# scipopt/SCIP-SDP

Measured on AMD Instinct MI355X. Metric: node-SDP solves/sec, dense block n x n with m vars (IPM iters/sec in iters_per_sec), higher is better.
Workload: dtype f64

## Files before the change

include/hipsdp_units.h:

```cpp
#ifndef HIPSDP_UNITS_H
#define HIPSDP_UNITS_H

#include "hipsdp.h"

#ifdef __cplusplus
extern "C" {
#endif

HIPSDP_API int  hipsdp_dgemm_selfcheck(int device, int M, int N, int K, int layB, int batch, int splitk, int flags, double beta,
   int* used_v2, long long* ndiff);
HIPSDP_API int  hipsdp_pass_at_unit(int device, int R, long long E, const double* A, const double* coef, double sa, const double* add, int split,
   double* out, int* chunks);
HIPSDP_API int  hipsdp_dgemm_selfcheck2(int device, int M, int N, int K, int layB, int batch, int splitk, int flags, double alpha, double beta,
   int reps, int* used, long long* ndiff, double* ms_tile, double* ms_fast);
HIPSDP_API int  hipsdp_gram_plan_info(int device, int M, long long K, int nslab, int* no, int* nd, int* nitems, double* span);
HIPSDP_API int  hipsdp_gram_selfcheck(int device, int M, long long K, int reps, int* used, double* maxdiff, long long* nrepro, double* ms_tile,
   double* ms_gram);
HIPSDP_API int  hipsdp_dgemm_selfcheck3(int device, int M, int N, int K, int layB, int batch, int splitk, int flags, double alpha, double beta,
   int reps, int* used, long long* ndiff, double* maxdiff, long long* nrepro, double* ms_tile, double* ms_fast);
HIPSDP_API int  hipsdp_schur_identity_unit(int device, int m1, int n, const double* A, double ws_gbytes, int full_storage, double* Mx,
   double* flops);
HIPSDP_API int  hipsdp_schur_dense(int device, int m1, int n, const double* A, const double* X, const double* Zinv, double* Mx,
   double ws_gbytes);
HIPSDP_API int  hipsdp_schur_w(int device, int m1, int n, const double* A, const double* X, const double* Z, double* Mx);
HIPSDP_API int  hipsdp_schur_shard_time(int device, int m1, int n, int nranks, int rank, int by_columns, int reps, double ws_gbytes, double* ms);
HIPSDP_API int  hipsdp_schur_var_share_time(int device, int m1, int n, int nranks, int rank, int cw, int reps, double* ms, double* a2a_bytes);
HIPSDP_API int  hipsdp_schur_sparse_unit(int device, int n, int m, long long nnz, const int* var, const int* row, const int* col,
   const double* val, const double* X, const double* Zinv, double* Mx);
HIPSDP_API int  hipsdp_mfma_peak(int device, double ms, double* tflops, double* ghz);
HIPSDP_API int  hipsdp_potrf(int device, int n, double* A, int* fail);
HIPSDP_API int  hipsdp_potrf_ex(int device, int n, double* A, int psd, int v1, double* dinv, int* regmask, int* fail);
HIPSDP_API int  hipsdp_potrs(int device, int n, const double* A, int nrhs, double* rhs);
HIPSDP_API int  hipsdp_potrs_seq(int device, int n, const double* A, int psd, int ncalls, const int* nrhs, const int* mode, double* rhs,
   int* regmask, int* fail);
HIPSDP_API int  hipsdp_potrf_small_unit(int device, int n, int pair, const double* base, const double* dir, double alpha, int set_flag,
   int want_gram, double* L, double* dinv, double* Mout, double* Linv, double* Gram, int* flag);
HIPSDP_API int  hipsdp_trtri(int device, int n, const double* A, double* Linv);
HIPSDP_API int  hipsdp_lambda_min(int device, int n, const double* W, int steps, double* theta, double* resid);
HIPSDP_API int  hipsdp_lambda_min_scaled(int device, int n, const double* L, const double* D, int steps, double* theta, double* resid);
HIPSDP_API int  hipsdp_solve1_fits(int m, int q, int nblk, const int* ns);
HIPSDP_API int  hipsdp_solve1_class(int m, int nblk, const int* ns);
HIPSDP_API unsigned long long hipsdp_gram_gen_next(unsigned long long* counter);
HIPSDP_API int  hipsdp_gram_key_match_unit(int m_a, int nblk_a, const int* n_a, const int* form_a, const unsigned long long* gen_a,
   const long long* ws_a, int m_b, int nblk_b, const int* n_b, const int* form_b, const unsigned long long* gen_b, const long long* ws_b);
HIPSDP_API int  hipsdp_syev_many_unit(int device, int count, const int* ns, const double* A, double* lam, double* V, int* launches);
HIPSDP_API int  hipsdp_tridiag_unit(int device, int n, const double* A, double* d, double* e, double* Vrefl, double* tau);
HIPSDP_API int  hipsdp_tvec_unit(int device, int n, const double* d, const double* e, double* lam, double* Z);

#ifdef __cplusplus
}
#endif

#endif
```

scip-sdp_amd/binding.py:

```python
import ctypes as C
import os
import numpy as np

_HERE = os.path.dirname(os.path.abspath(__file__))
LIBPATH = os.environ.get("HIPSDP_LIB", os.path.join(_HERE, "lib", "libhipsdp.so"))

STATUS_NAMES = {0: "optimal", 1: "dual_infeasible", 2: "dual_unbounded", 3: "both_infeasible", 4: "iterlimit",
                5: "numeric", 6: "timelimit", 7: "objlimit", -1: "unsolved"}


class Params(C.Structure):
    _fields_ = [("gaptol", C.c_double), ("feastol", C.c_double), ("infeastol", C.c_double), ("objlimit", C.c_double),
                ("timelimit", C.c_double), ("gamma", C.c_double), ("ws_gbytes", C.c_double), ("maxiter", C.c_int),
                ("verbose", C.c_int), ("lanczos_steps", C.c_int), ("settings", C.c_int), ("pabstol", C.c_double), ("preoptgap", C.c_double)]


class Info(C.Structure):
    _fields_ = [("status", C.c_int), ("iterations", C.c_int), ("pobj", C.c_double), ("dobj", C.c_double),
                ("pinf", C.c_double), ("dinf", C.c_double), ("dabs", C.c_double), ("gap", C.c_double), ("mu", C.c_double),
                ("tau", C.c_double), ("kappa", C.c_double), ("solve_seconds", C.c_double), ("schur_seconds", C.c_double),
                ("schur_flops", C.c_double), ("schur_calls", C.c_int), ("chol_fail", C.c_int), ("warm_started", C.c_int),
                ("settings_used", C.c_int), ("schur_flops_executed", C.c_double)]


# ... 419 lines not shown
    L = _f64(A).copy()
    n = L.shape[0]
    dinv = np.zeros(((n + 63) // 64) * 4096)
    mask = np.zeros(n, dtype=np.int32)
    fail = C.c_int(0)
    _chk(ulib().hipsdp_potrf_ex(device, n, _dp(L), int(psd), int(v1), _dp(dinv), _ip(mask), C.byref(fail)), "hipsdp_potrf_ex")
    return L, dinv, mask, fail.value


def potrs(A, rhs, device=0):
    A = _f64(A)
    r = _f64(rhs).copy()
    r2 = r.reshape(-1, A.shape[0])
    _chk(ulib().hipsdp_potrs(device, A.shape[0], _dp(A), r2.shape[0], _dp(r2)), "hipsdp_potrs")
    return r2.reshape(r.shape)


def potrs_seq(A, calls, psd=False, device=0):
    A = _f64(A)
    n = A.shape[0]
    nc = len(calls)
    slab = np.zeros((max(nc, 1), 4, n))
    nrhs = np.zeros(max(nc, 1), dtype=np.int32)
    mode = np.zeros(max(nc, 1), dtype=np.int32)
    for c, (md, r) in enumerate(calls):
        r = _f64(r).reshape(-1, n)
        nrhs[c], mode[c] = r.shape[0], md
        slab[c, :min(r.shape[0], 4)] = r[:4]
    mask = np.zeros(n, dtype=np.int32)
    fail = C.c_int(0)
    _chk(ulib().hipsdp_potrs_seq(device, n, _dp(A), int(psd), nc, _ip(nrhs), _ip(mode), _dp(slab), _ip(mask), C.byref(fail)),
         "hipsdp_potrs_seq")
    return [slab[c, :nrhs[c]].copy() for c in range(nc)], mask, fail.value


def potrf_small_unit(base, dir=None, alpha=0.0, pair=False, set_flag=False, want_gram=False, device=0):
    base = _f64(base)
    n = base.shape[-1]
    npb = 2 if pair else 1
    assert base.size == npb * n * n
    d = None if dir is None else _f64(dir)
    assert d is None or d.size == base.size
    shp = (2, n, n) if pair else (n, n)
    out = {"L": np.zeros(shp), "dinv": np.zeros((2, 64, 64) if pair else (64, 64)), "Mout": np.zeros(shp), "Linv": np.zeros(shp),
           "Gram": np.zeros(shp) if want_gram else None}
    flag = np.zeros(2, dtype=np.int32)
    _chk(ulib().hipsdp_potrf_small_unit(device, n, int(pair), _dp(base), None if d is None else _dp(d), C.c_double(alpha), int(set_flag),
                                        int(want_gram), _dp(out["L"]), _dp(out["dinv"]), _dp(out["Mout"]), _dp(out["Linv"]),
                                        None if not want_gram else _dp(out["Gram"]), _ip(flag)), "hipsdp_potrf_small_unit")
    out["flag"] = flag.copy() if pair else int(flag[0])
    return out


def trtri(A, device=0):
    A = _f64(A)
    Li = np.zeros_like(A)
    _chk(ulib().hipsdp_trtri(device, A.shape[0], _dp(A), _dp(Li)), "hipsdp_trtri")
    return Li


def lambda_min(W, steps=0, device=0):
    W = _f64(W)
    th = C.c_double(0.0)
    rs = C.c_double(0.0)
    _chk(ulib().hipsdp_lambda_min(device, W.shape[0], _dp(W), steps, C.byref(th), C.byref(rs)), "hipsdp_lambda_min")
    return th.value, rs.value


def syev(A, device=0):
    A = _f64(A)
    n = A.shape[0]
    lam = np.zeros(n)
    V = np.zeros((n, n))
    _chk(lib().hipsdp_syev(device, n, _dp(A), _dp(lam), _dp(V)), "hipsdp_syev")
    return lam, V


def syevx(A, il, iu, vectors=True, device=0):
    A = _f64(A)
    n = A.shape[0]
    k = max(0, iu - il + 1)
    lam = np.zeros(k)
    V = np.zeros((k, n)) if vectors else None
    _chk(lib().hipsdp_syevx(device, n, _dp(A), int(il), int(iu), _dp(lam), _dp(V) if vectors else None), "hipsdp_syevx")
    return lam, V


def syevx_below(A, bound, maxk, vectors=True, device=0):
    A = _f64(A)
    n = A.shape[0]
    lam = np.zeros(max(1, maxk))
    V = np.zeros((max(1, maxk), n)) if vectors else None
    cnt, nbelow = C.c_int(-1), C.c_int(-1)
    _chk(lib().hipsdp_syevx_below(device, n, _dp(A), C.c_double(bound), int(maxk), C.byref(cnt), C.byref(nbelow), _dp(lam),
                                  _dp(V) if vectors else None), "hipsdp_syevx_below")
    return lam[:cnt.value].copy(), (V[:cnt.value].copy() if vectors else None), nbelow.value


def syevr(A, vectors=True, device=0):
    A = _f64(A)
    n = A.shape[0]
    lam = np.zeros(n)
    V = np.zeros((n, n)) if vectors else None
    _chk(lib().hipsdp_syevr(device, n, _dp(A), _dp(lam), _dp(V) if vectors else None), "hipsdp_syevr")
    return lam, V

# ... 85 lines not shown
```

scip-sdp_amd/csrc/chol.hip:

```cpp
#include "hs_kernels.h"
#include "hs_wave.h"
#include <cstdlib>

#define NB 64

#ifdef PD_TIMING
__device__ long long pd_tbuf[16];
__device__ int pd_tj0;
#define PD_T(idx) do { if ( threadIdx.x == 0 && j0 == pd_tj0 && blockIdx.x == (gridDim.x > 1 ? 1u : 0u) ) pd_tbuf[idx] = wall_clock64(); } while (0)
extern "C" __attribute__((visibility("default"))) int hipsdp_debug_pd_timing(int j0, long long* out)
{
   if ( out != NULL && hipMemcpyFromSymbol(out, HIP_SYMBOL(pd_tbuf), sizeof(long long) * 16) != hipSuccess )
      return 1;
   return hipMemcpyToSymbol(HIP_SYMBOL(pd_tj0), &j0, sizeof(int)) == hipSuccess ? 0 : 1;
}
#else
#define PD_T(idx) do { } while (0)
#endif

__device__ __forceinline__ void sqrt_and_rsqrt(double d, double y0, double* sd, double* isd)
{
   const double t = d * y0;
   const double e = fma(-t, y0, 1.0);
   const double p = fma(0.375, e, 0.5);
// ... 449 lines not shown

__device__ __forceinline__ void ps_load_tile(const double* __restrict__ src, long long lda, int rows, double (*dst)[PD_LD])
{
   double v0[8], v1[8];
#pragma unroll
   for (int q = 0; q < 8; ++q)
   {
      const int e = threadIdx.x + 256 * q;
      const int r = e >> 5, c = (e & 31) * 2;
      v0[q] = 0.0; v1[q] = 0.0;
      if ( r < rows )
      {
         v0[q] = src[(long long) r * lda + c];
         v1[q] = src[(long long) r * lda + c + 1];
      }
   }
#pragma unroll
   for (int q = 0; q < 8; ++q)
   {
      const int e = threadIdx.x + 256 * q;
      const int r = e >> 5, c = (e & 31) * 2;
      dst[r][c] = v0[q];
      dst[r][c + 1] = v1[q];
   }
}

template<bool LOWTRI>
__device__ __forceinline__ void ps_mma(const double (*Ta)[PD_LD], const double (*Tb)[PD_LD], int wave, int lane, v4dc* acc)
{
   const int lr = lane & 15, lk = lane >> 4;
   double a[16];
#pragma unroll
   for (int sidx = 0; sidx < 16; ++sidx)
      a[sidx] = Ta[16 * wave + lr][4 * sidx + lk];
#pragma unroll
   for (int t = 0; t < 4; ++t)
      acc[t] = (v4dc){0.0, 0.0, 0.0, 0.0};
#pragma unroll
   for (int sidx = 0; sidx < 16; ++sidx)
   {
#pragma unroll
      for (int t = 0; t < 4; ++t)
      {
         if ( !LOWTRI || sidx < 4 * (t + 1) )
         {
            const double b = Tb[16 * t + lr][4 * sidx + lk];
            acc[t] = __builtin_amdgcn_mfma_f64_16x16x4f64(a[sidx], b, acc[t], 0, 0, 0);
         }
      }
   }
}

template<int NBK>
__global__ void __launch_bounds__(256) k_potrf_step(double* __restrict__ A, long long lda, int n, int kb, int nblk,
   double* __restrict__ dinv, int* __restrict__ flag, const double* __restrict__ diag0, double regtol, pd_ext ext)
{
   extern __shared__ __attribute__((aligned(16))) double pd_smem[];
   double* lstage = dinv + (long long) nblk * NB * NB;
   double (*bufA)[PD_LD] = reinterpret_cast<double (*)[PD_LD]>(pd_smem);
   double (*bufB)[PD_LD] = reinterpret_cast<double (*)[PD_LD]>(pd_smem + NB * PD_LD);
   const double* forced = pd_smem + 2 * NB * PD_LD + 2 * NB;
   const int tid = threadIdx.x, lane = tid & 63;
   const int wave = __builtin_amdgcn_readfirstlane(tid >> 6);
   const int lr = lane & 15, lk = lane >> 4;
   const int nS = nblk - kb;
   const int j0 = kb * NB;
   v4dc acc[4];

   if ( (int) blockIdx.x >= nS )
   {
      const int tt = (int) blockIdx.x - nS;
      int ti = (int) ((sqrt(8.0 * (double) tt + 1.0) - 1.0) * 0.5);
      while ( (ti + 1) * (ti + 2) / 2 <= tt ) ++ti;
      while ( ti * (ti + 1) / 2 > tt ) --ti;
      const int tj = tt - ti * (ti + 1) / 2;
      const int bi = kb + 1 + ti, bj = kb + 1 + tj;
      const int ri = min(NB, n - bi * NB), rj = min(NB, n - bj * NB);
      const double* Pi = A + (long long) bi * NB * lda + (j0 - NB);
      const double* Pj = A + (long long) bj * NB * lda + (j0 - NB);
      ps_load_tile(Pi, lda, ri, bufA);
      if ( bi != bj )
         ps_load_tile(Pj, lda, rj, bufB);
      __syncthreads();
      ps_mma<false>(bufA, bi != bj ? bufB : bufA, wave, lane, acc);
      double* C = A + (long long) bi * NB * lda + (long long) bj * NB;
#pragma unroll
      for (int t = 0; t < 4; ++t)
#pragma unroll
         for (int rr = 0; rr < 4; ++rr)
         {
            const int row = 16 * wave + lk + 4 * rr, col = 16 * t + lr;
            if ( row < ri && col < rj )
            {
               double* c = C + (long long) row * lda + col;
               double v = -acc[t][rr];
               v += *c;
               *c = v;
            }
         }
      return;
   }

   PD_T(0);
   const int rb = kb + (int) blockIdx.x;
   const int r0 = rb * NB;
   const int nb = min(NB, n - j0);
   const int rows = min(NB, n - r0);
   double* Akk = A + (long long) j0 * lda + j0;
// ... 56 lines not shown
      PD_T(2);
   }
   pd_ext e2 = ext;
   e2.from_lds = from_lds ? 1 : 0;
   e2.nostore = blockIdx.x > 0 ? 1 : 0;
   e2.Lout = (nS > 1) ? lstage + (long long) kb * NB * NB : NULL;
   pd_body<NBK>(Akk, lda, nb, j0, dinv + (long long) kb * NB * NB, flag, diag0, regtol, e2);
   if ( blockIdx.x == 0 )
   {
      if ( kb > 0 )
      {
         const double* src = lstage + (long long) (kb - 1) * NB * NB;
         double* dst = A + (long long) (j0 - NB) * lda + (j0 - NB);
         for (int e = tid; e < NB * NB; e += 256)
         {
            const int r = e >> 6, c = e & 63;
            if ( c <= r )
               dst[(long long) r * lda + c] = src[e];
         }
      }
      return;
   }
   PD_T(9);
   __syncthreads();
#pragma unroll
   for (int t = 0; t < 4; ++t)
#pragma unroll
      for (int rr = 0; rr < 4; ++rr)
      {
         const int row = 16 * wave + lk + 4 * rr, col = 16 * t + lr;
         double v = 0.0;
         if ( row < rows )
         {
            v = -accB[t][rr];
            v += ark[t][rr];
         }
         bufB[row][col] = v;
      }
   __syncthreads();
   ps_mma<true>(bufB, bufA, wave, lane, acc);
#pragma unroll
   for (int t = 0; t < 4; ++t)
#pragma unroll
      for (int rr = 0; rr < 4; ++rr)
      {
         const int row = 16 * wave + lk + 4 * rr, col = 16 * t + lr;
         if ( row < rows )
            Ark[(long long) row * lda + col] = forced[col] != 0.0 ? 0.0 : acc[t][rr];
      }
   PD_T(10);
}

template<int NBK>
static int launch_potrf_step(hipStream_t s, double* A, long long lda, int n, int kb, int nblk, double* dinv, int* flag,
   const double* diag0, const pd_ext& ext)
{
   static hs_attr_mask attr_done;
   HS_CALL( hs_func_max_lds(reinterpret_cast<const void*>(&k_potrf_step<NBK>), PD_SMEM_BYTES, &attr_done) );
   const int nS = nblk - kb;
   const int t = nblk - kb - 1;
   const int nT = kb > 0 ? t * (t + 1) / 2 : 0;
   hipLaunchKernelGGL((k_potrf_step<NBK>), dim3(nS + nT), dim3(256), PD_SMEM_BYTES, s, A, lda, n, kb, nblk, dinv, flag, diag0, 1e-13, ext);
   HS_LAUNCH_CHECK();
   return HS_OK;
}

template<int NBK>
static int launch_potrf_diag(hipStream_t s, double* Ajj, long long lda, int nb, int j0, double* dj, int* flag, const double* diag0,
   const pd_ext* extp = NULL)
{
   pd_ext ext = {NULL, NULL, 0.0, NULL, NULL, NULL, 0, 2, NULL};
   if ( extp != NULL )
      ext = *extp;
   static hs_attr_mask attr_done;
   HS_CALL( hs_func_max_lds(reinterpret_cast<const void*>(&k_potrf_diag<NBK>), PD_SMEM_BYTES, &attr_done) );
   hipLaunchKernelGGL((k_potrf_diag<NBK>), dim3(1), dim3(256), PD_SMEM_BYTES, s, Ajj, lda, nb, j0, dj, flag, diag0, 1e-13, ext);
   HS_LAUNCH_CHECK();
   return HS_OK;
}

int hs_potrf_small_ext(hipStream_t s, int n, double* L, double* dinv, int* flag, const double* base, const double* dir, double alpha,
   double* Mout, double* Linv, double* Gram, int set_flag)
{
   if ( n <= 0 )
      return HS_OK;
   if ( n > NB || base == NULL || (Gram != NULL && n > 32) )
      return HS_ERR_ARG;
   pd_ext ext = {base, dir, alpha, Mout, Linv, Gram, set_flag, 2, NULL};
   if ( n <= 16 )
      return launch_potrf_diag<16>(s, L, n, n, 0, dinv, flag, NULL, &ext);
   if ( n <= 32 )
      return launch_potrf_diag<32>(s, L, n, n, 0, dinv, flag, NULL, &ext);
   if ( n <= 48 )
      return launch_potrf_diag<48>(s, L, n, n, 0, dinv, flag, NULL, &ext);
   return launch_potrf_diag<64>(s, L, n, n, 0, dinv, flag, NULL, &ext);
}

template<int NBK>
static int launch_potrf_diag_pair(hipStream_t s, int n, const pd_job& J0, const pd_job& J1)
{
   static hs_attr_mask attr_done;
   HS_CALL( hs_func_max_lds(reinterpret_cast<const void*>(&k_potrf_diag_pair<NBK>), PD_SMEM_BYTES, &attr_done) );
   hipLaunchKernelGGL((k_potrf_diag_pair<NBK>), dim3(2), dim3(256), PD_SMEM_BYTES, s, J0, J1, (long long) n, n);
   HS_LAUNCH_CHECK();
   return HS_OK;
}

int hs_potrf_small_ext_pair(hipStream_t s, int n, double* const* L, double* const* dinv, int* const* flag, const double* const* base,
   const double* const* dir, double alpha, double* const* Mout, double* const* Linv, double* const* Gram, int set_flag)
{
   if ( n <= 0 )
      return HS_OK;
   if ( n > NB || base[0] == NULL || base[1] == NULL || ((Gram[0] != NULL || Gram[1] != NULL) && n > 32) )
      return HS_ERR_ARG;
   pd_job J[2];
   for (int k = 0; k < 2; ++k)
   {
      const pd_ext ext = {base[k], dir[k], alpha, Mout[k], Linv[k], Gram[k], set_flag, 2, NULL};
      J[k].A = L[k]; J[k].dinv = dinv[k]; J[k].flag = flag[k]; J[k].ext = ext;
   }
   if ( n <= 16 )
      return launch_potrf_diag_pair<16>(s, n, J[0], J[1]);
   if ( n <= 32 )
      return launch_potrf_diag_pair<32>(s, n, J[0], J[1]);
   if ( n <= 48 )
      return launch_potrf_diag_pair<48>(s, n, J[0], J[1]);
   return launch_potrf_diag_pair<64>(s, n, J[0], J[1]);
}

__global__ void k_zero_forced_cols(int rows, int nb, double* __restrict__ P, long long lda, const int* __restrict__ mask)
{
   for (long long e = (long long) blockIdx.x * blockDim.x + threadIdx.x; e < (long long) rows * nb; e += (long long) gridDim.x * blockDim.x)
   {
      const int r = (int) (e / nb), c = (int) (e - (long long) r * nb);
      if ( mask[c] )
         P[(long long) r * lda + c] = 0.0;
   }
}

static int g_potrf_force_v1 = 0;
int hs_potrf_force_v1(int on) { const int old = g_potrf_force_v1; g_potrf_force_v1 = on; return old; }

long long hs_potrf_dinv_len(int n)
{
   const long long nblk = n > 0 ? (n + NB - 1) / NB : 1;
   return (nblk > 1 ? 2 : 1) * nblk * NB * NB;
}

int hs_potrf(hipStream_t s, int n, double* A, double* dinv, int* flag, const double* diag0)
{
   return hs_potrf_psd(s, n, A, dinv, flag, diag0, NULL, 0);
}

int hs_potrf_psd(hipStream_t s, int n, double* A, double* dinv, int* flag, const double* diag0, int* regmask, int set_flag)
{
   if ( n <= 0 )
      return HS_OK;
   if ( diag0 != NULL && regmask == NULL && n > NB )
      return HS_ERR_ARG;
   static int rule = getenv("HIPSDP_PIVOT_RULE") != NULL ? atoi(getenv("HIPSDP_PIVOT_RULE")) : 3;
   pd_ext ext = {NULL, NULL, 0.0, NULL, NULL, NULL, (set_flag && n <= NB) ? 1 : 0, rule, regmask};
   const pd_ext* extp = ((diag0 != NULL && regmask != NULL) || ext.set_flag) ? &ext : NULL;
   const long long lda = n;
   const int nblk = (n + NB - 1) / NB;
   if ( nblk > 1 && !g_potrf_force_v1 )
   {
      pd_ext est = {NULL, NULL, 0.0, NULL, NULL, NULL, 0, rule, (diag0 != NULL) ? regmask : NULL, 0, 0, NULL};
      for (int b = 0; b < nblk; ++b)
      {
         const int nb = (n - b * NB) < NB ? (n - b * NB) : NB;
         if ( nb <= 16 )
            HS_CALL( launch_potrf_step<16>(s, A, lda, n, b, nblk, dinv, flag, diag0, est) );
         else if ( nb <= 32 )
            HS_CALL( launch_potrf_step<32>(s, A, lda, n, b, nblk, dinv, flag, diag0, est) );
         else
            HS_CALL( launch_potrf_step<64>(s, A, lda, n, b, nblk, dinv, flag, diag0, est) );
      }
      return HS_OK;
   }
   for (int b = 0; b < nblk; ++b)
   {
      const int j0 = b * NB;
      const int nb = (n - j0) < NB ? (n - j0) : NB;
      double* Ajj = A + (long long) j0 * lda + j0;
      double* dj = dinv + (long long) b * NB * NB;
      if ( nb <= 16 )
         HS_CALL( launch_potrf_diag<16>(s, Ajj, lda, nb, j0, dj, flag, diag0, extp) );
      else if ( nb <= 32 )
         HS_CALL( launch_potrf_diag<32>(s, Ajj, lda, nb, j0, dj, flag, diag0, extp) );
      else
         HS_CALL( launch_potrf_diag<64>(s, Ajj, lda, nb, j0, dj, flag, diag0, extp) );
      const int j1 = j0 + nb;
      const int rem = n - j1;
      if ( rem <= 0 )
         break;
      double* P = A + (long long) j1 * lda + j0;
      hs_gemm_args g1 = {rem, nb, nb, HS_KC, HS_KC, P, lda, 0, dj, NB, 0, P, lda, 0, 1.0, 0.0, 1, HS_GEMM_TILE64, 1, NULL};
      HS_CALL( hs_dgemm(s, &g1) );
      if ( diag0 != NULL && regmask != NULL )
      {
         long long blocks = ((long long) rem * nb + 255) / 256;
         if ( blocks > 1024 ) blocks = 1024;
         hipLaunchKernelGGL(k_zero_forced_cols, dim3((unsigned) blocks), dim3(256), 0, s, rem, nb, P, lda, regmask + j0);
         HS_LAUNCH_CHECK();
// ... 749 lines not shown
```

scip-sdp_amd/csrc/hs_kernels.h:

```cpp
#ifndef HS_KERNELS_H
#define HS_KERNELS_H

#include "hs_common.h"

int hs_fill(hipStream_t s, double* p, long long n, double v);
int hs_set_identity(hipStream_t s, double* A, int n, double v);
int hs_copy(hipStream_t s, double* dst, const double* src, long long n);
int hs_axpy(hipStream_t s, long long n, double a, const double* x, double* y);
int hs_scale_add(hipStream_t s, long long n, double a, const double* x, double b, const double* y, double* out);
int hs_mirror_lower(hipStream_t s, double* A, int n, long long lda);
int hs_symmetrize(hipStream_t s, double* A, int n);
int hs_transpose(hipStream_t s, int n, const double* src, double* dst);

int hs_gemv_n(hipStream_t s, int R, long long E, const double* A, long long lda, int nv, const double* const* V,
   double* out, long long ldo, double* ws, long long wsdoubles);
int hs_gemv_t(hipStream_t s, int R, long long E, const double* A, long long lda, const double* coef, double sa,
   const double* add, double* out);

int hs_gemv_t_chunks(int R, long long E);
int hs_gemv_t_ws(hipStream_t s, int R, long long E, const double* A, long long lda, const double* coef, double sa,
   const double* add, double* out, double* ws, long long wsdoubles);
int hs_gemv_t3(hipStream_t s, int R, long long E, const double* A, long long lda, const double* c0, const double* c1, const double* c2,
   double* o0, double* o1, double* o2);

void hs_red_batch_begin(hipStream_t s);
int hs_red_batch_end(void);
int hs_red_batch_end_publish(hipStream_t s, int n, const double* src, double* dst, unsigned long long seq, unsigned long long* flag);
void hs_red_batch_reset(void);
int hs_fill_scalar(hipStream_t s, double* p, double v);
int hs_red_batch_solve(hipStream_t s, int m, const double* dinv, const double* L, int nrhs, double* vec, long long ld);
struct hs_rb_finish { int m; double eta, rg, sigmu, tau, kappa, etk; const double* u1; const double* u2; double* dy; double* dyt; double* sc;
   int s0, bub, bh, wrp, bu1, dtau, dkappa, den; };
int hs_red_batch_finish(hipStream_t s, const void* fin, size_t bytes);
int hs_copy_scalar(hipStream_t s, double* dst, const double* src);
void hs_red_batch_hold(hipStream_t s);
int hs_red_batch_release(void);
int hs_red_batch_flush(void);
int hs_red_batch_end_all(void);
int hs_make_ext(hipStream_t s, int m, double s0, double s1, const double* v, double* ext);
int hs_lp_rows_small(hipStream_t s, int q, int m1, const double* Dext, const double* v, int mode, double eta, double sigmu, const double* x,
   const double* z, const double* rd, const double* elp, double* out1, double* out2);
#define HS_AS_MAXBLK 8
struct hs_as_args { int nblk; int n2[HS_AS_MAXBLK]; const double* A[HS_AS_MAXBLK]; const double* V[HS_AS_MAXBLK]; };
int hs_apply_A_small(hipStream_t s, int m1, const hs_as_args* B, int q, const double* Dext, const double* vlp, double* out, int epi,
   double scal, const double* vin, double* vout);
int hs_axpy3(hipStream_t s, double a, long long n1, const double* x1, double* y1, long long n2, const double* x2, double* y2,
   long long n3, const double* x3, double* y3);
int hs_dot(hipStream_t s, long long n, const double* a, const double* b, double* out, int accumulate, double* ws);
int hs_absmax(hipStream_t s, long long n, const double* a, double* out, int accumulate, double* ws);
int hs_ratio_min(hipStream_t s, long long n, const double* x, const double* d, double* out, int accumulate, double* ws);

#define HS_SMALL_N 48
int hs_dir_block_small(hipStream_t s, int n, double c, const double* X, const double* R, const double* E, const double* Zinv,
   double s1, double* out);
int hs_dirmat(hipStream_t s, int n, double s1, const double* Zinv, const double* X, const double* GZ, double* H);

int hs_lp_dir(hipStream_t s, int q, double sigmu, double eta, const double* x, const double* z, const double* rd_or_dz,
   const double* elp, double* out);
int hs_lp_scale_rows(hipStream_t s, int q, int cols, const double* x, const double* z, const double* D, double* S);
int hs_vec_mul(hipStream_t s, long long n, const double* a, const double* b, double* out);
int hs_lp_s0(hipStream_t s, int q, const double* x, const double* z, const double* beta, double* out, int accumulate, double* ws);

int hs_pack_rows(hipStream_t s, int m1, int n, long long Lp, const double* A, double* Apk);
int hs_packed_diag(hipStream_t s, int m1, int n, int ldd, long long Lp, const double* Apk, double* D);
int hs_sub_lower(hipStream_t s, int n, const double* S, double* C);
int hs_pack_weighted(hipStream_t s, int n, const double* V, double* pk);
int hs_unpack_sym(hipStream_t s, int n, const double* pk, double sa, const double* add, double* out);
int hs_zero_upper(hipStream_t s, double* A, int n);

struct hs_schur_ws
{
   double*   T;
   double*   U;
   double*   K;
   double*   V;
   long long capT, capV;
   long long chunk_cols;
   long long n2;
   long long kws_len;
   int       full;
   double*   U2;
   double*   V2;
   void*     evP[2];
   void*     evX[2];
   void*     ev_g2;
   int       (*after_g1)(void*);
   void*     after_g1_arg;
};
int  hs_schur_ws_alloc(hs_schur_ws* w, int m1, long long n2max, double budget_gb);
void hs_schur_ws_free(hs_schur_ws* w);
int  hs_schur_U(hipStream_t s, int m1, int n, const double* A, const double* X, const double* Zinv, double* Mx,
   hs_schur_ws* w, int j_begin, int j_end);
int  hs_schur_W(hipStream_t s, int m1, int n, const double* A, const double* R, const double* G, double* Mx, hs_schur_ws* w);
int  hs_schur_W_identity(hipStream_t s, int m1, int n, const double* A, double* Mx, hs_schur_ws* w);
int  hs_schur_W_identity_range(hipStream_t s, int m1, int n, const double* A, long long k0, long long k1, double* Mx, hs_schur_ws* w);
int  hs_schur_W_identity_packed(hipStream_t s, int m1, int n, const double* Apk, long long Lp, double* Mx, hs_schur_ws* w);
int  hs_schur_identity_packed_fits(const hs_schur_ws* w, int m1, int n);

int  hs_schur_Urows(hipStream_t s, int m1, int n, const double* A, const double* X, const double* Zinv, double* Mx,
   hs_schur_ws* w, int r_begin, int r_end);
void hs_shard_rows(int m1, int nranks, int rank, int* chunk_rows, int* first_begin, int* second_begin);
int  hs_schur_Wcols(hipStream_t s, int m1, int n, const double* A, const double* R, const double* G, double* Mx, hs_schur_ws* w,
   int c0, int cw);
void hs_shard_cols(int m1, int n, int nranks, int rank, int* c_begin, int* c_width);
int  hs_schur_Wvar(hipStream_t s, void* comm, int rank, int nranks, int m1, int n, const double* A, const double* R, const double* G,
   double* Mx, hs_schur_ws* w, int c0, int cw);
int  hs_schur_ws_alloc_var(hs_schur_ws* w, int m1, int nranks, int n, int cwmax);
int  hs_schur_ws_alloc_var_overlap(hs_schur_ws* w);
int  hs_schur_Wvar_all(hipStream_t s, hipStream_t sc, void* comm, int rank, int nranks, int m1, int n, const double* A, const double* R,
   const double* G, double* Mx, hs_schur_ws* w, int cwmax, int overlap);
void hs_var_rows(int m1, int nranks, int rank, int* r0, int* r1);
void hs_var_wrows(int n, int nranks, int rank, int* q0, int* q1);
int  hs_alltoall(void* comm, const double* send, double* recv, const long long* cnt, hipStream_t stream);
int  hs_allreduce_sum(void* comm, double* buf, long long count, hipStream_t stream);
int  hs_mirror_upper(hipStream_t s, double* A, int n, long long lda);
int  hs_allgather_inplace(void* comm, double* buf, long long count_per_rank, int rank, hipStream_t stream);
int  hs_allgather(void* comm, const double* send, double* recv, long long count_per_rank, hipStream_t stream);

struct hs_sparse;
int  hs_sp_prefers_sparse(int n, int m, long long nnz);
int  hs_sp_build(hs_sparse** out, int n, int m, long long nnz, const int* var, const int* row, const int* col, const double* val);
void hs_sp_free(hs_sparse* sp);
long long hs_sp_nnz(const hs_sparse* sp);
int  hs_sp_apply_A(hipStream_t s, const hs_sparse* sp, const double* V, double* out_var1);
int  hs_sp_apply_AT(hipStream_t s, const hs_sparse* sp, const double* coef, double* out);
int  hs_sp_schur(hipStream_t s, const hs_sparse* sp, const double* X, const double* Zinv, double* Mx);
int  hs_sp_expand(hipStream_t s, const hs_sparse* sp, double* A);

int hs_potrf(hipStream_t s, int n, double* A, double* dinv, int* flag, const double* diag0);
long long hs_potrf_dinv_len(int n);
int hs_potrf_psd(hipStream_t s, int n, double* A, double* dinv, int* flag, const double* diag0, int* regmask, int set_flag);
int hs_trtri(hipStream_t s, int n, const double* L, const double* dinv, double* Linv, double* tmp);
int hs_potrf_small_ext_pair(hipStream_t s, int n, double* const* L, double* const* dinv, int* const* flag, const double* const* base,
   const double* const* dir, double alpha, double* const* Mout, double* const* Linv, double* const* Gram, int set_flag);
int hs_potrf_small_ext(hipStream_t s, int n, double* L, double* dinv, int* flag, const double* base, const double* dir, double alpha,
   double* Mout, double* Linv, double* Gram, int set_flag);
int hs_schur_small(hipStream_t s, int m1, int nblk, const int* n, const double* const* A, const double* const* X,
   const double* const* Zinv, int q, const double* Dext, const double* x, const double* z, double* Mx, double* Lm, double* diagM);
int hs_trsv(hipStream_t s, int n, const double* L, const double* dinv, int nrhs, double* rhs, long long ldr, int mode);
long long hs_trsv_sync_ws(int n);
int hs_trsv_sync_init(hipStream_t s, int n, int* sync_ws, int* epoch);
int hs_trsv_sync(hipStream_t s, int n, const double* L, const double* dinv, int nrhs, double* rhs, long long ldr, int mode,
   int* sync_ws, int* epoch);

int hs_lanczos_lmin(hipStream_t s, int n, const double* W, int maxsteps, double* res, double* ws);
long long hs_lanczos_ws(int n, int maxsteps);
#define HS_STEP_MAXJOBS 32
struct hs_step_jobs { int nblk; int n[HS_STEP_MAXJOBS]; const double* L0[HS_STEP_MAXJOBS]; const double* D0[HS_STEP_MAXJOBS];
   const double* L1[HS_STEP_MAXJOBS]; const double* D1[HS_STEP_MAXJOBS]; double* res0[HS_STEP_MAXJOBS]; double* res1[HS_STEP_MAXJOBS]; };
int hs_steplen_small_multi(hipStream_t s, const hs_step_jobs* P, int maxsteps);
int hs_lmin_exact_multi(hipStream_t st, const hs_step_jobs* P);
int hs_lanczos_scaled_small(hipStream_t s, int n, int maxsteps, const double* L0, const double* D0, const double* L1, const double* D1,
   double* res0, double* res1);
int hs_lmin_scaled_tiny(hipStream_t s, int n, const double* L0, const double* D0, const double* L1, const double* D1, double* res0,
   double* res1);
int hs_lanczos_lmin2(hipStream_t s, int n, const double* W0, const double* W1, int maxsteps, double* res0, double* res1,
   double* ws0, double* ws1, int* rot, unsigned long long* dsync, int nwipe);
long long hs_lanczos_sync_words(void);
int hs_lanczos_sync_reset(hipStream_t s, unsigned long long* dsync, int* rot);

long long hs_syev_small_scratch(int n);
int hs_syev_small_dev(hipStream_t st, int n, const double* A, double* lam, double* V, double* scratch);
struct hs_eig_job { int n; int pad; const double* in; double* ws; };
long long hs_syev_many_vecpos(int n);
int hs_syev_many_class(int n);
int hs_syev_small_many(hipStream_t st, int count, const hs_eig_job* hjobs, const hs_eig_job* jobs, int* launches);

int hs_psd_project_one(int device, int n, int nnz, const int* row, const int* col, const double* val, double minev,
   double epsilon, int mode, int cap, int* nnz_out, int* rowout, int* colout, double* valout);

#define HS_EC_DENSE  0
#define HS_EC_PACKED 1
#define HS_EC_SPARSE 2
struct hs_sp_view { long long nnz, npos; const int *voff, *vrow, *vcol; const double* vval; const int *poff, *prow, *pcol, *pvar; const double* pval; };
void hs_sp_get_view(const hs_sparse* sp, hs_sp_view* v);
struct hs_ec_job
{
   int n, form, blk, pad;
   long long ld;
   const double* A;
   hs_sp_view sp;
   double* Z;
   double* ws;
   long long vpos;
// ... 321 lines not shown
```

scip-sdp_amd/csrc/ipm.hip:

```cpp
#include "hs_kernels.h"
#include "hs_gram_cache.h"
#include "../../include/hipsdp.h"
#include <rocprofiler-sdk-roctx/roctx.h>
#include <vector>
#include <atomic>
#include <utility>
#include <functional>
#include <chrono>
#include <algorithm>
#include <cmath>
#include <cassert>
#include <cstdio>
#include <cstdlib>
#include <cstring>

enum
{
   SC_AX0 = 0,
   SC_DOBJ,
   SC_XZ,
   SC_RP2,
   SC_RD2,
   SC_RDLPMAX,
   SC_HP2,
// ... 747 lines not shown
      for (double** pm : mats)
         HS_CALL( dalloc(pm, n2) );
      const long long nd = hs_potrf_dinv_len(B.n);
      HS_CALL( dalloc(&R.dinvz, nd) );
      HS_CALL( dalloc(&R.dinvx, nd) );
      R.Lp = (((long long) B.n * (B.n + 1) / 2) + 1) & ~1LL;
      a_written(s, R);
      R.Apk = NULL;
      R.pkv = NULL;
      if ( B.n > 64 && !R.sparse )
      {
         if ( hipMalloc((void**) &R.Apkown, (size_t) ((arowsA > 0 ? arowsA : 1) * R.Lp) * sizeof(double)) != hipSuccess )
         {
            (void) hipGetLastError();
            R.Apkown = NULL;
         }
         else
         {
            R.Apk = R.Apkown - (long long) s->a_r0 * R.Lp;
            HS_CALL( dalloc(&R.pkv, 2 * R.Lp) );
            HS_HIP( hipMemsetAsync(R.pkv, 0, (size_t) (2 * R.Lp) * sizeof(double), s->stream) );
         }
      }
   }
   HS_CALL( dalloc(&s->b, mA) );
   HS_CALL( dalloc(&s->Dext, (long long) qA * m1A) );
   HS_CALL( dalloc(&s->y, mA) ); HS_CALL( dalloc(&s->ys, mA) );
   double** qv[] = {&s->x, &s->z, &s->rd, &s->tmpq, &s->hl, &s->beta, &s->elp, &s->dxa, &s->dza, &s->dx, &s->dz, &s->xs, &s->zs};
   for (double** p : qv) HS_CALL( dalloc(p, qA) );
   double** ev[] = {&s->yt, &s->dyt, &s->wt, &s->AX, &s->AH, &s->tmpe};
   for (double** p : ev) HS_CALL( dalloc(p, m1A) );
   double** mv[] = {&s->rp, &s->u2, &s->dy, &s->dya};
   for (double** p : mv) HS_CALL( dalloc(p, mA) );
   HS_CALL( dalloc(&s->rhs2, 3LL * mA) );
   s->u1 = s->rhs2 + 2LL * m;
   HS_CALL( dalloc(&s->cvec, 2LL * m1A) );
   HS_CALL( dalloc(&s->Mx, (m1A + 32) * m1A) );
   HS_CALL( dalloc(&s->Lm, (long long) mA * mA) );
   HS_CALL( dalloc(&s->dinvm, hs_potrf_dinv_len(mA)) );
   HS_CALL( dalloc(&s->Slp, (long long) qA * m1A) );
   HS_CALL( dalloc(&s->regmask, mA) );
   s->nsc = SC_FIXED_END + 8 * (nblocks > 0 ? nblocks : 1) + 8;
   HS_CALL( dalloc(&s->sc, s->nsc + 4) );
   s->flags = reinterpret_cast<int*>(s->sc + s->nsc);
   if ( s->hsc_cap < s->nsc + 8 )
   {
      if ( s->hsc != NULL ) (void) hipHostFree(s->hsc);
      s->hsc = NULL;
      s->hsc_cap = 2LL * (s->nsc + 8);
      HS_HIP( hipHostMalloc((void**) &s->hsc, (size_t) s->hsc_cap * sizeof(double), hipHostMallocMapped | hipHostMallocCoherent) );
      HS_HIP( hipHostGetDevicePointer((void**) &s->hsc_dev, s->hsc, 0) );
      memset(s->hsc, 0, (size_t) s->hsc_cap * sizeof(double));
   }
   HS_CALL( dalloc(&s->red_ws, 1024) );
   s->gemv_ws_len = 8192 + 4LL * 1024 * 4;
   HS_CALL( dalloc(&s->gemv_ws, s->gemv_ws_len) );
   {
      long long need = 0;
      for (auto& B : s->blk)
      {
         const long long n2 = (long long) B.n * B.n, lp = (long long) B.n * (B.n + 1) / 2;
         need = std::max(need, std::max((long long) hs_gemv_t_chunks(mA + 1, n2) * n2, (long long) hs_gemv_t_chunks(mA + 1, lp) * lp));
      }
      s->gemvt_ws_len = need;
      if ( need > 0 )
         HS_CALL( dalloc(&s->gemvt_ws, need) );
   }
   HS_CALL( dalloc(&s->lan_ws, hs_lanczos_ws(nmax, 256)) );
   HS_CALL( dalloc(&s->lan_ws2, hs_lanczos_ws(nmax, 256)) );
   if ( nmax > 64 )
   {
      if ( s->lan_sync == NULL )
         HS_HIP( hipMalloc((void**) &s->lan_sync, (size_t) hs_lanczos_sync_words() * sizeof(unsigned long long)) );
      HS_CALL( hs_lanczos_sync_reset(s->stream, s->lan_sync, s->lan_rot) );
   }
   HS_CALL( dalloc(&s->trsv_ws, hs_trsv_sync_ws(mA)) );
   if ( m > 2 * 64 )
      HS_CALL( hs_trsv_sync_init(s->stream, m, s->trsv_ws, &s->trsv_epoch) );
   s->trsv_epoch = 0;
   s->sws.T = s->sws.U = s->sws.K = s->sws.V = s->sws.U2 = s->sws.V2 = NULL;
   s->sws.evP[0] = s->sws.evP[1] = s->sws.evX[0] = s->sws.evX[1] = NULL; s->sws.ev_g2 = NULL; s->sws.after_g1 = NULL; s->sws.after_g1_arg = NULL;
   HS_HIP( hipMemsetAsync(s->Dext, 0, (size_t) ((long long) q * m1 > 0 ? (long long) q * m1 : 1) * sizeof(double), s->stream) );
   HS_HIP( hipMemsetAsync(s->b, 0, (size_t) (m > 0 ? m : 1) * sizeof(double), s->stream) );
   HS_HIP( hipStreamSynchronize(s->stream) );
   s->shaped = true;
   s->have_start = false;
   return HIPSDP_OK;
}

extern "C" int hipsdp_set_obj(hipsdp_solver* s, const double* b)
{
   if ( s == NULL || !s->shaped ) return HIPSDP_ERR_ARG;
   HS_HIP( hipSetDevice(s->device) );
   if ( s->m > 0 )
      HS_CALL( stage_upload(s, s->b, b, (size_t) s->m * sizeof(double)) );
   s->zero_b = false;
   s->solved = false;
   return HIPSDP_OK;
}

__global__ void k_scatter_coo(long long nnz, int n, const int* __restrict__ var, const int* __restrict__ row,
   const int* __restrict__ col, const double* __restrict__ val, double* __restrict__ A, int r0, int r1, double* __restrict__ A0,
   int vmax, int* __restrict__ err)
{
   const long long n2 = (long long) n * n;
   for (long long e = (long long) blockIdx.x * blockDim.x + threadIdx.x; e < nnz; e += (long long) gridDim.x * blockDim.x)
   {
// ... 373 lines not shown
      else
      {
         int *dact, *dkept;
         HS_CALL( flush_cmds(s) );
         HS_CALL( dalloc(&dact, nactive) ); HS_CALL( dalloc(&dkept, nkept) );
         HS_HIP( hipMemcpyAsync(dact, activevars, (size_t) nactive * sizeof(int), hipMemcpyHostToDevice, s->stream) );
         HS_HIP( hipMemcpyAsync(dkept, kept, (size_t) nkept * sizeof(int), hipMemcpyHostToDevice, s->stream) );
         hipLaunchKernelGGL(k_master_gather, dim3((unsigned) g), dim3(256), 0, s->stream, nactive, nkept, N, dact, dkept,
            s->master_A[master_block], B.A);
         HS_LAUNCH_CHECK();
         HS_HIP( hipStreamSynchronize(s->stream) );
         dfree(dact); dfree(dkept);
      }
   }
   s->solved = false;
   return HIPSDP_OK;
}

extern "C" int hipsdp_set_block_dense(hipsdp_solver* s, int block, const double* A)
{
   if ( s == NULL || !s->shaped || block < 0 || block >= (int) s->blk.size() )
      return HIPSDP_ERR_ARG;
   HS_HIP( hipSetDevice(s->device) );
   HS_CALL( stage_sync(s) );
   Block& B = s->blk[block];
   if ( B.sparse )
   {
      set_err("hipsdp_set_block_dense: the block is kept as nonzeros (hipsdp_set_shape2 with a count): use hipsdp_add_entries");
      return HIPSDP_ERR_ARG;
   }
   const size_t n2b = (size_t) B.n * B.n * sizeof(double);
   a_written(s, B);
   if ( s->a_r1 > s->a_r0 )
      HS_HIP( hipMemcpy(B.Aown, A + (size_t) s->a_r0 * B.n * B.n, (size_t) (s->a_r1 - s->a_r0) * n2b, hipMemcpyHostToDevice) );
   if ( B.A0sep != NULL )
      HS_HIP( hipMemcpy(B.A0sep, A, n2b, hipMemcpyHostToDevice) );
   s->solved = false;
   return HIPSDP_OK;
}

extern "C" int hipsdp_set_lp(hipsdp_solver* s, const double* Dext)
{
   if ( s == NULL || !s->shaped ) return HIPSDP_ERR_ARG;
   HS_HIP( hipSetDevice(s->device) );
   if ( s->q > 0 )
      HS_CALL( stage_upload(s, s->Dext, Dext, (size_t) s->q * (s->m + 1) * sizeof(double)) );
   s->zero_D = false;
   s->solved = false;
   return HIPSDP_OK;
}

int hs_gen_dense(hipStream_t s, int n, int i0, int i1, long long seed, double* A);
static int ensure_packed(hipsdp_solver* s);
static int pass_A(hipsdp_solver* s, Block& B, const double* V, double* out);
static int pass_AT(hipsdp_solver* s, Block& B, const double* coef, double sa, const double* add, double* out);

extern "C" int hipsdp_gen_planted(hipsdp_solver* s, int n, int m, long long seed, const double* Xstar, const double* Zstar,
   const double* ystar, double* b_out)
{
   if ( s == NULL || !s->shaped || s->blk.size() != 1 || s->blk[0].n != n || s->m != m || s->q != 0 || s->blk[0].sparse )
      return HIPSDP_ERR_ARG;
   HS_HIP( hipSetDevice(s->device) );
   HS_CALL( stage_sync(s) );
   Block& B = s->blk[0];
   const long long n2 = (long long) n * n;
   const int m1 = m + 1;
   hipStream_t st = s->stream;
   a_written(s, B);
   HS_CALL( hs_gen_dense(st, n, s->a_r0 > 1 ? s->a_r0 : 1, s->a_r1, seed, B.A) );
   HS_HIP( hipMemcpyAsync(B.Z, Zstar, (size_t) n2 * sizeof(double), hipMemcpyHostToDevice, st) );
   HS_HIP( hipMemcpyAsync(B.X, Xstar, (size_t) n2 * sizeof(double), hipMemcpyHostToDevice, st) );
   HS_HIP( hipMemsetAsync(s->yt, 0, sizeof(double), st) );
   HS_HIP( hipMemcpyAsync(s->yt + 1, ystar, (size_t) m * sizeof(double), hipMemcpyHostToDevice, st) );
   HS_HIP( hipMemsetAsync(B.A0, 0, (size_t) n2 * sizeof(double), st) );
   if ( s->shardA )
   {
      a_written(s, B);
      HS_CALL( ensure_packed(s) );
      HS_CALL( pass_AT(s, B, s->yt, -1.0, B.Z, B.T1) );
      HS_CALL( hs_symmetrize(st, B.T1, n) );
      HS_CALL( hs_copy(st, B.A0, B.T1, n2) );
      HS_CALL( pass_A(s, B, B.X, s->AX) );
   }
   else
   {
   HS_CALL( hs_gemv_t(st, m1, n2, B.A, n2, s->yt, -1.0, B.Z, B.T1) );
   HS_CALL( hs_symmetrize(st, B.T1, n) );
   HS_CALL( hs_copy(st, B.A, B.T1, n2) );
   const double* v = B.X;
   HS_CALL( hs_gemv_n(st, m1, n2, B.A, n2, 1, &v, s->AX, m1, s->gemv_ws, s->gemv_ws_len) );
   }
   HS_CALL( hs_copy(st, s->b, s->AX + 1, m) );
   HS_HIP( hipMemcpyAsync(b_out, s->b, (size_t) m * sizeof(double), hipMemcpyDeviceToHost, st) );
   HS_HIP( hipStreamSynchronize(st) );
   a_written(s, B);
   s->solved = false;
   return HIPSDP_OK;
}

void hs_gen_set_density(double density);

extern "C" int hipsdp_gen_planted_density(hipsdp_solver* s, int n, int m, long long seed, double density, const double* Xstar,
   const double* Zstar, const double* ystar, double* b_out)
{
   hs_gen_set_density(density);
   const int rc = hipsdp_gen_planted(s, n, m, seed, Xstar, Zstar, ystar, b_out);
   hs_gen_set_density(1.0);
// ... 47 lines not shown
   HS_HIP( hipSetDevice(s->device) );
   if ( s->m > 0 )
      HS_CALL( stage_upload(s, s->y, y, (size_t) s->m * sizeof(double)) );
   for (size_t k = 0; k < s->blk.size(); ++k)
   {
      const size_t bytes = (size_t) s->blk[k].n * s->blk[k].n * sizeof(double);
      HS_CALL( stage_upload(s, s->blk[k].X, X[k], bytes) );
      HS_CALL( stage_upload(s, s->blk[k].Z, Z[k], bytes) );
   }
   if ( s->q > 0 )
   {
      HS_CALL( stage_upload(s, s->x, x, (size_t) s->q * sizeof(double)) );
      HS_CALL( stage_upload(s, s->z, z, (size_t) s->q * sizeof(double)) );
   }
   s->have_start = true;
   s->s1_sol_host = false;
   return HIPSDP_OK;
}


__global__ void k_flag_nonpositive(int q, const double* __restrict__ x, const double* __restrict__ z, int* __restrict__ flag)
{
   const int i = blockIdx.x * blockDim.x + threadIdx.x;
   if ( i < q && (!(x[i] > 0.0) || !(z[i] > 0.0) || !(x[i] < 1e300) || !(z[i] < 1e300)) )
      atomicExch(flag, 1);
}

__global__ void k_rp(int m, double tau, const double* __restrict__ b, const double* __restrict__ AX, double* __restrict__ rp)
{
   const int i = blockIdx.x * blockDim.x + threadIdx.x;
   if ( i < m )
      rp[i] = b[i] * tau - AX[1 + i];
}

__global__ void k_rhs2(int m, const double* __restrict__ Mx, const double* __restrict__ b, double* __restrict__ rhs2)
{
   const int i = blockIdx.x * blockDim.x + threadIdx.x;
   if ( i < m )
   {
      rhs2[i] = Mx[1 + i];
      rhs2[m + i] = b[i];
   }
}

__global__ void k_after_solve2(int m, const double* __restrict__ rhs2, double* __restrict__ u2, double* __restrict__ wt)
{
   const int i = blockIdx.x * blockDim.x + threadIdx.x;
   if ( i == 0 )
      wt[0] = 1.0;
   if ( i < m )
   {
      u2[i] = rhs2[m + i] - rhs2[i];
      wt[1 + i] = -rhs2[i];
   }
}

__global__ void __launch_bounds__(128) k_solve2_small(int m, const double* __restrict__ Mx, const double* __restrict__ b,
   const double* __restrict__ dinv, const double* __restrict__ L, double* __restrict__ rhs2, double* __restrict__ u2, double* __restrict__ wt,
   int subst)
{
   __shared__ double r[2][64], t[2][64], c[2][64];
   __shared__ double sL[64 * 65];
   const int k = threadIdx.x >> 6, i = threadIdx.x & 63;
   r[k][i] = (i < m) ? (k == 0 ? Mx[1 + i] : b[i]) : 0.0;
   if ( subst )
   {
      for (int e = threadIdx.x; e < m * m; e += 128)
      {
         const int ii = e / m, jj = e - ii * m;
         if ( jj <= ii )
            sL[ii * 65 + jj] = L[(long long) ii * m + jj];
      }
      __syncthreads();
      const double x = hs_wl_msolve(sL, m, i, r[k][i]);
      __syncthreads();
      r[k][i] = x;
      __syncthreads();
      if ( i < m )
         rhs2[k * m + i] = x;
      if ( k == 0 )
      {
         if ( i == 0 )
            wt[0] = 1.0;
         if ( i < m )
         {
            u2[i] = r[1][i] - r[0][i];
            wt[1 + i] = -r[0][i];
         }
      }
      return;
   }
   __syncthreads();
   double acc = 0.0;
   if ( i < m )
      for (int j = 0; j <= i; ++j)
         acc += dinv[i * 64 + j] * r[k][j];
   t[k][i] = acc;
   __syncthreads();
   double res = 0.0;
   if ( i < m )
   {
      for (int j = 0; j <= i; ++j)
         res += L[(long long) i * m + j] * t[k][j];
      res = r[k][i] - res;
   }
   c[k][i] = res;
// ... 36 lines not shown
      if ( i < m )
      {
         u2[i] = r[1][i] - r[0][i];
         wt[1 + i] = -r[0][i];
      }
   }
}

__global__ void k_h(int m, double eta, const double* __restrict__ AH, const double* __restrict__ rp, double* __restrict__ h)
{
   const int i = blockIdx.x * blockDim.x + threadIdx.x;
   if ( i < m )
      h[i] = AH[1 + i] - eta * rp[i];
}

__global__ void k_finish_dir(int m, double eta, double rg, double sigmu, double tau, double kappa, double etk,
   const double* __restrict__ u1, const double* __restrict__ u2, double* __restrict__ dy, double* __restrict__ dyt,
   double* __restrict__ sc)
{
   const double den = sc[SC_S0] + kappa / tau + sc[SC_BUB];
   const double num = -eta * rg + (sigmu - tau * kappa - etk) / tau - sc[SC_BH] - eta * sc[SC_WRP] + sc[SC_BU1];
   const double dtau = num / den;
   const int i = blockIdx.x * blockDim.x + threadIdx.x;
   if ( i == 0 )
   {
      sc[SC_DTAU] = dtau;
      sc[SC_DKAPPA] = (sigmu - tau * kappa - etk - kappa * dtau) / tau;
      sc[SC_DEN] = den;
      dyt[0] = -dtau;
   }
   if ( i < m )
   {
      const double v = u1[i] - u2[i] * dtau;
      dy[i] = v;
      dyt[1 + i] = v;
   }
}

__global__ void k_dz_combine(long long n2, double* __restrict__ dZ, const double* __restrict__ P2, const double* __restrict__ sc, double eta,
   const double* __restrict__ Rd)
{
   const double dtau = sc[SC_DTAU];
   for (long long i = (long long) blockIdx.x * blockDim.x + threadIdx.x; i < n2; i += (long long) gridDim.x * blockDim.x)
      dZ[i] = (dZ[i] - dtau * P2[i]) + eta * Rd[i];
}

__global__ void k_cert(long long n2, double tau, const double* __restrict__ Rd, const double* __restrict__ A0, double* __restrict__ out)
{
   for (long long i = (long long) blockIdx.x * blockDim.x + threadIdx.x; i < n2; i += (long long) gridDim.x * blockDim.x)
      out[i] = Rd[i] + tau * A0[i];
}

static inline dim3 g1d(long long n) { long long g = (n + 255) / 256; if ( g < 1 ) g = 1; if ( g > 4096 ) g = 4096; return dim3((unsigned) g); }

static int gemm_on(hipStream_t st, int layA, int layB, int M, int N, int K, double alpha, const double* A, long long lda,
   const double* B, long long ldb, double beta, double* C, long long ldc, int flags = 0)
{
   (void) hs_red_batch_flush();
   hs_gemm_args g = {M, N, K, layA, layB, A, lda, 0, B, ldb, 0, C, ldc, 0, alpha, beta, 1, flags, 1, NULL};
   return hs_dgemm(st, &g);
}

static int gemm(hipsdp_solver* s, int layA, int layB, int M, int N, int K, double alpha, const double* A, long long lda,
   const double* B, long long ldb, double beta, double* C, long long ldc, int flags = 0)
{
   return gemm_on(s->stream, layA, layB, M, N, K, alpha, A, lda, B, ldb, beta, C, ldc, flags);
}

static int fork2(hipsdp_solver* s)
{
   if ( !s->use2 )
      return HS_OK;
   s->busy2 = true;
   HS_HIP( hipEventRecord(s->evFork, s->stream) );
   HS_HIP( hipStreamWaitEvent(s->stream2, s->evFork, 0) );
   return HS_OK;
}

static int join2(hipsdp_solver* s)
{
   if ( !s->use2 )
      return HS_OK;
   s->busy2 = false;
   HS_HIP( hipEventRecord(s->evJoin, s->stream2) );
   HS_HIP( hipStreamWaitEvent(s->stream, s->evJoin, 0) );
   return HS_OK;
}

static int ensure_schur_ws(hipsdp_solver* s)
{
   if ( s->sws.T != NULL )
      return HS_OK;
   {
      bool anydense = false;
      for (auto& B : s->blk) anydense = anydense || !B.sparse;
      if ( !anydense && !s->blk.empty() )
         return HS_OK;
   }
   const int m1 = s->m + 1;
   long long n2max = 1;
   for (auto& B : s->blk) { const long long n2 = (long long) B.n * B.n; if ( !B.sparse && n2 > n2max ) n2max = n2; }
   double budget = s->par.ws_gbytes > 0.0 ? s->par.ws_gbytes : 40.0;
   const char* env = getenv("HIPSDP_WS_GB");
   if ( env != NULL && atof(env) > 0.0 )
      budget = atof(env);
   else if ( s->par.ws_gbytes <= 0.0 && s->comm == NULL )
// ... 205 lines not shown
   *r1 = *r0 + c < m1 ? *r0 + c : m1;
}

static int ensure_sparse(hipsdp_solver* s)
{
   for (auto& B : s->blk)
      if ( B.sparse && (B.sp_dirty || B.sp == NULL) )
      {
         if ( B.sp != NULL ) hs_sp_free(B.sp);
         B.sp = NULL;
         HS_HIP( hipStreamSynchronize(s->stream) );
         const SpHost& h = *B.sph;
         HS_CALL( hs_sp_build(&B.sp, B.n, s->m, (long long) h.var.size(), h.var.data(), h.row.data(), h.col.data(), h.val.data()) );
         B.sp_dirty = false;
      }
   return HS_OK;
}

__global__ void k_sp_base(long long n2, const double* __restrict__ c, const double* __restrict__ A0, double sa, const double* __restrict__ add,
   double* __restrict__ out)
{
   const double c0 = c[0];
   for (long long e = (long long) blockIdx.x * blockDim.x + threadIdx.x; e < n2; e += (long long) gridDim.x * blockDim.x)
      out[e] = c0 * A0[e] + (add != NULL ? sa * add[e] : 0.0);
}

__global__ void __launch_bounds__(1024) k_sp_dot0(long long n, const double* __restrict__ a, const double* __restrict__ b, double* __restrict__ out)
{
   __shared__ double part[16];
   double acc = 0.0;
   for (long long e = threadIdx.x; e < n; e += 1024)
      acc += a[e] * b[e];
#pragma unroll
   for (int off = 32; off > 0; off >>= 1)
      acc += __shfl_xor(acc, off, 64);
   if ( (threadIdx.x & 63) == 0 )
      part[threadIdx.x >> 6] = acc;
   __syncthreads();
   if ( threadIdx.x == 0 )
   {
      double t = 0.0;
      for (int w = 0; w < 16; ++w)
         t += part[w];
      out[0] = t;
   }
}

__global__ void k_add_col0(int m1, const double* __restrict__ v, double* __restrict__ Mx)
{
   for (int i = blockIdx.x * blockDim.x + threadIdx.x; i < m1; i += gridDim.x * blockDim.x)
      Mx[(long long) i * m1] += v[i];
}

static int pass_A(hipsdp_solver* s, Block& B, const double* V, double* out)
{
   const int m1 = s->m + 1;
   if ( B.sparse )
   {
      HS_CALL( hs_gemv_n(s->stream, 1, (long long) B.n * B.n, B.A0, (long long) B.n * B.n, 1, &V, out, 1, s->gemv_ws, s->gemv_ws_len) );
      return hs_sp_apply_A(s->stream, B.sp, V, out + 1);
   }
   if ( passes_sharded(s, B) )
   {
      int c, r0, r1;
      pass_rows(s, &c, &r0, &r1);
      if ( s->passg == NULL )
         HS_CALL( dalloc(&s->passg, (long long) c * s->nranks) );
      double* mine = s->passg + (long long) s->rank * c;
      if ( B.Apk != NULL )
      {
         HS_CALL( hs_pack_weighted(s->stream, B.n, V, B.pkv) );
         const double* v = B.pkv;
         if ( r1 > r0 )
            HS_CALL( hs_gemv_n(s->stream, r1 - r0, B.Lp, B.Apk + (long long) r0 * B.Lp, B.Lp, 1, &v, mine, r1 - r0, s->gemv_ws, s->gemv_ws_len) );
      }
      else if ( r1 > r0 )
      {
         const long long n2 = (long long) B.n * B.n;
         HS_CALL( hs_gemv_n(s->stream, r1 - r0, n2, B.A + (long long) r0 * n2, n2, 1, &V, mine, r1 - r0, s->gemv_ws, s->gemv_ws_len) );
      }
      hs_comm_phase(1);
      const int rcg = hs_allgather_inplace(s->comm, s->passg, c, s->rank, s->stream);
      hs_comm_phase(2);
      HS_CALL( rcg );
      return hs_copy(s->stream, out, s->passg, m1);
   }
   if ( B.Apk != NULL )
   {
      HS_CALL( hs_pack_weighted(s->stream, B.n, V, B.pkv) );
      const double* v = B.pkv;
      return hs_gemv_n(s->stream, m1, B.Lp, B.Apk, B.Lp, 1, &v, out, m1, s->gemv_ws, s->gemv_ws_len);
   }
   return hs_gemv_n(s->stream, m1, (long long) B.n * B.n, B.A, (long long) B.n * B.n, 1, &V, out, m1, s->gemv_ws, s->gemv_ws_len);
}

static int pass_AT(hipsdp_solver* s, Block& B, const double* coef, double sa, const double* add, double* out)
{
   const int m1 = s->m + 1;
   const long long n2 = (long long) B.n * B.n;
   if ( B.sparse )
   {
      hipLaunchKernelGGL(k_sp_base, g1d(n2), dim3(256), 0, s->stream, n2, coef, B.A0, sa, add, out);
      HS_LAUNCH_CHECK();
      return hs_sp_apply_AT(s->stream, B.sp, coef, out);
   }
   if ( passes_sharded(s, B) )
   {
      int c, r0, r1;
      pass_rows(s, &c, &r0, &r1);
      if ( B.Apk != NULL )
      {
         HS_CALL( hs_gemv_t(s->stream, r1 - r0, B.Lp, B.Apk + (long long) r0 * B.Lp, B.Lp, coef + r0, 0.0, NULL, B.pkv + B.Lp) );
         hs_comm_phase(1);
         const int rcr = hs_allreduce_sum(s->comm, B.pkv + B.Lp, B.Lp, s->stream);
         hs_comm_phase(2);
         HS_CALL( rcr );
         return hs_unpack_sym(s->stream, B.n, B.pkv + B.Lp, sa, add, out);
      }
      HS_CALL( hs_gemv_t(s->stream, r1 - r0, n2, B.A + (long long) r0 * n2, n2, coef + r0, s->rank == 0 ? sa : 0.0,
            s->rank == 0 ? add : NULL, out) );
      hs_comm_phase(1);
      const int rcr = hs_allreduce_sum(s->comm, out, n2, s->stream);
      hs_comm_phase(2);
      return rcr;
   }
   if ( B.Apk != NULL )
   {
      HS_CALL( hs_gemv_t_ws(s->stream, m1, B.Lp, B.Apk, B.Lp, coef, 0.0, NULL, B.pkv + B.Lp, s->gemvt_ws, s->gemvt_ws_len) );
      return hs_unpack_sym(s->stream, B.n, B.pkv + B.Lp, sa, add, out);
   }
   return hs_gemv_t_ws(s->stream, m1, n2, B.A, n2, coef, sa, add, out, s->gemvt_ws, s->gemvt_ws_len);
}

#define AS_MAXBLK HS_AS_MAXBLK

static bool small_problem(const hipsdp_solver* s)
{
   if ( s->blk.size() > AS_MAXBLK || s->q > 4096 || s->m + 1 > 4096 || s->shardA )
      return false;
   long long tot = 0;
   for (auto& B : s->blk)
   {
      if ( B.Apk != NULL || B.sparse || B.A == NULL )
         return false;
      tot += (long long) B.n * B.n;
   }
   return tot <= 8192;
}

static bool batch_regions(const hipsdp_solver* s)
{
   static int on = -1;
   if ( on < 0 )
   {
      const char* env = getenv("HIPSDP_BATCH");
      on = (env != NULL && env[0] == '0') ? 0 : 1;
   }
   return on != 0 && s->comm == NULL && small_problem(s);
}

struct BatchRegion
{
   bool on;
   BatchRegion(hipsdp_solver* s, bool want) : on(want) { if ( on ) hs_red_batch_hold(s->stream); }
   int close() { if ( !on ) return HS_OK; on = false; return hs_red_batch_release(); }
   ~BatchRegion() { if ( on ) (void) hs_red_batch_release(); }
};

static int apply_A_small(hipsdp_solver* s, double* const* Vk, const double* vlp, double* out, int epi, double scal,
   const double* vin, double* vout)
{
   if ( !small_problem(s) )
      return 0;
   for (auto& Bk : s->blk)
      if ( Bk.A == NULL )
         return 0;
   hs_as_args B;
   B.nblk = (int) s->blk.size();
   for (int k = 0; k < AS_MAXBLK; ++k)
   {
      B.n2[k] = 0; B.A[k] = NULL; B.V[k] = NULL;
   }
   for (size_t k = 0; k < s->blk.size(); ++k)
   {
      B.n2[k] = s->blk[k].n * s->blk[k].n;
      B.A[k] = s->blk[k].A;
      B.V[k] = Vk[k];
   }
   const int rc = hs_apply_A_small(s->stream, s->m + 1, &B, s->q, s->Dext, vlp, out, epi, scal, vin, vout);
   if ( rc != HS_OK )
      return -rc;
   return 1;
}

static int apply_A(hipsdp_solver* s, double* const* Vk, const double* vlp, double* out)
{
   const int m1 = s->m + 1;
   bool first = true;
   for (size_t k = 0; k < s->blk.size(); ++k)
   {
      Block& B = s->blk[k];
      const double* v = Vk[k];
      double* dst = first ? out : s->tmpe;
      HS_CALL( pass_A(s, B, v, dst) );
      if ( !first )
         HS_CALL( hs_axpy(s->stream, m1, 1.0, s->tmpe, out) );
      first = false;
   }
   if ( first )
      HS_CALL( hs_fill(s->stream, out, m1, 0.0) );
   if ( s->q > 0 )
      HS_CALL( hs_gemv_t(s->stream, s->q, m1, s->Dext, m1, vlp, 1.0, out, out) );
   return HS_OK;
}

struct QueueSwap
{
   hipsdp_solver* s;
   explicit QueueSwap(hipsdp_solver* s_) : s(s_) { std::swap(s->stream, s->stream2); }
   ~QueueSwap() { std::swap(s->stream, s->stream2); }
};

static const int SOLVE_MODE = 3 | 4;

static int direction(hipsdp_solver* s, double sigma, double eta, double mu, double rg, bool useE, double etk, int part = 0,
   bool u1_solved = false, int split = 0)
{
   const int m = s->m, m1 = s->m + 1, q = s->q;
   const double sigmu = sigma * mu;
   std::vector<double*> Hs;
   int fusedA = 0;
   BatchRegion region(s, part == 0 && batch_regions(s));
   if ( part != 2 )
   {
   for (auto& B : s->blk)
   {
      const int n = B.n;
      const long long n2 = (long long) n * n;
      if ( n <= HS_SMALL_N )
         HS_CALL( hs_dir_block_small(s->stream, n, eta, B.X, B.Rd, useE ? B.E : NULL, B.Zinv, sigmu, B.H) );
      else
      {
         if ( useE )
            HS_CALL( hs_copy(s->stream, B.G, B.E, n2) );
         HS_CALL( gemm(s, HS_KC, HS_MC, n, n, n, eta, B.X, n, B.Rd, n, useE ? 1.0 : 0.0, B.G, n) );
         HS_CALL( gemm(s, HS_KC, HS_MC, n, n, n, 1.0, B.G, n, B.Zinv, n, 0.0, B.GZ, n) );
         HS_CALL( hs_dirmat(s->stream, n, sigmu, B.Zinv, B.X, B.GZ, B.H) );
      }
      Hs.push_back(B.H);
   }
   if ( q > 0 )
      HS_CALL( hs_lp_dir(s->stream, q, sigmu, eta, s->x, s->z, s->rd, useE ? s->elp : NULL, s->hl) );
   fusedA = part == 1 ? 0 : apply_A_small(s, Hs.data(), s->hl, s->AH, 1, eta, s->rp, s->u1);
   if ( fusedA < 0 )
      return -fusedA;
   if ( fusedA == 0 )
      HS_CALL( apply_A(s, Hs.data(), s->hl, s->AH) );
   if ( fusedA == 0 && m > 0 )
   {
      HS_CALL( hs_red_batch_flush() );
      hipLaunchKernelGGL(k_h, g1d(m), dim3(256), 0, s->stream, m, eta, s->AH, s->rp, s->u1);
      HS_LAUNCH_CHECK();
   }
   if ( part == 1 )
      return HS_OK;
   }
   const bool fuse_solve = (fusedA == 1) && m > 0 && m <= 64;
   if ( m > 0 && !fuse_solve && !u1_solved )
   {
      HS_CALL( hs_red_batch_flush() );
      HS_CALL( hs_trsv_sync(s->stream, m, s->Lm, s->dinvm, 1, s->u1, m, SOLVE_MODE, s->trsv_ws, &s->trsv_epoch) );
   }
   hs_red_batch_begin(s->stream);
   if ( fuse_solve )
      (void) hs_red_batch_solve(s->stream, m, s->dinvm, s->Lm, 1, s->u1, m);
   HS_CALL( hs_fill_scalar(s->stream, s->sc + SC_BH, 0.0) );
   for (auto& B : s->blk)
      HS_CALL( hs_dot(s->stream, (long long) B.n * B.n, B.B, B.H, s->sc + SC_BH, 1, s->red_ws) );
   if ( q > 0 )
      HS_CALL( hs_dot(s->stream, q, s->beta, s->hl, s->sc + SC_BH, 1, s->red_ws) );
   HS_CALL( hs_dot(s->stream, m, s->rhs2, s->rp, s->sc + SC_WRP, 0, s->red_ws) );
   HS_CALL( hs_dot(s->stream, m, s->b, s->u1, s->sc + SC_BU1, 0, s->red_ws) );
   bool finished = false;
   if ( fuse_solve )
   {
      hs_rb_finish F = {m, eta, rg, sigmu, s->tau, s->kappa, etk, s->u1, s->u2, s->dy, s->dyt, s->sc,
         SC_S0, SC_BUB, SC_BH, SC_WRP, SC_BU1, SC_DTAU, SC_DKAPPA, SC_DEN};
      finished = hs_red_batch_finish(s->stream, &F, sizeof(F)) == 1;
   }
   HS_CALL( hs_red_batch_end() );
   if ( !finished )
   {
      HS_CALL( hs_red_batch_flush() );
      hipLaunchKernelGGL(k_finish_dir, g1d(m > 0 ? m : 1), dim3(256), 0, s->stream, m, eta, rg, sigmu, s->tau, s->kappa, etk,
         s->u1, s->u2, s->dy, s->dyt, s->sc);
      HS_LAUNCH_CHECK();
   }
   for (auto& B : s->blk)
   {
      const int n = B.n;
      const long long n2 = (long long) n * n;
      if ( split == 0 )
         HS_CALL( pass_AT(s, B, s->dyt, eta, B.Rd, B.dZ) );
      else
      {
         if ( split == 1 )
         {
            if ( &B == &s->blk[0] )
            {
               HS_CALL( hs_make_ext(s->stream, m, 0.0, 1.0, s->u1, s->cvec + m1) );
               HS_LAUNCH_CHECK();
            }
            HS_CALL( pass_AT(s, B, s->cvec + m1, 0.0, NULL, B.dZ) );
         }
         HS_CALL( hs_red_batch_flush() );
         hipLaunchKernelGGL(k_dz_combine, g1d(n2), dim3(256), 0, s->stream, n2, B.dZ, B.P2, s->sc, eta, B.Rd);
         HS_LAUNCH_CHECK();
      }
      if ( n <= HS_SMALL_N )
         HS_CALL( hs_dir_block_small(s->stream, n, 1.0, B.X, B.dZ, useE ? B.E : NULL, B.Zinv, sigmu, B.dX) );
      else
      {
         if ( useE )
            HS_CALL( hs_copy(s->stream, B.G, B.E, n2) );
         HS_CALL( gemm(s, HS_KC, HS_MC, n, n, n, 1.0, B.X, n, B.dZ, n, useE ? 1.0 : 0.0, B.G, n) );
         HS_CALL( gemm(s, HS_KC, HS_MC, n, n, n, 1.0, B.G, n, B.Zinv, n, 0.0, B.GZ, n) );
         HS_CALL( hs_dirmat(s->stream, n, sigmu, B.Zinv, B.X, B.GZ, B.dX) );
      }
   }
   if ( q > 0 )
   {
      if ( small_problem(s) )
      {
         HS_CALL( hs_lp_rows_small(s->stream, q, m1, s->Dext, s->dyt, 1, eta, sigmu, s->x, s->z,
            s->rd, useE ? s->elp : NULL, s->dz, s->dx) );
      }
      else
      {
         const double* v = s->dyt;
         HS_CALL( hs_gemv_n(s->stream, q, m1, s->Dext, m1, 1, &v, s->tmpq, q, s->gemv_ws, s->gemv_ws_len) );
         HS_CALL( hs_scale_add(s->stream, q, 1.0, s->tmpq, eta, s->rd, s->dz) );
         HS_CALL( hs_lp_dir(s->stream, q, sigmu, 1.0, s->x, s->z, s->dz, useE ? s->elp : NULL, s->dx) );
      }
   }
   return region.close();
}

static int steplen_enqueue(hipsdp_solver* s)
{
   int k = 0;
   hipStream_t st = s->stream, st2 = s->use2 ? s->stream2 : s->stream;
   HS_CALL( fork2(s) );
   for (auto& B : s->blk)
   {
      const int n = B.n;
      if ( n <= 64 )
         continue;
      HS_CALL( gemm_on(st, HS_KC, HS_MC, n, n, n, 1.0, B.LxInv, n, B.dX, n, 0.0, B.T1, n) );
      HS_CALL( gemm_on(st, HS_KC, HS_KC, n, n, n, 1.0, B.T1, n, B.LxInv, n, 0.0, B.W, n) );
      HS_CALL( gemm_on(st2, HS_KC, HS_MC, n, n, n, 1.0, B.LzInv, n, B.dZ, n, 0.0, B.T2, n) );
      HS_CALL( gemm_on(st2, HS_KC, HS_KC, n, n, n, 1.0, B.T2, n, B.LzInv, n, 0.0, B.W2, n) );
   }
   HS_CALL( join2(s) );
   int nmax_blk = 0;
   for (auto& B : s->blk)
      if ( B.n > nmax_blk ) nmax_blk = B.n;
   for (int cls = 0; cls < 2; ++cls)
   {
      hs_step_jobs J;
      J.nblk = 0;
// ... 683 lines not shown
         for (auto& B : s->blk)
         {
            const long long n2 = (long long) B.n * B.n;
            HS_CALL( hs_symmetrize(st, B.X, B.n) );
            HS_CALL( hs_symmetrize(st, B.Z, B.n) );
            HS_CALL( factor(st, B.n, B.Lz, B.dinvz, B.Z, 0) );
            HS_CALL( factor(st, B.n, B.Lx, B.dinvx, B.X, 1) );
            HS_CALL( hs_dot(st, n2, B.X, B.Z, s->sc + SC_XZ, 1, s->red_ws) );
         }
         if ( q > 0 )
         {
            hipLaunchKernelGGL(k_flag_nonpositive, g1d(q), dim3(256), 0, st, q, s->x, s->z, s->flags + 3);
            HS_LAUNCH_CHECK();
            HS_CALL( hs_dot(st, q, s->x, s->z, s->sc + SC_XZ, 1, s->red_ws) );
         }
         int f4[4];
         HS_HIP( hipMemcpyAsync(s->hsc + 4, s->flags, 4 * sizeof(int), hipMemcpyDeviceToHost, st) );
         HS_HIP( hipMemcpyAsync(s->hsc + 8, s->sc + SC_XZ, sizeof(double), hipMemcpyDeviceToHost, st) );
         HS_HIP( hipStreamSynchronize(st) );
         memcpy(f4, s->hsc + 4, sizeof(f4));
         const double mu0 = s->hsc[8] / (double) (N > 0 ? N : 1);
         if ( f4[0] == 0 && f4[1] == 0 && f4[3] == 0 && std::isfinite(mu0) && mu0 > 0.0 )
         {
            s->tau = 1.0;
            s->kappa = mu0;
            factors_valid = true;
         }
         else
            s->have_start = false;
      }
      if ( !s->have_start )
      {
         const double xi = fmax(1.0, sqrt(fmax(fmax(normb, normC), 1.0)));
         HS_CALL( hs_fill(st, s->y, m, 0.0) );
         for (auto& B : s->blk)
         {
            HS_CALL( hs_set_identity(st, B.X, B.n, xi) );
            HS_CALL( hs_set_identity(st, B.Z, B.n, xi) );
         }
         HS_CALL( hs_fill(st, s->x, q, xi) );
         HS_CALL( hs_fill(st, s->z, q, xi) );
         s->tau = 1.0;
         s->kappa = xi * xi;
         identity_start = !no_identity_start;
      }
      info->warm_started = s->have_start ? 1 : 0;
      s->have_start = false;
      return HS_OK;
   }

   int enqueue_residuals()
   {
      const bool recur = rd_have && !want_cert;
      HS_CALL( hs_make_ext(st, m, -s->tau, 1.0, s->y, s->yt) );
      HS_LAUNCH_CHECK();
      hs_red_batch_begin(st);
      HS_CALL( hs_fill_scalar(st, s->sc + SC_RD2, 0.0) );
      HS_CALL( hs_fill_scalar(st, s->sc + SC_XZ, 0.0) );
      HS_CALL( hs_fill_scalar(st, s->sc + SC_HD2, 0.0) );
      std::vector<double*> Xs;
      for (int k = 0; k < K; ++k)
      {
         Block& B = s->blk[k];
         const long long n2 = (long long) B.n * B.n;
         if ( !recur )
            HS_CALL( pass_AT(s, B, s->yt, -1.0, B.Z, B.Rd) );
         else if ( rd_pending )
            HS_CALL( hs_scale_add(st, n2, rd_scale, B.Rd, 0.0, NULL, B.Rd) );
         HS_CALL( hs_dot(st, n2, B.Rd, B.Rd, s->sc + SC_BLK(k, 0), 0, s->red_ws) );
         HS_CALL( hs_dot(st, n2, B.X, B.Z, s->sc + SC_XZ, 1, s->red_ws) );
         if ( want_cert )
         {
            HS_CALL( hs_red_batch_flush() );
            hipLaunchKernelGGL(k_cert, g1d(n2), dim3(256), 0, st, n2, s->tau, B.Rd, B.A0, B.T1);
            HS_LAUNCH_CHECK();
            HS_CALL( hs_dot(st, n2, B.T1, B.T1, s->sc + SC_HD2, 1, s->red_ws) );
         }
         Xs.push_back(B.X);
      }
      if ( q > 0 )
      {
         if ( small_problem(s) )
         {
            HS_CALL( hs_lp_rows_small(st, q, m1, s->Dext, s->yt, 0, 0.0, 0.0, s->x, s->z,
               (const double*) NULL, (const double*) NULL, s->rd, (double*) NULL) );
         }
         else if ( !recur )
         {
            const double* v = s->yt;
            HS_CALL( hs_gemv_n(st, q, m1, s->Dext, m1, 1, &v, s->tmpq, q, s->gemv_ws, s->gemv_ws_len) );
            HS_CALL( hs_scale_add(st, q, 1.0, s->tmpq, -1.0, s->z, s->rd) );
         }
         else if ( rd_pending )
            HS_CALL( hs_scale_add(st, q, rd_scale, s->rd, 0.0, NULL, s->rd) );
         HS_CALL( hs_dot(st, q, s->rd, s->rd, s->sc + SC_RD2, 1, s->red_ws) );
         HS_CALL( hs_absmax(st, q, s->rd, s->sc + SC_RDLPMAX, 0, s->red_ws) );
         HS_CALL( hs_dot(st, q, s->x, s->z, s->sc + SC_XZ, 1, s->red_ws) );
         if ( want_cert )
         {
            HS_CALL( hs_red_batch_flush() );
            HS_HIP( hipMemcpy2DAsync(s->tmpq, sizeof(double), s->Dext, (size_t) m1 * sizeof(double), sizeof(double), (size_t) q, hipMemcpyDeviceToDevice, st) );
            HS_CALL( hs_scale_add(st, q, s->tau, s->tmpq, 1.0, s->rd, s->tmpq) );
            HS_CALL( hs_dot(st, q, s->tmpq, s->tmpq, s->sc + SC_HD2, 1, s->red_ws) );
         }
      }
      else
         HS_CALL( hs_fill_scalar(st, s->sc + SC_RDLPMAX, 0.0) );
      const int fusedA = apply_A_small(s, Xs.data(), s->x, s->AX, 2, s->tau, s->b, s->rp);
      if ( fusedA < 0 )
         return -fusedA;
      if ( fusedA == 0 )
         HS_CALL( apply_A(s, Xs.data(), s->x, s->AX) );
      HS_CALL( hs_copy_scalar(st, s->sc + SC_AX0, s->AX) );
      if ( fusedA == 0 )
      {
         HS_CALL( hs_red_batch_flush() );
         hipLaunchKernelGGL(k_rp, g1d(m > 0 ? m : 1), dim3(256), 0, st, m, s->tau, s->b, s->AX, s->rp);
         HS_LAUNCH_CHECK();
      }
      HS_CALL( hs_dot(st, m, s->rp, s->rp, s->sc + SC_RP2, 0, s->red_ws) );
      HS_CALL( hs_dot(st, m, s->AX + 1, s->AX + 1, s->sc + SC_HP2, 0, s->red_ws) );
      HS_CALL( hs_dot(st, m, s->b, s->y, s->sc + SC_DOBJ, 0, s->red_ws) );
      rd_pending = false;
// ... 392 lines not shown
         HS_LAUNCH_CHECK();
         HS_CALL( hs_sp_schur(st, B.sp, B.X, B.Zinv, s->Mx) );
      }
      if ( q > 0 )
      {
         HS_CALL( hs_lp_scale_rows(st, q, m1, s->x, s->z, s->Dext, s->Slp) );
         HS_CALL( gemm(s, HS_MC, HS_MC, m1, m1, q, 1.0, s->Dext, m1, s->Slp, m1, 1.0, s->Mx, m1, HS_GEMM_LOWER) );
      }
      return hs_mirror_lower(st, s->Mx, m1, m1);
   }

   int solve_m()
   {
      phase_mark(s, PH_MSOLVE);
      predH_queued = predH_joined = split_dz = false;
      if ( s->use2 && s->comm == NULL && !small_problem(s) && m > 0 )
      {
         HS_CALL( fork2(s) );
         {
            QueueSwap sw(s);
            HS_CALL( direction(s, 0.0, 1.0, mu, rg, false, 0.0, 1) );
         }
         predH_queued = true;
      }
      if ( m > 0 )
      {
         if ( !schur_small )
         {
            HS_HIP( hipMemcpy2DAsync(s->Lm, (size_t) m * sizeof(double), s->Mx + m1 + 1, (size_t) m1 * sizeof(double),
                  (size_t) m * sizeof(double), (size_t) m, hipMemcpyDeviceToDevice, st) );
            HS_HIP( hipMemcpy2DAsync(s->dya, sizeof(double), s->Mx + m1 + 1, (size_t) (m1 + 1) * sizeof(double), sizeof(double), (size_t) m,
                  hipMemcpyDeviceToDevice, st) );
         }
         HS_CALL( hs_potrf_psd(st, m, s->Lm, s->dinvm, s->flags + 2, s->dya, s->regmask, setf) );
         if ( m <= 64 )
         {
            hipLaunchKernelGGL(k_solve2_small, dim3(1), dim3(128), 0, st, m, s->Mx, s->b, s->dinvm, s->Lm, s->rhs2, s->u2, s->wt, hs_small_solve_by_substitution());
            HS_LAUNCH_CHECK();
         }
         else
         {
            hipLaunchKernelGGL(k_rhs2, g1d(m), dim3(256), 0, st, m, s->Mx, s->b, s->rhs2);
            HS_LAUNCH_CHECK();
            if ( predH_queued )
            {
               HS_CALL( join2(s) );
               predH_joined = true;
               HS_CALL( hs_trsv_sync(st, m, s->Lm, s->dinvm, 3, s->rhs2, m, SOLVE_MODE, s->trsv_ws, &s->trsv_epoch) );
            }
            else
               HS_CALL( hs_trsv_sync(st, m, s->Lm, s->dinvm, 2, s->rhs2, m, SOLVE_MODE, s->trsv_ws, &s->trsv_epoch) );
         }
      }
      if ( m == 0 || m > 64 )
      {
         hipLaunchKernelGGL(k_after_solve2, g1d(m1), dim3(256), 0, st, m, s->rhs2, s->u2, s->wt);
         HS_LAUNCH_CHECK();
      }
      hs_red_batch_begin(st);
      HS_CALL( hs_fill_scalar(st, s->sc + SC_S0, 0.0) );
      split_dz = predH_joined && s->comm == NULL;
      for (auto& B : s->blk)
         if ( B.Apk == NULL )
            split_dz = false;
      if ( split_dz )
      {
         HS_CALL( hs_make_ext(st, m, 1.0, 1.0, s->u2, s->cvec) );
         HS_CALL( hs_make_ext(st, m, 0.0, 1.0, s->u1, s->cvec + m1) );
         HS_LAUNCH_CHECK();
      }
      for (auto& B : s->blk)
      {
         const int n = B.n;
         const long long n2 = (long long) n * n;
         bool swept = false;
         if ( split_dz )
         {
            if ( B.P2 == NULL )
            {
               HS_CALL( dalloc(&B.P2, n2) );
               HS_CALL( dalloc(&B.pk3, 3 * B.Lp) );
            }
            const int r3 = hs_gemv_t3(st, m1, B.Lp, B.Apk, B.Lp, s->wt, s->cvec, s->cvec + m1, B.pk3, B.pk3 + B.Lp, B.pk3 + 2 * B.Lp);
            if ( r3 < 0 )
               return -r3;
            if ( r3 == 1 )
            {
               HS_CALL( hs_unpack_sym(st, n, B.pk3, 0.0, NULL, B.B) );
               HS_CALL( hs_unpack_sym(st, n, B.pk3 + B.Lp, 0.0, NULL, B.P2) );
               HS_CALL( hs_unpack_sym(st, n, B.pk3 + 2 * B.Lp, 0.0, NULL, B.dZ) );
               swept = true;
            }
            else
            {
               HS_CALL( pass_AT(s, B, s->cvec, 0.0, NULL, B.P2) );
               HS_CALL( pass_AT(s, B, s->cvec + m1, 0.0, NULL, B.dZ) );
            }
         }
         if ( !swept )
            HS_CALL( pass_AT(s, B, s->wt, 0.0, NULL, B.B) );
         HS_CALL( gemm(s, HS_KC, HS_MC, n, n, n, 1.0, B.X, n, B.B, n, 0.0, B.T1, n) );
         HS_CALL( gemm(s, HS_KC, HS_MC, n, n, n, 1.0, B.T1, n, B.Zinv, n, 0.0, B.W, n) );
         HS_CALL( hs_dot(st, n2, B.B, B.W, s->sc + SC_S0, 1, s->red_ws) );
      }
      if ( q > 0 )
      {
         const double* v = s->wt;
         HS_CALL( hs_gemv_n(st, q, m1, s->Dext, m1, 1, &v, s->beta, q, s->gemv_ws, s->gemv_ws_len) );
         HS_CALL( hs_lp_s0(st, q, s->x, s->z, s->beta, s->sc + SC_S0, 1, s->red_ws) );
      }
      HS_CALL( hs_dot(st, m, s->b, s->rhs2 + m, s->sc + SC_BUB, 0, s->red_ws) );
      return hs_red_batch_end();
   }

   int predictor()
   {
      phase_mark(s, PH_PRED);
      if ( predH_queued && !predH_joined )
         HS_CALL( join2(s) );
      HS_CALL( direction(s, 0.0, 1.0, mu, rg, false, 0.0, predH_queued ? 2 : 0, predH_joined, split_dz ? 2 : 0) );
      HS_CALL( steplen_enqueue(s) );
      HS_CALL( read_scalars(s, hs, hflags) );
      float ms = 0.f;
      if ( hipEventElapsedTime(&ms, s->ev0, s->ev1) == hipSuccess )
         schur_ms += ms;
      info->schur_calls++;
      for (auto& B : s->blk)
         if ( !gram_cached )
            info->schur_flops += (gram_only_used && !B.sparse ? 0.0 : 4.0 * m1 * (double) B.n * B.n * B.n) + (double) m1 * m1 * (double) B.n * B.n;
      if ( hflags[0] != 0 || hflags[1] != 0 || hflags[2] != 0 )
      {
         if ( par.verbose )
            printf("hipsdp: Cholesky failure flags Z=%d X=%d M=%d\n", hflags[0], hflags[1], hflags[2]);
         return halt(HIPSDP_STATUS_NUMERIC);
      }
      const double aa = fmin(1.0, steplen_host(s, hs));
      dta = hs.v[SC_DTAU];
      dka = hs.v[SC_DKAPPA];
      if ( !std::isfinite(aa) || !std::isfinite(dta) )
      {
         if ( par.verbose )
            printf("hipsdp: predictor not finite (alpha %g dtau %g)\n", aa, dta);
         return halt(HIPSDP_STATUS_NUMERIC);
      }
      sigma = (1.0 - aa) * (1.0 - aa) * (1.0 - aa);
      sigma = fmin(1.0, fmax(sigma_floor, sigma));
      eta = 1.0 - sigma;
      return HS_OK;
   }

   int corrector()
   {
      phase_mark(s, PH_CORR);
      for (auto& B : s->blk)
         HS_CALL( gemm(s, HS_KC, HS_MC, B.n, B.n, B.n, 1.0, B.dX, B.n, B.dZ, B.n, 0.0, B.E, B.n) );
      {
         BatchRegion region(s, batch_regions(s));
         if ( q > 0 )
            HS_CALL( hs_vec_mul(st, q, s->dx, s->dz, s->elp) );
         HS_CALL( direction(s, sigma, eta, mu, rg, true, dta * dka, 0, false, split_dz ? 1 : 0) );
         HS_CALL( region.close() );
      }
      HS_CALL( steplen_enqueue(s) );
      HS_CALL( read_scalars(s, hs, NULL) );
      amax = steplen_host(s, hs);
      alpha = fmin(1.0, gamma_eff * amax);
      dt = hs.v[SC_DTAU];
      dk = hs.v[SC_DKAPPA];
      if ( !std::isfinite(alpha) || !std::isfinite(dt) || !std::isfinite(dk) )
      {
         if ( par.verbose )
            printf("hipsdp: corrector not finite (alpha %g dtau %g dkappa %g)\n", alpha, dt, dk);
         return halt(HIPSDP_STATUS_NUMERIC);
      }
      return HS_OK;
   }

   int update()
   {
      phase_mark(s, PH_UPDATE);
      for (auto& B : s->blk)
      {
         const long long n2 = (long long) B.n * B.n;
         if ( B.n <= 64 )
            continue;
         HS_CALL( hs_copy(st, B.Xs, B.X, n2) );
         HS_CALL( hs_copy(st, B.Zs, B.Z, n2) );
      }
      tau0 = s->tau;
      kappa0 = s->kappa;
      applied = 0.0;
      return (small_all && K > 0) ? step_small() : step_general();
   }

   int step_small()
   {
      for (int attempt = 0; attempt < 8; ++attempt)
      {
         if ( !setf )
            HS_HIP( hipMemsetAsync(s->flags, 0, 8 * sizeof(int), st) );
         for (auto& B : s->blk)
         {
            double* L2[2] = {B.Lx, B.Lz};
            double* di2[2] = {B.dinvx, B.dinvz};
            int* fl2[2] = {s->flags + 1, s->flags + 0};
            const double* ba2[2] = {B.X, B.Z};
            const double* dr2[2] = {B.dX, B.dZ};
            double* mo2[2] = {B.Xs, B.Zs};
            double* li2[2] = {B.LxInv, B.LzInv};
            double* gr2[2] = {NULL, B.n <= 32 ? B.Zinv : NULL};
            HS_CALL( hs_potrf_small_ext_pair(st, B.n, L2, di2, fl2, ba2, dr2, alpha, mo2, li2, gr2, setf) );
         }
         swap_trial();
         if ( batch_regions(s) )
            hs_red_batch_hold(st);
         HS_CALL( apply_step() );
         HS_CALL( enqueue_residuals() );
         HS_CALL( read_scalars(s, hs, hflags) );
         if ( hflags[0] == 0 && hflags[1] == 0 )
         {
            for (auto& B : s->blk)
               B.derived_valid = true;
            factors_valid = true;
            residuals_ready = true;
            alpha_last = alpha;
            return HS_OK;
         }
         swap_trial();
         alpha *= 0.5;
         info->chol_fail++;
      }
      return give_up(true);
   }

   int step_general()
   {
      if ( it == 2 && overstep != NULL )
         alpha = amax * atof(overstep);
      for (int attempt = 0; attempt < 8; ++attempt)
      {
         HS_HIP( hipMemsetAsync(s->flags, 0, 8 * sizeof(int), st) );
         HS_CALL( fork2(s) );
         for (auto& B : s->blk)
         {
            const int n = B.n;
            const long long n2 = (long long) n * n;
            if ( n <= 64 )
            {
               HS_CALL( hs_potrf_small_ext(st, n, B.Lx, B.dinvx, s->flags + 1, B.X, B.dX, alpha, B.Xs, B.LxInv, NULL, setf) );
               HS_CALL( hs_potrf_small_ext(st2, n, B.Lz, B.dinvz, s->flags + 0, B.Z, B.dZ, alpha, B.Zs, B.LzInv, n <= 32 ? B.Zinv : NULL, setf) );
               continue;
            }
            HS_CALL( hs_scale_add(st, n2, alpha, B.dX, 1.0, B.Xs, B.X) );
            HS_CALL( factor(st, n, B.Lx, B.dinvx, B.X, 1) );
            HS_CALL( hs_scale_add(st2, n2, alpha, B.dZ, 1.0, B.Zs, B.Z) );
            HS_CALL( factor(st2, n, B.Lz, B.dinvz, B.Z, 0) );
         }
         HS_CALL( join2(s) );
         if ( K == 0 )
            break;
         if ( optimistic )
         {
            swap_trial();
            HS_CALL( apply_step() );
            factors_valid = true;
            if ( s->use2 && !zchain_queued )
               HS_CALL( queue_z_chains() );
            if ( attempt == 0 )
            {
               rd_have = !small_problem(s);
               rd_pending = rd_have;
               rd_scale = 1.0 - alpha * eta;
            }
            HS_CALL( enqueue_residuals() );
            HS_CALL( read_back(hflags) );
            if ( hflags[0] == 0 && hflags[1] == 0 )
               break;
            swap_trial();
            factors_valid = zchain_queued = xchain_queued = false;
            rd_have = rd_pending = false;
         }
         else
         {
            if ( s->comm == NULL )
               HS_CALL( publish_and_wait(s, s->nsc, 2) );
            else
            {
               HS_CALL( hs_bcast_ints(s->comm, s->flags, 3, st) );
               HS_HIP( hipMemcpyAsync(s->hsc + s->nsc, s->flags, 4 * sizeof(int), hipMemcpyDeviceToHost, st) );
               HS_HIP( hipStreamSynchronize(st) );
            }
            memcpy(hflags, s->hsc + s->nsc, 3 * sizeof(int));
            if ( hflags[0] == 0 && hflags[1] == 0 )
               break;
         }
         alpha *= 0.5;
         info->chol_fail++;
      }
      if ( K > 0 && (hflags[0] != 0 || hflags[1] != 0) )
         return give_up(optimistic && applied != 0.0);
      if ( !optimistic )
         swap_trial();
      for (auto& B : s->blk)
         if ( B.n <= 64 )
            B.derived_valid = true;
      factors_valid = (K > 0);
      alpha_last = alpha;
      if ( optimistic && K > 0 )
      {
         residuals_ready = true;
         return HS_OK;
// ... 893 lines not shown
```

scip-sdp_amd/csrc/kernels.hip:

```cpp
#include "hs_kernels.h"
#include <string.h>
#include <stdio.h>
#include <stdlib.h>

static int hs_rec_dir_block_small(hipStream_t s, int n, double c, const double* X, const double* R, const double* E, const double* Zinv,
   double s1, double* out);
static int hs_rec_lp_dir(hipStream_t s, int q, double sigmu, double eta, const double* x, const double* z, const double* r, const double* elp,
   double* out);
static int hs_rec_vec_mul(hipStream_t s, long long n, const double* a, const double* b, double* out);
static int hs_rec_axpy3(hipStream_t s, double a, long long n1, const double* x1, double* y1, long long n2, const double* x2, double* y2,
   long long n3, const double* x3, double* y3);
static int hs_rec_gemv_t(hipStream_t s, int R, long long E, const double* A, long long lda, const double* coef, double sa, const double* add,
   double* out);

struct __attribute__((aligned(16))) dbl2 { double x, y; };
__device__ __forceinline__ dbl2 load_stream2(const double* p)
{
   typedef double gv2 __attribute__((ext_vector_type(2)));
   const gv2 t = __builtin_nontemporal_load(reinterpret_cast<const gv2*>(p));
   dbl2 r; r.x = t.x; r.y = t.y;
   return r;
}

static inline int hs_launch_ok(void)
// ... 66 lines not shown
      const int r = (int) (rc / n), c = (int) (rc - (long long) r * n);
      if ( c <= r )
         Apk[i * Lp + (long long) r * (r + 1) / 2 + c] = A[e];
   }
}

__global__ void k_packed_diag(int m1, int n, int ldd, long long Lp, const double* __restrict__ Apk, double* __restrict__ D)
{
   const long long total = (long long) m1 * ldd;
   for (long long e = (long long) blockIdx.x * blockDim.x + threadIdx.x; e < total; e += (long long) gridDim.x * blockDim.x)
   {
      const long long i = e / ldd;
      const int r = (int) (e - i * ldd);
      D[e] = r < n ? Apk[i * Lp + (long long) r * (r + 3) / 2] : 0.0;
   }
}

__global__ void k_sub_lower(int n, const double* __restrict__ S, double* __restrict__ C)
{
   const long long total = (long long) n * n;
   for (long long e = (long long) blockIdx.x * blockDim.x + threadIdx.x; e < total; e += (long long) gridDim.x * blockDim.x)
   {
      const int r = (int) (e / n), c = (int) (e - (long long) r * n);
      if ( c <= r )
         C[e] -= S[e];
   }
}

__global__ void k_pack_weighted(int n, const double* __restrict__ V, double* __restrict__ pk)
{
   const long long total = (long long) n * n;
   for (long long e = (long long) blockIdx.x * blockDim.x + threadIdx.x; e < total; e += (long long) gridDim.x * blockDim.x)
   {
      const int r = (int) (e / n), c = (int) (e - (long long) (e / n) * n);
      if ( c <= r )
         pk[(long long) r * (r + 1) / 2 + c] = (r == c ? 1.0 : 2.0) * V[e];
   }
}

__global__ void k_unpack_sym(int n, const double* __restrict__ pk, double sa, const double* __restrict__ add, double* __restrict__ out)
{
   const long long total = (long long) n * n;
   for (long long e = (long long) blockIdx.x * blockDim.x + threadIdx.x; e < total; e += (long long) gridDim.x * blockDim.x)
   {
      const int r0 = (int) (e / n), c0 = (int) (e - (long long) (e / n) * n);
      const int r = r0 > c0 ? r0 : c0, c = r0 > c0 ? c0 : r0;
      double v = pk[(long long) r * (r + 1) / 2 + c];
      if ( add != NULL )
         v += sa * add[e];
      out[e] = v;
   }
}

__global__ void k_zero_upper(double* A, int n)
{
   const long long total = (long long) n * n;
   for (long long i = (long long) blockIdx.x * blockDim.x + threadIdx.x; i < total; i += (long long) gridDim.x * blockDim.x)
   {
      const int r = (int) (i / n);
      const int c = (int) (i - (long long) r * n);
      if ( r < c )
         A[i] = 0.0;
   }
}

__global__ void k_symmetrize(double* A, int n)
{
   const long long total = (long long) n * n;
   for (long long i = (long long) blockIdx.x * blockDim.x + threadIdx.x; i < total; i += (long long) gridDim.x * blockDim.x)
   {
      const int r = (int) (i / n);
      const int c = (int) (i - (long long) r * n);
      if ( r > c )
      {
         const double v = 0.5 * (A[(long long) r * n + c] + A[(long long) c * n + r]);
         A[(long long) r * n + c] = v;
         A[(long long) c * n + r] = v;
      }
   }
}

__global__ void k_dirmat(int n, double s1, const double* __restrict__ Zinv, const double* __restrict__ X,
   const double* __restrict__ GZ, double* __restrict__ H)
{
   const long long total = (long long) n * n;
   for (long long i = (long long) blockIdx.x * blockDim.x + threadIdx.x; i < total; i += (long long) gridDim.x * blockDim.x)
   {
      const int r = (int) (i / n);
      const int c = (int) (i - (long long) r * n);
      const double g = 0.5 * (GZ[i] + GZ[(long long) c * n + r]);
      H[i] = s1 * Zinv[i] - X[i] - g;
   }
}

__global__ void k_lp_dir(int q, double sigmu, double eta, const double* __restrict__ x, const double* __restrict__ z,
   const double* __restrict__ r, const double* __restrict__ elp, double* __restrict__ out)
{
   const int i = blockIdx.x * blockDim.x + threadIdx.x;
   if ( i < q )
   {
      double t = eta * x[i] * r[i];
      if ( elp != NULL )
         t += elp[i];
      out[i] = sigmu / z[i] - x[i] - t / z[i];
   }
}
// ... 49 lines not shown

int hs_copy(hipStream_t s, double* dst, const double* src, long long n)
{
   (void) hs_red_batch_flush();
   if ( n <= 0 ) return HS_OK;
   if ( n <= (1LL << 16) )
   {
      hipLaunchKernelGGL(k_copy, dim3(grid_for(n, 256, 256)), dim3(256), 0, s, n, src, dst);
      HS_LAUNCH_CHECK();
      return HS_OK;
   }
   HS_HIP( hipMemcpyAsync(dst, src, (size_t) n * sizeof(double), hipMemcpyDeviceToDevice, s) );
   return HS_OK;
}

__global__ void k_axpy3(double a, long long n1, const double* __restrict__ x1, double* __restrict__ y1, long long n2,
   const double* __restrict__ x2, double* __restrict__ y2, long long n3, const double* __restrict__ x3, double* __restrict__ y3)
{
   const long long total = n1 + n2 + n3;
   for (long long i = (long long) blockIdx.x * blockDim.x + threadIdx.x; i < total; i += (long long) gridDim.x * blockDim.x)
   {
      if ( i < n1 )
         y1[i] += a * x1[i];
      else if ( i < n1 + n2 )
         y2[i - n1] += a * x2[i - n1];
      else
         y3[i - n1 - n2] += a * x3[i - n1 - n2];
   }
}

int hs_axpy3(hipStream_t s, double a, long long n1, const double* x1, double* y1, long long n2, const double* x2, double* y2,
   long long n3, const double* x3, double* y3)
{
   if ( n1 < 0 ) n1 = 0;
   if ( n2 < 0 ) n2 = 0;
   if ( n3 < 0 ) n3 = 0;
   if ( n1 + n2 + n3 == 0 ) return HS_OK;
   if ( hs_rec_axpy3(s, a, n1, x1, y1, n2, x2, y2, n3, x3, y3) )
      return HS_OK;
   hipLaunchKernelGGL(k_axpy3, dim3(grid_for(n1 + n2 + n3, 256, 2048)), dim3(256), 0, s, a, n1, x1, y1, n2, x2, y2, n3, x3, y3);
   HS_LAUNCH_CHECK();
   return HS_OK;
}

int hs_scale_add(hipStream_t s, long long n, double a, const double* x, double b, const double* y, double* out)
{
   (void) hs_red_batch_flush();
   if ( n <= 0 ) return HS_OK;
   hipLaunchKernelGGL(k_scale_add, dim3(grid_for(n, 256, 2048)), dim3(256), 0, s, n, a, x, b, y, out);
   HS_LAUNCH_CHECK();
   return HS_OK;
}

int hs_axpy(hipStream_t s, long long n, double a, const double* x, double* y)
{
   (void) hs_red_batch_flush();
   return hs_scale_add(s, n, a, x, 1.0, y, y);
}

int hs_mirror_lower(hipStream_t s, double* A, int n, long long lda)
{
   (void) hs_red_batch_flush();
   if ( n <= 1 ) return HS_OK;
   hipLaunchKernelGGL(k_mirror_lower, dim3(grid_for((long long) n * n, 256, 2048)), dim3(256), 0, s, A, n, lda);
   HS_LAUNCH_CHECK();
   return HS_OK;
}

int hs_mirror_upper(hipStream_t s, double* A, int n, long long lda)
{
   (void) hs_red_batch_flush();
   if ( n <= 1 ) return HS_OK;
   hipLaunchKernelGGL(k_mirror_upper, dim3(grid_for((long long) n * n, 256, 2048)), dim3(256), 0, s, A, n, lda);
   HS_LAUNCH_CHECK();
   return HS_OK;
}

int hs_pack_rows(hipStream_t s, int m1, int n, long long Lp, const double* A, double* Apk)
{
   (void) hs_red_batch_flush();
   HS_HIP( hipMemsetAsync(Apk, 0, (size_t) m1 * (size_t) Lp * sizeof(double), s) );
   hipLaunchKernelGGL(k_pack_rows, dim3(grid_for((long long) m1 * n * n, 256, 65536)), dim3(256), 0, s, m1, n, Lp, A, Apk);
   HS_LAUNCH_CHECK();
   return HS_OK;
}

int hs_packed_diag(hipStream_t s, int m1, int n, int ldd, long long Lp, const double* Apk, double* D)
{
   (void) hs_red_batch_flush();
   if ( ldd < n )
      return HS_ERR_ARG;
   hipLaunchKernelGGL(k_packed_diag, dim3(grid_for((long long) m1 * ldd, 256, 2048)), dim3(256), 0, s, m1, n, ldd, Lp, Apk, D);
   HS_LAUNCH_CHECK();
   return HS_OK;
}

int hs_sub_lower(hipStream_t s, int n, const double* S, double* C)
{
   (void) hs_red_batch_flush();
   hipLaunchKernelGGL(k_sub_lower, dim3(grid_for((long long) n * n, 256, 2048)), dim3(256), 0, s, n, S, C);
   HS_LAUNCH_CHECK();
   return HS_OK;
}

int hs_pack_weighted(hipStream_t s, int n, const double* V, double* pk)
{
   (void) hs_red_batch_flush();
   hipLaunchKernelGGL(k_pack_weighted, dim3(grid_for((long long) n * n, 256, 2048)), dim3(256), 0, s, n, V, pk);
   HS_LAUNCH_CHECK();
   return HS_OK;
}

int hs_unpack_sym(hipStream_t s, int n, const double* pk, double sa, const double* add, double* out)
{
   (void) hs_red_batch_flush();
   hipLaunchKernelGGL(k_unpack_sym, dim3(grid_for((long long) n * n, 256, 2048)), dim3(256), 0, s, n, pk, sa, add, out);
   HS_LAUNCH_CHECK();
   return HS_OK;
}

int hs_zero_upper(hipStream_t s, double* A, int n)
{
   (void) hs_red_batch_flush();
   if ( n <= 1 ) return HS_OK;
   hipLaunchKernelGGL(k_zero_upper, dim3(grid_for((long long) n * n, 256, 2048)), dim3(256), 0, s, A, n);
   HS_LAUNCH_CHECK();
   return HS_OK;
}

__global__ void __launch_bounds__(256) k_transpose(int n, const double* __restrict__ src, double* __restrict__ dst)
{
   __shared__ double tile[32][33];
   const int bx = blockIdx.x * 32, by = blockIdx.y * 32;
   const int tx = threadIdx.x & 31, ty = threadIdx.x >> 5;
   for (int r = ty; r < 32; r += 8)
      if ( by + r < n && bx + tx < n )
         tile[r][tx] = src[(long long) (by + r) * n + bx + tx];
   __syncthreads();
   for (int r = ty; r < 32; r += 8)
      if ( bx + r < n && by + tx < n )
         dst[(long long) (bx + r) * n + by + tx] = tile[tx][r];
}

int hs_transpose(hipStream_t s, int n, const double* src, double* dst)
{
   (void) hs_red_batch_flush();
   if ( n <= 0 ) return HS_OK;
   const int t = (n + 31) / 32;
   hipLaunchKernelGGL(k_transpose, dim3(t, t), dim3(256), 0, s, n, src, dst);
   HS_LAUNCH_CHECK();
   return HS_OK;
}

int hs_symmetrize(hipStream_t s, double* A, int n)
{
   (void) hs_red_batch_flush();
   if ( n <= 1 ) return HS_OK;
   hipLaunchKernelGGL(k_symmetrize, dim3(grid_for((long long) n * n, 256, 2048)), dim3(256), 0, s, A, n);
   HS_LAUNCH_CHECK();
   return HS_OK;
}

#include "hs_lds_product.h"

__device__ void d_dir_block_small(int n, double c, const double* __restrict__ X, const double* __restrict__ R,
   const double* __restrict__ E, const double* __restrict__ Zinv, double s1, double* __restrict__ out, double* db_smem)
{
   const int ld = n + 1;
   double* sx = db_smem;
// ... 74 lines not shown
            sr[r * ld + cc] = rv[u];
            sz[r * ld + cc] = zv[u];
         }
      }
   }
   __syncthreads();
   db_product(n, ld, sx, sr, [&](int i, int j, int r, int cc, double acc)
   {
      double g = acc * c;
      if ( E != NULL )
         g = __dadd_rn(g, ev[i][j]);
      sg[r * ld + cc] = g;
   });
   __syncthreads();
   db_product(n, ld, sg, sz, [&](int, int, int r, int cc, double acc) { sr[r * ld + cc] = acc; });
   __syncthreads();
   for (int e = tid; e < n2; e += 256)
   {
      const int r = e / n, cc = e - r * n;
      out[e] = s1 * sz[r * ld + cc] - sx[r * ld + cc] - 0.5 * (sr[r * ld + cc] + sr[cc * ld + r]);
   }
}

__global__ void __launch_bounds__(256) k_dir_block_small(int n, double c, const double* __restrict__ X, const double* __restrict__ R,
   const double* __restrict__ E, const double* __restrict__ Zinv, double s1, double* __restrict__ out)
{
   extern __shared__ double db_smem_k[];
   d_dir_block_small(n, c, X, R, E, Zinv, s1, out, db_smem_k);
}

int hs_dir_block_small(hipStream_t s, int n, double c, const double* X, const double* R, const double* E, const double* Zinv,
   double s1, double* out)
{
   if ( n <= 0 ) return HS_OK;
   if ( n > HS_SMALL_N ) return HS_ERR_ARG;
   if ( hs_rec_dir_block_small(s, n, c, X, R, E, Zinv, s1, out) )
      return HS_OK;
   static hs_attr_mask attr_done;
   HS_CALL( hs_func_max_lds(reinterpret_cast<const void*>(&k_dir_block_small), 4 * HS_SMALL_N * (HS_SMALL_N + 1) * (int) sizeof(double), &attr_done) );
   hipLaunchKernelGGL(k_dir_block_small, dim3(1), dim3(256), (size_t) 4 * n * (n + 1) * sizeof(double), s, n, c, X, R, E, Zinv, s1, out);
   HS_LAUNCH_CHECK();
   return HS_OK;
}

int hs_dirmat(hipStream_t s, int n, double s1, const double* Zinv, const double* X, const double* GZ, double* H)
{
   (void) hs_red_batch_flush();
   if ( n <= 0 ) return HS_OK;
   hipLaunchKernelGGL(k_dirmat, dim3(grid_for((long long) n * n, 256, 2048)), dim3(256), 0, s, n, s1, Zinv, X, GZ, H);
   HS_LAUNCH_CHECK();
   return HS_OK;
}

int hs_lp_dir(hipStream_t s, int q, double sigmu, double eta, const double* x, const double* z, const double* r,
   const double* elp, double* out)
{
   if ( q <= 0 ) return HS_OK;
   if ( hs_rec_lp_dir(s, q, sigmu, eta, x, z, r, elp, out) )
      return HS_OK;
   hipLaunchKernelGGL(k_lp_dir, dim3((q + 255) / 256), dim3(256), 0, s, q, sigmu, eta, x, z, r, elp, out);
   HS_LAUNCH_CHECK();
   return HS_OK;
}

int hs_lp_scale_rows(hipStream_t s, int q, int cols, const double* x, const double* z, const double* D, double* S)
{
   (void) hs_red_batch_flush();
   if ( q <= 0 ) return HS_OK;
   hipLaunchKernelGGL(k_lp_scale_rows, dim3(grid_for((long long) q * cols, 256, 2048)), dim3(256), 0, s, q, cols, x, z, D, S);
   HS_LAUNCH_CHECK();
   return HS_OK;
}

int hs_vec_mul(hipStream_t s, long long n, const double* a, const double* b, double* out)
{
   if ( n <= 0 ) return HS_OK;
   if ( hs_rec_vec_mul(s, n, a, b, out) )
      return HS_OK;
   hipLaunchKernelGGL(k_vec_mul, dim3(grid_for(n, 256, 2048)), dim3(256), 0, s, n, a, b, out);
   HS_LAUNCH_CHECK();
   return HS_OK;
}


struct OpSum { __device__ static double id() { return 0.0; } __device__ static double f(double a, double b) { return a + b; } };
struct OpMax { __device__ static double id() { return 0.0; } __device__ static double f(double a, double b) { return a > b ? a : b; } };
struct OpMin { __device__ static double id() { return 1e300; } __device__ static double f(double a, double b) { return a < b ? a : b; } };

template<class OP>
__device__ __forceinline__ double wave_reduce(double v)
{
#pragma unroll
   for (int off = 32; off > 0; off >>= 1)
      v = OP::f(v, __shfl_down(v, off, 64));
   return v;
}

template<class OP>
__device__ __forceinline__ double block_reduce_256(double v, double* sh)
{
   v = wave_reduce<OP>(v);
   const int lane = threadIdx.x & 63;
   const int wave = threadIdx.x >> 6;
   if ( lane == 0 )
      sh[wave] = v;
   __syncthreads();
// ... 27 lines not shown
      return a[i] * b[i];
   if ( KIND == RED_ABSMAX )
      return fabs(a[i]);
   if ( KIND == RED_RATIOMIN )
   {
      const double d = b[i];
      return d < 0.0 ? -a[i] / d : 1e300;
   }
   return (a[i] / b[i]) * c[i] * c[i];
}

template<int KIND>
__global__ void __launch_bounds__(256) k_reduce_stage1(long long n, const double* __restrict__ a, const double* __restrict__ b,
   const double* __restrict__ c, double* __restrict__ part, double* __restrict__ out, int accumulate, int direct)
{
   typedef typename RedTraits<KIND>::OP OP;
   __shared__ double sh[4];
   double v = OP::id();
   for (long long i = (long long) blockIdx.x * blockDim.x + threadIdx.x; i < n; i += (long long) gridDim.x * blockDim.x)
      v = OP::f(v, red_elem<KIND>(i, a, b, c));
   v = block_reduce_256<OP>(v, sh);
   if ( threadIdx.x == 0 )
   {
      if ( direct )
         *out = accumulate ? OP::f(*out, v) : v;
      else
         part[blockIdx.x] = v;
   }
}

template<int KIND>
__global__ void __launch_bounds__(256) k_reduce_stage2(int nparts, const double* __restrict__ part, double* __restrict__ out,
   int accumulate)
{
   typedef typename RedTraits<KIND>::OP OP;
   __shared__ double sh[4];
   double v = OP::id();
   for (int i = threadIdx.x; i < nparts; i += blockDim.x)
      v = OP::f(v, part[i]);
   v = block_reduce_256<OP>(v, sh);
   if ( threadIdx.x == 0 )
      *out = accumulate ? OP::f(*out, v) : v;
}

#define RB_MAX   24
#define RB_MAXN  16384
#define RB_ROWS  64
#define RB_MATS  32
#define RB_MAXWORK 16384
#define RB_FILL  100
#define RB_COPY1 101
#define RB_SOLVE 102
#define RB_FINISH 103
#define RB_DIRBLK  110
#define RB_LPDIR   111
#define RB_VECMUL  112
#define RB_AXPY3   113
#define RB_MAKEEXT 114
#define RB_GEMVT   115
#define RB_LPROWS  116
#define RB_APPLYA  117

struct rb_desc { int kind; int accumulate; int i[6]; double d[4]; const void* p[10]; };
struct rb_finish { int m; double eta, rg, sigmu, tau, kappa, etk; const double* u1; const double* u2; double* dy; double* dyt; double* sc;
   int s0, bub, bh, wrp, bu1, dtau, dkappa, den; };
struct rb_args { int cnt; rb_desc d[RB_MAX]; rb_finish fin; int pub_n; const double* pub_src; double* pub_dst;
   unsigned long long pub_seq; unsigned long long* pub_flag;
   unsigned long long* dbg; };
static_assert(sizeof(rb_args) <= 4096, "the records travel as kernel arguments");
static thread_local struct { bool open; hipStream_t s; int hold; size_t smem; rb_args args; } g_rb = {false, NULL, 0, 0, {0, {}}};

template<int KIND>
__device__ __forceinline__ double rb_run(const rb_desc& D, double* sh)
{
   typedef typename RedTraits<KIND>::OP OP;
   double v = OP::id();
   const double* a = (const double*) D.p[0];
   const double* b = (const double*) D.p[1];
   const double* c = (const double*) D.p[2];
   double* out = (double*) D.p[3];
   for (long long i = threadIdx.x; i < D.i[0]; i += 256)
      v = OP::f(v, red_elem<KIND>(i, a, b, c));
   v = block_reduce_256<OP>(v, sh);
   if ( threadIdx.x == 0 )
      *out = D.accumulate ? OP::f(*out, v) : v;
   return v;
}

__device__ __forceinline__ double d_tree64(double (&p)[64])
{
#pragma unroll
   for (int off = 32; off > 0; off >>= 1)
#pragma unroll
      for (int l = 0; l < off; ++l)
         p[l] += p[l + off];
   return p[0];
}

template<int KIND>
__device__ __forceinline__ void rb_run_wave(const rb_desc& D)
{
   typedef typename RedTraits<KIND>::OP OP;
   const double* a = (const double*) D.p[0];
   const double* b = (const double*) D.p[1];
   const double* c = (const double*) D.p[2];
   double* out = (double*) D.p[3];
// ... 22 lines not shown
{
   extern __shared__ double rb_dyn[];
   __shared__ double sh[4];
   for (int t = 0; t < A.cnt; ++t)
   {
      {
         int g = 0;
         while ( g < 4 && t + g < A.cnt && A.d[t + g].kind <= RED_LPS0 && A.d[t + g].i[0] <= 1024 )
         {
            bool fresh = true;
            for (int h = 0; h < g; ++h)
               fresh = fresh && A.d[t + h].p[3] != A.d[t + g].p[3];
            if ( !fresh )
               break;
            ++g;
         }
         if ( g > 1 )
         {
            const unsigned long long tg_begin = (A.dbg != NULL) ? wall_clock64() : 0ULL;
            const int w = threadIdx.x >> 6;
            if ( w < g )
            {
               const rb_desc& G = A.d[t + w];
               switch ( G.kind )
               {
               case RED_DOT:      rb_run_wave<RED_DOT>(G); break;
               case RED_ABSMAX:   rb_run_wave<RED_ABSMAX>(G); break;
               case RED_RATIOMIN: rb_run_wave<RED_RATIOMIN>(G); break;
               default:           rb_run_wave<RED_LPS0>(G); break;
               }
            }
            __threadfence_block();
            __syncthreads();
            if ( A.dbg != NULL && threadIdx.x == 0 )
            {
               atomicAdd(A.dbg + 2 * 8, wall_clock64() - tg_begin);
               atomicAdd(A.dbg + 2 * 8 + 1, 1ULL);
            }
            t += g - 1;
            continue;
         }
      }
      const rb_desc& D = A.d[t];
      const unsigned long long t_begin = (A.dbg != NULL) ? wall_clock64() : 0ULL;
      const unsigned long long c_begin = (A.dbg != NULL) ? clock64() : 0ULL;
      switch ( D.kind )
      {
      case RED_DOT:      rb_run<RED_DOT>(D, sh); break;
      case RED_ABSMAX:   rb_run<RED_ABSMAX>(D, sh); break;
      case RED_RATIOMIN: rb_run<RED_RATIOMIN>(D, sh); break;
      case RED_LPS0:     rb_run<RED_LPS0>(D, sh); break;
      case RB_FILL:      if ( threadIdx.x == 0 ) *(double*) D.p[3] = D.d[0]; break;
      case RB_COPY1:     if ( threadIdx.x == 0 ) *(double*) D.p[3] = *(const double*) D.p[0]; break;
      case RB_DIRBLK:
         d_dir_block_small(D.i[0], D.d[0], (const double*) D.p[0], (const double*) D.p[1], (const double*) D.p[2], (const double*) D.p[3],
            D.d[1], (double*) D.p[4], rb_dyn);
         break;
      case RB_LPDIR:
      {
         const double* x = (const double*) D.p[0]; const double* z = (const double*) D.p[1]; const double* r = (const double*) D.p[2];
         const double* elp = (const double*) D.p[3]; double* out = (double*) D.p[4];
         const double sigmu = D.d[0], eta = D.d[1];
         for (int i = threadIdx.x; i < D.i[0]; i += 256)
         {
            double t = eta * x[i] * r[i];
            if ( elp != NULL )
               t += elp[i];
            out[i] = sigmu / z[i] - x[i] - t / z[i];
         }
         break;
      }
      case RB_VECMUL:
      {
         const double* a = (const double*) D.p[0]; const double* b = (const double*) D.p[1]; double* out = (double*) D.p[2];
         for (int i = threadIdx.x; i < D.i[0]; i += 256)
            out[i] = a[i] * b[i];
         break;
      }
      case RB_AXPY3:
      {
         const double a = D.d[0];
         for (int v = 0; v < 3; ++v)
         {
            const double* x = (const double*) D.p[2 * v]; double* y = (double*) D.p[2 * v + 1];
            for (int i = threadIdx.x; i < D.i[v]; i += 256)
               y[i] += a * x[i];
         }
         break;
      }
      case RB_MAKEEXT:
      {
         const double* v = (const double*) D.p[0]; double* ext = (double*) D.p[1];
         if ( threadIdx.x == 0 )
            ext[0] = D.d[0];
         for (int i = threadIdx.x; i < D.i[0]; i += 256)
            ext[1 + i] = D.d[1] * v[i];
         break;
      }
      case RB_GEMVT:
      {
         const double* Am = (const double*) D.p[0]; const double* coef = (const double*) D.p[1]; const double* add = (const double*) D.p[2];
         double* out = (double*) D.p[3];
         const int R = D.i[0], E = D.i[1];
         const long long lda = D.i[2];
         const double sa = D.d[0];
         for (int e = threadIdx.x; e < E; e += 256)
// ... 752 lines not shown
   {
      rb_desc* D = rb_record_ext(s, RB_APPLYA, (size_t) RB_MATS * 4 * 65 * sizeof(double));
      if ( D != NULL )
      {
         D->i[0] = m1; D->i[1] = B->nblk; D->i[2] = B->n2[0]; D->i[3] = B->nblk > 1 ? B->n2[1] : 0; D->i[4] = q; D->i[5] = epi;
         D->d[0] = scal;
         D->p[0] = B->A[0]; D->p[1] = B->V[0]; D->p[2] = B->nblk > 1 ? B->A[1] : NULL; D->p[3] = B->nblk > 1 ? B->V[1] : NULL;
         D->p[4] = Dext; D->p[5] = vlp; D->p[6] = out; D->p[7] = vin; D->p[8] = vout;
         return HS_OK;
      }
   }
   else
      (void) rb_decline();
   hipLaunchKernelGGL(k_apply_A_small, dim3(m1), dim3(256), 0, s, m1, *B, q, Dext, vlp, out, epi, scal, vin, vout);
   HS_LAUNCH_CHECK();
   return HS_OK;
}

template<int KIND>
static int reduce_launch(hipStream_t s, long long n, const double* a, const double* b, const double* c, double* out,
   int accumulate, double* ws)
{
   if ( n > 0 && rb_record(s, KIND, n, a, b, c, out, accumulate, 0.0) )
      return HS_OK;
   if ( n <= 0 )
   {
      if ( !accumulate )
      {
         const double idv = (KIND == RED_RATIOMIN) ? 1e300 : 0.0;
         HS_CALL( hs_fill_scalar(s, out, idv) );
      }
      return HS_OK;
   }
   const int g = grid_for(n, 2048, 256);
   (void) hs_red_batch_flush();
   if ( g == 1 )
   {
      hipLaunchKernelGGL((k_reduce_stage1<KIND>), dim3(1), dim3(256), 0, s, n, a, b, c, ws, out, accumulate, 1);
      HS_LAUNCH_CHECK();
      return HS_OK;
   }
   hipLaunchKernelGGL((k_reduce_stage1<KIND>), dim3(g), dim3(256), 0, s, n, a, b, c, ws, out, accumulate, 0);
   HS_LAUNCH_CHECK();
   hipLaunchKernelGGL((k_reduce_stage2<KIND>), dim3(1), dim3(256), 0, s, g, ws, out, accumulate);
   HS_LAUNCH_CHECK();
   return HS_OK;
}

int hs_dot(hipStream_t s, long long n, const double* a, const double* b, double* out, int accumulate, double* ws)
{
   return reduce_launch<RED_DOT>(s, n, a, b, NULL, out, accumulate, ws);
}

int hs_absmax(hipStream_t s, long long n, const double* a, double* out, int accumulate, double* ws)
{
   return reduce_launch<RED_ABSMAX>(s, n, a, NULL, NULL, out, accumulate, ws);
}

int hs_ratio_min(hipStream_t s, long long n, const double* x, const double* d, double* out, int accumulate, double* ws)
{
   return reduce_launch<RED_RATIOMIN>(s, n, x, d, NULL, out, accumulate, ws);
}

int hs_lp_s0(hipStream_t s, int q, const double* x, const double* z, const double* beta, double* out, int accumulate, double* ws)
{
   return reduce_launch<RED_LPS0>(s, q, x, z, beta, out, accumulate, ws);
}


struct gemvn_vecs { const double* v[4]; };

template<int NV, bool VEC>
__global__ void __launch_bounds__(256) k_gemv_n(int R, long long E, const double* __restrict__ A, long long lda,
   gemvn_vecs V, double* __restrict__ out, long long ldo, int nsplit, long long chunk)
{
   __shared__ double sh[4];
   const int row = blockIdx.x;
   const int sp = blockIdx.y;
   const long long e0 = sp * chunk;
   long long e1 = e0 + chunk;
   if ( e1 > E ) e1 = E;
   const double* a = A + (long long) row * lda;
   double acc[NV];
#pragma unroll
   for (int v = 0; v < NV; ++v)
      acc[v] = 0.0;

   if ( VEC )
   {
      long long e = e0 + 2 * threadIdx.x;
      for (; e + 1 < e1; e += 512)
      {
         const dbl2 x = *reinterpret_cast<const dbl2*>(a + e);
#pragma unroll
         for (int v = 0; v < NV; ++v)
         {
            const dbl2 w = *reinterpret_cast<const dbl2*>(V.v[v] + e);
            acc[v] += x.x * w.x;
            acc[v] += x.y * w.y;
         }
      }
      if ( ((e1 - e0) & 1) && threadIdx.x == 0 )
      {
#pragma unroll
         for (int v = 0; v < NV; ++v)
            acc[v] += a[e1 - 1] * V.v[v][e1 - 1];
// ... 394 lines not shown
```

scip-sdp_amd/csrc/units.hip:

```cpp
#include "hs_kernels.h"
#include "hs_gram_cache.h"
#include "../../include/hipsdp.h"
#include "../../include/hipsdp_units.h"
#include <vector>
#include <cstring>
#include <cstdlib>

namespace {

struct DevBuf
{
   double* p;
   DevBuf() : p(NULL) {}
   ~DevBuf() { if ( p ) (void) hipFree(p); }
   int alloc(long long n) { if ( n <= 0 ) n = 1; hipError_t e = hipMalloc((void**) &p, (size_t) n * sizeof(double)); if ( e != hipSuccess ) { hs_record_hip_error(e, "hipMalloc", __FILE__, __LINE__); return e == hipErrorOutOfMemory ? HS_ERR_NOMEM : HS_ERR_HIP; } return HS_OK; }
   int up(const double* h, long long n) { if ( n <= 0 ) return HS_OK; hipError_t e = hipMemcpy(p, h, (size_t) n * sizeof(double), hipMemcpyHostToDevice); if ( e != hipSuccess ) { hs_record_hip_error(e, "H2D", __FILE__, __LINE__); return HS_ERR_HIP; } return HS_OK; }
   int down(double* h, long long n) { if ( n <= 0 ) return HS_OK; hipError_t e = hipMemcpy(h, p, (size_t) n * sizeof(double), hipMemcpyDeviceToHost); if ( e != hipSuccess ) { hs_record_hip_error(e, "D2H", __FILE__, __LINE__); return HS_ERR_HIP; } return HS_OK; }
};

int pick_device(int device)
{
   int nd = 0;
   if ( hipGetDeviceCount(&nd) != hipSuccess || nd <= 0 )
      return HIPSDP_ERR_NODEVICE;
// ... 624 lines not shown
      for (int i = 0; i < n; ++i) regmask[i] = psd ? hint[1 + i] : 0;
   return gaveup == 0 ? HIPSDP_OK : HIPSDP_ERR_NUMERIC;
}

extern "C" int hipsdp_potrf_small_unit(int device, int n, int pair, const double* base, const double* dir, double alpha, int set_flag,
   int want_gram, double* L, double* dinv, double* Mout, double* Linv, double* Gram, int* flag)
{
   if ( n < 1 || n > 64 || (pair != 0 && pair != 1) || base == NULL || L == NULL || dinv == NULL || flag == NULL
         || (set_flag != 0 && set_flag != 1) || (want_gram != 0 && want_gram != 1) || (want_gram && (n > 32 || Gram == NULL)) )
      return HIPSDP_ERR_ARG;
   HS_CALL( pick_device(device) );
   const int np = pair ? 2 : 1;
   const long long n2 = (long long) n * n;
   DevBuf dB, dR, dL, dD, dM, dI, dG;
   int* dflag = NULL;
   HS_CALL( dB.alloc(np * n2) ); HS_CALL( dR.alloc(np * n2) ); HS_CALL( dL.alloc(np * n2) ); HS_CALL( dD.alloc(np * 4096) );
   HS_CALL( dM.alloc(np * n2) ); HS_CALL( dI.alloc(np * n2) ); HS_CALL( dG.alloc(np * n2) );
   HS_HIP( hipMalloc((void**) &dflag, 2 * sizeof(int)) );
   HS_HIP( hipMemset(dflag, 0, 2 * sizeof(int)) );
   HS_HIP( hipMemset(dL.p, 0xFF, (size_t) (np * n2) * sizeof(double)) ); HS_HIP( hipMemset(dD.p, 0xFF, (size_t) (np * 4096) * sizeof(double)) );
   HS_HIP( hipMemset(dM.p, 0xFF, (size_t) (np * n2) * sizeof(double)) ); HS_HIP( hipMemset(dI.p, 0xFF, (size_t) (np * n2) * sizeof(double)) );
   HS_HIP( hipMemset(dG.p, 0xFF, (size_t) (np * n2) * sizeof(double)) );
   HS_CALL( dB.up(base, np * n2) );
   if ( dir != NULL ) HS_CALL( dR.up(dir, np * n2) );
   int rc;
   if ( !pair )
      rc = hs_potrf_small_ext(0, n, dL.p, dD.p, dflag, dB.p, dir != NULL ? dR.p : NULL, alpha, Mout != NULL ? dM.p : NULL,
         Linv != NULL ? dI.p : NULL, want_gram ? dG.p : NULL, set_flag);
   else
   {
      double* pL[2] = {dL.p, dL.p + n2};
      double* pD[2] = {dD.p, dD.p + 4096};
      int* pF[2] = {dflag, dflag + 1};
      const double* pB[2] = {dB.p, dB.p + n2};
      const double* pR[2] = {dir != NULL ? dR.p : NULL, dir != NULL ? dR.p + n2 : NULL};
      double* pM[2] = {Mout != NULL ? dM.p : NULL, Mout != NULL ? dM.p + n2 : NULL};
      double* pI[2] = {Linv != NULL ? dI.p : NULL, Linv != NULL ? dI.p + n2 : NULL};
      double* pG[2] = {want_gram ? dG.p : NULL, want_gram ? dG.p + n2 : NULL};
      rc = hs_potrf_small_ext_pair(0, n, pL, pD, pF, pB, pR, alpha, pM, pI, pG, set_flag);
   }
   if ( rc == HS_OK && hipDeviceSynchronize() != hipSuccess ) rc = HS_ERR_HIP;
   int hflag[2] = {0, 0};
   if ( rc == HS_OK && hipMemcpy(hflag, dflag, 2 * sizeof(int), hipMemcpyDeviceToHost) != hipSuccess ) rc = HS_ERR_HIP;
   (void) hipFree(dflag);
   HS_CALL( rc );
   HS_CALL( dL.down(L, np * n2) ); HS_CALL( dD.down(dinv, np * 4096) );
   if ( Mout != NULL ) HS_CALL( dM.down(Mout, np * n2) );
   if ( Linv != NULL ) HS_CALL( dI.down(Linv, np * n2) );
   if ( want_gram ) HS_CALL( dG.down(Gram, np * n2) );
   for (int k = 0; k < np; ++k) flag[k] = hflag[k];
   return HIPSDP_OK;
}

extern "C" int hipsdp_trtri(int device, int n, const double* A, double* Linv)
{
   HS_CALL( pick_device(device) );
   const long long n2 = (long long) n * n;
   DevBuf dA, dD, dL, dT;
   int* dflag = NULL;
   HS_CALL( dA.alloc(n2) ); HS_CALL( dD.alloc(hs_potrf_dinv_len(n)) ); HS_CALL( dL.alloc(n2) ); HS_CALL( dT.alloc(n2) );
   HS_HIP( hipMalloc((void**) &dflag, sizeof(int)) );
   HS_HIP( hipMemset(dflag, 0, sizeof(int)) );
   HS_CALL( dA.up(A, n2) );
   int rc = hs_potrf(0, n, dA.p, dD.p, dflag, NULL);
   if ( rc == HS_OK ) rc = hs_trtri(0, n, dA.p, dD.p, dL.p, dT.p);
   if ( rc == HS_OK && hipDeviceSynchronize() != hipSuccess ) rc = HS_ERR_HIP;
   int hflag = 0;
   if ( rc == HS_OK && hipMemcpy(&hflag, dflag, sizeof(int), hipMemcpyDeviceToHost) != hipSuccess ) rc = HS_ERR_HIP;
   (void) hipFree(dflag);
   HS_CALL( rc );
   HS_CALL( dL.down(Linv, n2) );
   return hflag == 0 ? HIPSDP_OK : HIPSDP_ERR_NUMERIC;
}

extern "C" int hipsdp_lambda_min(int device, int n, const double* W, int steps, double* theta, double* resid)
{
   HS_CALL( pick_device(device) );
   if ( n <= 0 ) return HIPSDP_ERR_ARG;
   if ( steps <= 0 ) steps = n < 250 ? n : 250;
   if ( steps > 250 ) steps = 250;
   const long long n2 = (long long) n * n;
   DevBuf dW, dR, dS;
   HS_CALL( dW.alloc(n2) ); HS_CALL( dR.alloc(8) ); HS_CALL( dS.alloc(hs_lanczos_ws(n, steps)) );
   HS_CALL( dW.up(W, n2) );
   HS_CALL( hs_lanczos_lmin(0, n, dW.p, steps, dR.p, dS.p) );
   HS_HIP( hipDeviceSynchronize() );
   double h[3];
   HS_CALL( dR.down(h, 3) );
   *theta = h[0];
   if ( resid != NULL ) *resid = h[1];
   return HIPSDP_OK;
}

extern "C" int hipsdp_lambda_min_scaled(int device, int n, const double* L, const double* D, int steps, double* theta, double* resid)
{
   HS_CALL( pick_device(device) );
   if ( n <= 0 || n > 64 || theta == NULL ) return HIPSDP_ERR_ARG;
   const long long n2 = (long long) n * n;
   DevBuf dL, dD, dR;
   HS_CALL( dL.alloc(n2) ); HS_CALL( dD.alloc(n2) ); HS_CALL( dR.alloc(16) );
   HS_CALL( dL.up(L, n2) ); HS_CALL( dD.up(D, n2) );
   DevBuf dR2;
   HS_CALL( dR2.alloc(16) );
   hs_step_jobs J;
   J.nblk = 2;
   for (int j = 0; j < 2; ++j)
// ... 261 lines not shown
```

Before: 13.35.

## Fuse IPM direction tail kernels and batch paired Cholesky and trial-step launches

Adds fused device paths for the per-iteration IPM tail. Paired Cholesky factorizations run in one launch per panel step via blockIdx.y. Deferred dot reductions get separate workspace slots so they can be batched and finished in one kernel. Dirmat is fused with packing, three symmetric unpacks are fused, unpack is combined with the dZ update, and post-solve vector updates are merged into one kernel. The aim is fewer small kernel launches and synchronisation points per iteration, at the cost of more code paths and a larger reduction workspace.

```diff
diff --git a/include/hipsdp_units.h b/include/hipsdp_units.h
--- a/include/hipsdp_units.h
+++ b/include/hipsdp_units.h
@@ -35,6 +35,20 @@
    int* regmask, int* fail);
 HIPSDP_API int  hipsdp_potrf_small_unit(int device, int n, int pair, const double* base, const double* dir, double alpha, int set_flag,
    int want_gram, double* L, double* dinv, double* Mout, double* Linv, double* Gram, int* flag);
+HIPSDP_API long long hipsdp_potrf_dinv_len(int n);
+HIPSDP_API int  hipsdp_potrf_pair_unit(int device, int n, int pair, double* A, double* dinv, int* fail);
+HIPSDP_API int  hipsdp_trial_pair_unit(int device, int n, int fused, int first, double alpha, double* io);
+HIPSDP_API int  hipsdp_tail_after_solve2_unit(int device, int m, int fused, const double* rhs2, const double* u1, double* u2, double* wt,
+   double* e2, double* e1);
+HIPSDP_API int  hipsdp_tail_unpack3_unit(int device, int n, int fused, const double* pk, double* out);
+HIPSDP_API int  hipsdp_tail_dz_unit(int device, int n, int fused, const double* pk, const double* P2, const double* Rd, double dtau, double eta,
+   double* dZ);
+HIPSDP_API int  hipsdp_tail_dirmat_unit(int device, int n, int fused, double s1, const double* Zinv, const double* X, const double* GZ, double* H,
+   double* pk);
+HIPSDP_API int  hipsdp_tail_sc_len(void);
+HIPSDP_API int  hipsdp_tail_dir_unit(int device, int m, int n, int fused, const double* B, const double* H, const double* rhs2, const double* rp,
+   const double* b, const double* u1, const double* u2, const double* par, double* sc, double* dy, double* dyt);
+HIPSDP_API int  hipsdp_tail_dots_unit(int device, int m, int n, int fused, const double* a, const double* v, double* out);
 HIPSDP_API int  hipsdp_trtri(int device, int n, const double* A, double* Linv);
 HIPSDP_API int  hipsdp_lambda_min(int device, int n, const double* W, int steps, double* theta, double* resid);
 HIPSDP_API int  hipsdp_lambda_min_scaled(int device, int n, const double* L, const double* D, int steps, double* theta, double* resid);
diff --git a/scip-sdp_amd/binding.py b/scip-sdp_amd/binding.py
--- a/scip-sdp_amd/binding.py
+++ b/scip-sdp_amd/binding.py
@@ -495,6 +495,94 @@
     return out
 
 
+def potrf_pair_unit(A2, pair=True, device=0):
+    L = _f64(A2).copy()
+    n = L.shape[-1]
+    assert L.shape == (2, n, n)
+    ulib().hipsdp_potrf_dinv_len.restype = C.c_longlong
+    nd = int(ulib().hipsdp_potrf_dinv_len(n))
+    dinv = np.zeros((2, nd))
+    fail = np.zeros(2, dtype=np.int32)
+    _chk(ulib().hipsdp_potrf_pair_unit(device, n, int(pair), _dp(L), _dp(dinv), _ip(fail)), "hipsdp_potrf_pair_unit")
+    return L, dinv, fail
+
+
+def trial_pair_unit(arrays, alpha, fused=True, first=True, device=0):
+    io = _f64(arrays).copy()
+    n = io.shape[-1]
+    assert io.shape == (8, n, n)
+    _chk(ulib().hipsdp_trial_pair_unit(device, n, int(fused), int(first), C.c_double(alpha), _dp(io)), "hipsdp_trial_pair_unit")
+    return io
+
+
+def _packed_len(n):
+    t = n * (n + 1) // 2
+    return t + (t & 1)
+
+
+def tail_after_solve2_unit(rhs2, u1, fused, device=0):
+    rhs2, u1 = _f64(rhs2), _f64(u1)
+    m = u1.size
+    assert rhs2.size == 2 * m
+    u2, wt, e2, e1 = np.zeros(m), np.zeros(m + 1), np.zeros(m + 1), np.zeros(m + 1)
+    _chk(ulib().hipsdp_tail_after_solve2_unit(device, m, int(fused), _dp(rhs2), _dp(u1), _dp(u2), _dp(wt), _dp(e2), _dp(e1)),
+         "hipsdp_tail_after_solve2_unit")
+    return u2, wt, e2, e1
+
+
+def tail_unpack3_unit(pk, n, fused, device=0):
+    pk = _f64(pk)
+    assert pk.shape == (3, _packed_len(n))
+    out = np.zeros((3, n, n))
+    _chk(ulib().hipsdp_tail_unpack3_unit(device, n, int(fused), _dp(pk), _dp(out)), "hipsdp_tail_unpack3_unit")
+    return out
+
+
+def tail_dz_unit(pk, P2, Rd, dtau, eta, fused, device=0):
+    pk, P2, Rd = _f64(pk), _f64(P2), _f64(Rd)
+    n = P2.shape[0]
+    assert pk.size == _packed_len(n) and P2.shape == Rd.shape == (n, n)
+    dZ = np.zeros((n, n))
+    _chk(ulib().hipsdp_tail_dz_unit(device, n, int(fused), _dp(pk), _dp(P2), _dp(Rd), C.c_double(dtau), C.c_double(eta), _dp(dZ)),
+         "hipsdp_tail_dz_unit")
+    return dZ
+
+
+def tail_dirmat_unit(s1, Zinv, X, GZ, fused, device=0):
+    Zinv, X, GZ = _f64(Zinv), _f64(X), _f64(GZ)
+    n = X.shape[0]
+    H, pk = np.zeros((n, n)), np.zeros(_packed_len(n))
+    _chk(ulib().hipsdp_tail_dirmat_unit(device, n, int(fused), C.c_double(s1), _dp(Zinv), _dp(X), _dp(GZ), _dp(H), _dp(pk)),
+         "hipsdp_tail_dirmat_unit")
+    return H, pk
+
+
+def tail_dir_unit(B, H, rhs2, rp, b, u1, u2, par, sc, fused, device=0):
+    B, H = _f64(B), _f64(H)
+    vs = [_f64(v) for v in (rhs2, rp, b, u1, u2)]
+    m, n = vs[0].size, B.shape[0]
+    par = _f64(par)
+    sc = _f64(sc).copy()
+    assert par.size == 6 and sc.size == ulib().hipsdp_tail_sc_len() and all(v.size == m for v in vs) and B.shape == H.shape == (n, n)
+    dy, dyt = np.zeros(m), np.zeros(m + 1)
+    _chk(ulib().hipsdp_tail_dir_unit(device, m, n, int(fused), _dp(B), _dp(H), _dp(vs[0]), _dp(vs[1]), _dp(vs[2]), _dp(vs[3]), _dp(vs[4]),
+                                     _dp(par), _dp(sc), _dp(dy), _dp(dyt)), "hipsdp_tail_dir_unit")
+    return sc, dy, dyt
+
+
+def tail_sc_len():
+    return int(ulib().hipsdp_tail_sc_len())
+
+
+def tail_dots_unit(a, v, fused, device=0):
+    a, v = _f64(a), _f64(v)
+    n = int(round(np.sqrt(a.shape[1])))
+    assert a.shape == (3, n * n) and v.shape[0] == 2
+    out = np.zeros(3)
+    _chk(ulib().hipsdp_tail_dots_unit(device, v.shape[1], n, int(fused), _dp(a), _dp(v), _dp(out)), "hipsdp_tail_dots_unit")
+    return out
+
+
 def trtri(A, device=0):
     A = _f64(A)
     Li = np.zeros_like(A)
diff --git a/scip-sdp_amd/csrc/chol.hip b/scip-sdp_amd/csrc/chol.hip
--- a/scip-sdp_amd/csrc/chol.hip
+++ b/scip-sdp_amd/csrc/chol.hip
@@ -525,8 +525,8 @@
 }
 
 template<int NBK>
-__global__ void __launch_bounds__(256) k_potrf_step(double* __restrict__ A, long long lda, int n, int kb, int nblk,
-   double* __restrict__ dinv, int* __restrict__ flag, const double* __restrict__ diag0, double regtol, pd_ext ext)
+__device__ __forceinline__ void ps_step_body(double* __restrict__ A, long long lda, int n, int kb, int nblk,
+   double* __restrict__ dinv, int* __restrict__ flag, const double* __restrict__ diag0, double regtol, const pd_ext& ext)
 {
    extern __shared__ __attribute__((aligned(16))) double pd_smem[];
    double* lstage = dinv + (long long) nblk * NB * NB;
@@ -689,6 +689,34 @@
 }
 
 template<int NBK>
+__global__ void __launch_bounds__(256) k_potrf_step(double* __restrict__ A, long long lda, int n, int kb, int nblk,
+   double* __restrict__ dinv, int* __restrict__ flag, const double* __restrict__ diag0, double regtol, pd_ext ext)
+{
+   ps_step_body<NBK>(A, lda, n, kb, nblk, dinv, flag, diag0, regtol, ext);
+}
+
+struct ps_job { double* A; double* dinv; int* flag; };
+template<int NBK>
+__global__ void __launch_bounds__(256) k_potrf_step_pair(ps_job J0, ps_job J1, long long lda, int n, int kb, int nblk, pd_ext ext)
+{
+   const ps_job J = blockIdx.y ? J1 : J0;
+   ps_step_body<NBK>(J.A, lda, n, kb, nblk, J.dinv, J.flag, NULL, 1e-13, ext);
+}
+
+template<int NBK>
+static int launch_potrf_step_pair(hipStream_t s, const ps_job* J, long long lda, int n, int kb, int nblk, const pd_ext& ext)
+{
+   static hs_attr_mask attr_done;
+   HS_CALL( hs_func_max_lds(reinterpret_cast<const void*>(&k_potrf_step_pair<NBK>), PD_SMEM_BYTES, &attr_done) );
+   const int nS = nblk - kb;
+   const int t = nblk - kb - 1;
+   const int nT = kb > 0 ? t * (t + 1) / 2 : 0;
+   hipLaunchKernelGGL((k_potrf_step_pair<NBK>), dim3(nS + nT, 2), dim3(256), PD_SMEM_BYTES, s, J[0], J[1], lda, n, kb, nblk, ext);
+   HS_LAUNCH_CHECK();
+   return HS_OK;
+}
+
+template<int NBK>
 static int launch_potrf_step(hipStream_t s, double* A, long long lda, int n, int kb, int nblk, double* dinv, int* flag,
    const double* diag0, const pd_ext& ext)
 {
@@ -787,6 +815,33 @@
 int hs_potrf(hipStream_t s, int n, double* A, double* dinv, int* flag, const double* diag0)
 {
    return hs_potrf_psd(s, n, A, dinv, flag, diag0, NULL, 0);
+}
+
+int hs_potrf_pair(hipStream_t s, int n, const hs_potrf_job* jobs)
+{
+   if ( n <= 0 )
+      return HS_OK;
+   if ( jobs == NULL || jobs[0].A == NULL || jobs[1].A == NULL || jobs[0].A == jobs[1].A || jobs[0].dinv == jobs[1].dinv )
+      return HS_ERR_ARG;
+   const int nblk = (n + NB - 1) / NB;
+   if ( nblk <= 1 || g_potrf_force_v1 )
+   {
+      HS_CALL( hs_potrf(s, n, jobs[0].A, jobs[0].dinv, jobs[0].flag, NULL) );
+      return hs_potrf(s, n, jobs[1].A, jobs[1].dinv, jobs[1].flag, NULL);
+   }
+   const ps_job J[2] = {{jobs[0].A, jobs[0].dinv, jobs[0].flag}, {jobs[1].A, jobs[1].dinv, jobs[1].flag}};
+   const pd_ext est = {NULL, NULL, 0.0, NULL, NULL, NULL, 0, 3, NULL, 0, 0, NULL};
+   for (int b = 0; b < nblk; ++b)
+   {
+      const int nb = (n - b * NB) < NB ? (n - b * NB) : NB;
+      if ( nb <= 16 )
+         HS_CALL( launch_potrf_step_pair<16>(s, J, n, n, b, nblk, est) );
+      else if ( nb <= 32 )
+         HS_CALL( launch_potrf_step_pair<32>(s, J, n, n, b, nblk, est) );
+      else
+         HS_CALL( launch_potrf_step_pair<64>(s, J, n, n, b, nblk, est) );
+   }
+   return HS_OK;
 }
 
 int hs_potrf_psd(hipStream_t s, int n, double* A, double* dinv, int* flag, const double* diag0, int* regmask, int set_flag)
diff --git a/scip-sdp_amd/csrc/hs_kernels.h b/scip-sdp_amd/csrc/hs_kernels.h
--- a/scip-sdp_amd/csrc/hs_kernels.h
+++ b/scip-sdp_amd/csrc/hs_kernels.h
@@ -8,6 +8,8 @@
 int hs_copy(hipStream_t s, double* dst, const double* src, long long n);
 int hs_axpy(hipStream_t s, long long n, double a, const double* x, double* y);
 int hs_scale_add(hipStream_t s, long long n, double a, const double* x, double b, const double* y, double* out);
+struct hs_trial_job { double* V; const double* dV; double* Vs; double* L; };
+int hs_trial_pair(hipStream_t s, long long n, double alpha, int first, const hs_trial_job* jobs);
 int hs_mirror_lower(hipStream_t s, double* A, int n, long long lda);
 int hs_symmetrize(hipStream_t s, double* A, int n);
 int hs_transpose(hipStream_t s, int n, const double* src, double* dst);
@@ -47,6 +49,10 @@
 int hs_axpy3(hipStream_t s, double a, long long n1, const double* x1, double* y1, long long n2, const double* x2, double* y2,
    long long n3, const double* x3, double* y3);
 int hs_dot(hipStream_t s, long long n, const double* a, const double* b, double* out, int accumulate, double* ws);
+#define HS_DOT_SLOT_DOUBLES 256
+#define HS_DOT_SLOTS 4
+#define HS_RED_WS_DOUBLES (HS_DOT_SLOTS * HS_DOT_SLOT_DOUBLES)
+int hs_dot_deferred(hipStream_t s, long long n, const double* a, const double* b, double* out, int accumulate, double* ws, int slot);
 int hs_absmax(hipStream_t s, long long n, const double* a, double* out, int accumulate, double* ws);
 int hs_ratio_min(hipStream_t s, long long n, const double* x, const double* d, double* out, int accumulate, double* ws);
 
@@ -54,6 +60,7 @@
 int hs_dir_block_small(hipStream_t s, int n, double c, const double* X, const double* R, const double* E, const double* Zinv,
    double s1, double* out);
 int hs_dirmat(hipStream_t s, int n, double s1, const double* Zinv, const double* X, const double* GZ, double* H);
+int hs_dirmat_pack(hipStream_t s, int n, double s1, const double* Zinv, const double* X, const double* GZ, double* H, double* pk);
 
 int hs_lp_dir(hipStream_t s, int q, double sigmu, double eta, const double* x, const double* z, const double* rd_or_dz,
    const double* elp, double* out);
@@ -66,6 +73,9 @@
 int hs_sub_lower(hipStream_t s, int n, const double* S, double* C);
 int hs_pack_weighted(hipStream_t s, int n, const double* V, double* pk);
 int hs_unpack_sym(hipStream_t s, int n, const double* pk, double sa, const double* add, double* out);
+int hs_unpack_sym3(hipStream_t s, int n, int cnt, const double* const* pk, double* const* out);
+int hs_unpack_dz_combine(hipStream_t s, int n, const double* pk, const double* P2, const double* sc, int idtau, double eta, const double* Rd,
+   double* dZ);
 int hs_zero_upper(hipStream_t s, double* A, int n);
 
 struct hs_schur_ws
@@ -127,9 +137,20 @@
 int  hs_sp_schur(hipStream_t s, const hs_sparse* sp, const double* X, const double* Zinv, double* Mx);
 int  hs_sp_expand(hipStream_t s, const hs_sparse* sp, double* A);
 
+struct hs_dir_tail_args { int m, q, K; const int* n; const double* const* B; const double* const* H; const double* beta; const double* hl;
+   const double* rhs2; const double* rp; const double* b; double* u1; const double* u2; double* dy; double* dyt; double* sc; double* red_ws;
+   const double* dinvm; const double* Lm; double eta, rg, sigmu, tau, kappa, etk; };
+int hs_ipm_dir_tail(hipStream_t st, const hs_dir_tail_args* a, int tail, int fuse_solve);
+int hs_ipm_after_solve2(hipStream_t st, int m, const double* rhs2, double* u2, double* wt, const double* u1, double* e2, double* e1, int fused);
+int hs_ipm_dz_combine(hipStream_t st, long long n2, double* dZ, const double* P2, const double* sc, double eta, const double* Rd);
+int hs_ipm_sc_dtau(void);
+int hs_ipm_sc_len(int nblocks);
+
 int hs_potrf(hipStream_t s, int n, double* A, double* dinv, int* flag, const double* diag0);
 long long hs_potrf_dinv_len(int n);
 int hs_potrf_psd(hipStream_t s, int n, double* A, double* dinv, int* flag, const double* diag0, int* regmask, int set_flag);
+struct hs_potrf_job { double* A; double* dinv; int* flag; };
+int hs_potrf_pair(hipStream_t s, int n, const hs_potrf_job* jobs);
 int hs_trtri(hipStream_t s, int n, const double* L, const double* dinv, double* Linv, double* tmp);
 int hs_potrf_small_ext_pair(hipStream_t s, int n, double* const* L, double* const* dinv, int* const* flag, const double* const* base,
    const double* const* dir, double alpha, double* const* Mout, double* const* Linv, double* const* Gram, int set_flag);
diff --git a/scip-sdp_amd/csrc/ipm.hip b/scip-sdp_amd/csrc/ipm.hip
--- a/scip-sdp_amd/csrc/ipm.hip
+++ b/scip-sdp_amd/csrc/ipm.hip
@@ -823,7 +823,7 @@
       HS_HIP( hipHostGetDevicePointer((void**) &s->hsc_dev, s->hsc, 0) );
       memset(s->hsc, 0, (size_t) s->hsc_cap * sizeof(double));
    }
-   HS_CALL( dalloc(&s->red_ws, 1024) );
+   HS_CALL( dalloc(&s->red_ws, HS_RED_WS_DOUBLES) );
    s->gemv_ws_len = 8192 + 4LL * 1024 * 4;
    HS_CALL( dalloc(&s->gemv_ws, s->gemv_ws_len) );
    {
@@ -1303,7 +1303,7 @@
 
 int hs_gen_dense(hipStream_t s, int n, int i0, int i1, long long seed, double* A);
 static int ensure_packed(hipsdp_solver* s);
-static int pass_A(hipsdp_solver* s, Block& B, const double* V, double* out);
+static int pass_A(hipsdp_solver* s, Block& B, const double* V, double* out, bool packed = false);
 static int pass_AT(hipsdp_solver* s, Block& B, const double* coef, double sa, const double* add, double* out);
 
 extern "C" int hipsdp_gen_planted(hipsdp_solver* s, int n, int m, long long seed, const double* Xstar, const double* Zstar,
@@ -1457,6 +1457,26 @@
    {
       u2[i] = rhs2[m + i] - rhs2[i];
       wt[1 + i] = -rhs2[i];
+   }
+}
+
+__global__ void k_after_solve2_ext(int m, const double* __restrict__ rhs2, double* __restrict__ u2, double* __restrict__ wt,
+   double s20, double s21, double* __restrict__ e2, double s10, double s11, const double* __restrict__ u1, double* __restrict__ e1)
+{
+   const int i = blockIdx.x * blockDim.x + threadIdx.x;
+   if ( i == 0 )
+   {
+      wt[0] = 1.0;
+      e2[0] = s20;
+      e1[0] = s10;
+   }
+   if ( i < m )
+   {
+      const double v = rhs2[m + i] - rhs2[i];
+      u2[i] = v;
+      wt[1 + i] = -rhs2[i];
+      e2[1 + i] = s21 * v;
+      e1[1 + i] = s11 * u1[i];
    }
 }
 
@@ -1599,6 +1619,72 @@
 }
 
 static inline dim3 g1d(long long n) { long long g = (n + 255) / 256; if ( g < 1 ) g = 1; if ( g > 4096 ) g = 4096; return dim3((unsigned) g); }
+
+int hs_ipm_dir_tail(hipStream_t st, const hs_dir_tail_args* a, int tail, int fuse_solve)
+{
+   const int m = a->m;
+   hs_red_batch_begin(st);
+   if ( fuse_solve )
+      (void) hs_red_batch_solve(st, m, a->dinvm, a->Lm, 1, a->u1, m);
+   HS_CALL( hs_fill_scalar(st, a->sc + SC_BH, 0.0) );
+   for (int k = 0; k < a->K; ++k)
+   {
+      const long long n2 = (long long) a->n[k] * a->n[k];
+      if ( tail )
+         HS_CALL( hs_dot_deferred(st, n2, a->B[k], a->H[k], a->sc + SC_BH, 1, a->red_ws, k) );
+      else
+         HS_CALL( hs_dot(st, n2, a->B[k], a->H[k], a->sc + SC_BH, 1, a->red_ws) );
+   }
+   if ( a->q > 0 )
+      HS_CALL( hs_dot(st, a->q, a->beta, a->hl, a->sc + SC_BH, 1, a->red_ws) );
+   HS_CALL( hs_dot(st, m, a->rhs2, a->rp, a->sc + SC_WRP, 0, a->red_ws) );
+   HS_CALL( hs_dot(st, m, a->b, a->u1, a->sc + SC_BU1, 0, a->red_ws) );
+   bool finished = false;
+   if ( fuse_solve || tail )
+   {
+      hs_rb_finish F = {m, a->eta, a->rg, a->sigmu, a->tau, a->kappa, a->etk, a->u1, a->u2, a->dy, a->dyt, a->sc,
+         SC_S0, SC_BUB, SC_BH, SC_WRP, SC_BU1, SC_DTAU, SC_DKAPPA, SC_DEN};
+      finished = hs_red_batch_finish(st, &F, sizeof(F)) == 1;
+   }
+   HS_CALL( hs_red_batch_end() );
+   if ( !finished )
+   {
+      HS_CALL( hs_red_batch_flush() );
+      hipLaunchKernelGGL(k_finish_dir, g1d(m > 0 ? m : 1), dim3(256), 0, st, m, a->eta, a->rg, a->sigmu, a->tau, a->kappa, a->etk,
+         a->u1, a->u2, a->dy, a->dyt, a->sc);
+      HS_LAUNCH_CHECK();
+   }
+   return HS_OK;
+}
+
+int hs_ipm_after_solve2(hipStream_t st, int m, const double* rhs2, double* u2, double* wt, const double* u1, double* e2, double* e1, int fused)
+{
+   if ( fused && e2 != NULL )
+   {
+      hipLaunchKernelGGL(k_after_solve2_ext, g1d(m + 1), dim3(256), 0, st, m, rhs2, u2, wt, 1.0, 1.0, e2, 0.0, 1.0, u1, e1);
+      HS_LAUNCH_CHECK();
+      return HS_OK;
+   }
+   hipLaunchKernelGGL(k_after_solve2, g1d(m + 1), dim3(256), 0, st, m, rhs2, u2, wt);
+   HS_LAUNCH_CHECK();
+   if ( e2 != NULL )
+   {
+      HS_CALL( hs_make_ext(st, m, 1.0, 1.0, u2, e2) );
+      HS_CALL( hs_make_ext(st, m, 0.0, 1.0, u1, e1) );
+   }
+   return HS_OK;
+}
+
+int hs_ipm_dz_combine(hipStream_t st, long long n2, double* dZ, const double* P2, const double* sc, double eta, const double* Rd)
+{
+   HS_CALL( hs_red_batch_flush() );
+   hipLaunchKernelGGL(k_dz_combine, g1d(n2), dim3(256), 0, st, n2, dZ, P2, sc, eta, Rd);
+   HS_LAUNCH_CHECK();
+   return HS_OK;
+}
+
+int hs_ipm_sc_dtau(void) { return SC_DTAU; }
+int hs_ipm_sc_len(int nblocks) { return SC_FIXED_END + 8 * (nblocks > 0 ? nblocks : 1) + 8; }
 
 static int gemm_on(hipStream_t st, int layA, int layB, int M, int N, int K, double alpha, const double* A, long long lda,
    const double* B, long long ldb, double beta, double* C, long long ldc, int flags = 0)
@@ -1910,7 +1996,7 @@
       Mx[(long long) i * m1] += v[i];
 }
 
-static int pass_A(hipsdp_solver* s, Block& B, const double* V, double* out)
+static int pass_A(hipsdp_solver* s, Block& B, const double* V, double* out, bool packed)
 {
    const int m1 = s->m + 1;
    if ( B.sparse )
@@ -1945,7 +2031,8 @@
    }
    if ( B.Apk != NULL )
    {
-      HS_CALL( hs_pack_weighted(s->stream, B.n, V, B.pkv) );
+      if ( !packed )
+         HS_CALL( hs_pack_weighted(s->stream, B.n, V, B.pkv) );
       const double* v = B.pkv;
       return hs_gemv_n(s->stream, m1, B.Lp, B.Apk, B.Lp, 1, &v, out, m1, s->gemv_ws, s->gemv_ws_len);
    }
@@ -2024,6 +2111,21 @@
    int close() { if ( !on ) return HS_OK; on = false; return hs_red_batch_release(); }
    ~BatchRegion() { if ( on ) (void) hs_red_batch_release(); }
 };
+
+static bool general_tail(const hipsdp_solver* s)
+{
+   if ( s->comm != NULL || s->m <= 64 || s->blk.empty() || batch_regions(s) )
+      return false;
+   for (auto& B : s->blk)
+      if ( B.n <= 64 )
+         return false;
+   return true;
+}
+
+static bool pack_with_dirmat(const hipsdp_solver* s, const Block& B)
+{
+   return general_tail(s) && B.Apk != NULL && !B.sparse;
+}
 
 static int apply_A_small(hipsdp_solver* s, double* const* Vk, const double* vlp, double* out, int epi, double scal,
    const double* vin, double* vout)
@@ -2051,7 +2153,7 @@
    return 1;
 }
 
-static int apply_A(hipsdp_solver* s, double* const* Vk, const double* vlp, double* out)
+static int apply_A(hipsdp_solver* s, double* const* Vk, const double* vlp, double* out, bool packed = false)
 {
    const int m1 = s->m + 1;
    bool first = true;
@@ -2060,7 +2162,7 @@
       Block& B = s->blk[k];
       const double* v = Vk[k];
       double* dst = first ? out : s->tmpe;
-      HS_CALL( pass_A(s, B, v, dst) );
+      HS_CALL( pass_A(s, B, v, dst, packed && pack_with_dirmat(s, B)) );
       if ( !first )
          HS_CALL( hs_axpy(s->stream, m1, 1.0, s->tmpe, out) );
       first = false;
@@ -2103,7 +2205,10 @@
             HS_CALL( hs_copy(s->stream, B.G, B.E, n2) );
          HS_CALL( gemm(s, HS_KC, HS_MC, n, n, n, eta, B.X, n, B.Rd, n, useE ? 1.0 : 0.0, B.G, n) );
          HS_CALL( gemm(s, HS_KC, HS_MC, n, n, n, 1.0, B.G, n, B.Zinv, n, 0.0, B.GZ, n) );
-         HS_CALL( hs_dirmat(s->stream, n, sigmu, B.Zinv, B.X, B.GZ, B.H) );
+         if ( pack_with_dirmat(s, B) )
+            HS_CALL( hs_dirmat_pack(s->stream, n, sigmu, B.Zinv, B.X, B.GZ, B.H, B.pkv) );
+         else
+            HS_CALL( hs_dirmat(s->stream, n, sigmu, B.Zinv, B.X, B.GZ, B.H) );
       }
       Hs.push_back(B.H);
    }
@@ -2113,7 +2218,7 @@
    if ( fusedA < 0 )
       return -fusedA;
    if ( fusedA == 0 )
-      HS_CALL( apply_A(s, Hs.data(), s->hl, s->AH) );
+      HS_CALL( apply_A(s, Hs.data(), s->hl, s->AH, true) );
    if ( fusedA == 0 && m > 0 )
    {
       HS_CALL( hs_red_batch_flush() );
@@ -2129,30 +2234,16 @@
       HS_CALL( hs_red_batch_flush() );
       HS_CALL( hs_trsv_sync(s->stream, m, s->Lm, s->dinvm, 1, s->u1, m, SOLVE_MODE, s->trsv_ws, &s->trsv_epoch) );
    }
-   hs_red_batch_begin(s->stream);
-   if ( fuse_solve )
-      (void) hs_red_batch_solve(s->stream, m, s->dinvm, s->Lm, 1, s->u1, m);
-   HS_CALL( hs_fill_scalar(s->stream, s->sc + SC_BH, 0.0) );
-   for (auto& B : s->blk)
-      HS_CALL( hs_dot(s->stream, (long long) B.n * B.n, B.B, B.H, s->sc + SC_BH, 1, s->red_ws) );
-   if ( q > 0 )
-      HS_CALL( hs_dot(s->stream, q, s->beta, s->hl, s->sc + SC_BH, 1, s->red_ws) );
-   HS_CALL( hs_dot(s->stream, m, s->rhs2, s->rp, s->sc + SC_WRP, 0, s->red_ws) );
-   HS_CALL( hs_dot(s->stream, m, s->b, s->u1, s->sc + SC_BU1, 0, s->red_ws) );
-   bool finished = false;
-   if ( fuse_solve )
-   {
-      hs_rb_finish F = {m, eta, rg, sigmu, s->tau, s->kappa, etk, s->u1, s->u2, s->dy, s->dyt, s->sc,
-         SC_S0, SC_BUB, SC_BH, SC_WRP, SC_BU1, SC_DTAU, SC_DKAPPA, SC_DEN};
-      finished = hs_red_batch_finish(s->stream, &F, sizeof(F)) == 1;
-   }
-   HS_CALL( hs_red_batch_end() );
-   if ( !finished )
-   {
-      HS_CALL( hs_red_batch_flush() );
-      hipLaunchKernelGGL(k_finish_dir, g1d(m > 0 ? m : 1), dim3(256), 0, s->stream, m, eta, rg, sigmu, s->tau, s->kappa, etk,
-         s->u1, s->u2, s->dy, s->dyt, s->sc);
-      HS_LAUNCH_CHECK();
+   {
+      std::vector<int> bn;
+      std::vector<const double*> bB, bH;
+      for (auto& B : s->blk)
+      {
+         bn.push_back(B.n); bB.push_back(B.B); bH.push_back(B.H);
+      }
+      const hs_dir_tail_args ta = {m, q, (int) s->blk.size(), bn.data(), bB.data(), bH.data(), s->beta, s->hl, s->rhs2, s->rp, s->b, s->u1, s->u2,
+         s->dy, s->dyt, s->sc, s->red_ws, s->dinvm, s->Lm, eta, rg, sigmu, s->tau, s->kappa, etk};
+      HS_CALL( hs_ipm_dir_tail(s->stream, &ta, general_tail(s) ? 1 : 0, fuse_solve ? 1 : 0) );
    }
    for (auto& B : s->blk)
    {
@@ -2162,6 +2253,7 @@
          HS_CALL( pass_AT(s, B, s->dyt, eta, B.Rd, B.dZ) );
       else
       {
+         bool combined = false;
          if ( split == 1 )
          {
             if ( &B == &s->blk[0] )
@@ -2169,11 +2261,17 @@
                HS_CALL( hs_make_ext(s->stream, m, 0.0, 1.0, s->u1, s->cvec + m1) );
                HS_LAUNCH_CHECK();
             }
-            HS_CALL( pass_AT(s, B, s->cvec + m1, 0.0, NULL, B.dZ) );
-         }
-         HS_CALL( hs_red_batch_flush() );
-         hipLaunchKernelGGL(k_dz_combine, g1d(n2), dim3(256), 0, s->stream, n2, B.dZ, B.P2, s->sc, eta, B.Rd);
-         HS_LAUNCH_CHECK();
+            if ( pack_with_dirmat(s, B) )
+            {
+               HS_CALL( hs_gemv_t_ws(s->stream, m1, B.Lp, B.Apk, B.Lp, s->cvec + m1, 0.0, NULL, B.pkv + B.Lp, s->gemvt_ws, s->gemvt_ws_len) );
+               HS_CALL( hs_unpack_dz_combine(s->stream, n, B.pkv + B.Lp, B.P2, s->sc, SC_DTAU, eta, B.Rd, B.dZ) );
+               combined = true;
+            }
+            else
+               HS_CALL( pass_AT(s, B, s->cvec + m1, 0.0, NULL, B.dZ) );
+         }
+         if ( !combined )
+            HS_CALL( hs_ipm_dz_combine(s->stream, n2, B.dZ, B.P2, s->sc, eta, B.Rd) );
       }
       if ( n <= HS_SMALL_N )
          HS_CALL( hs_dir_block_small(s->stream, n, 1.0, B.X, B.dZ, useE ? B.E : NULL, B.Zinv, sigmu, B.dX) );
@@ -2963,6 +3061,7 @@
    int enqueue_residuals()
    {
       const bool recur = rd_have && !want_cert;
+      const bool tail = general_tail(s);
       HS_CALL( hs_make_ext(st, m, -s->tau, 1.0, s->y, s->yt) );
       HS_LAUNCH_CHECK();
       hs_red_batch_begin(st);
@@ -2978,8 +3077,16 @@
             HS_CALL( pass_AT(s, B, s->yt, -1.0, B.Z, B.Rd) );
          else if ( rd_pending )
             HS_CALL( hs_scale_add(st, n2, rd_scale, B.Rd, 0.0, NULL, B.Rd) );
-         HS_CALL( hs_dot(st, n2, B.Rd, B.Rd, s->sc + SC_BLK(k, 0), 0, s->red_ws) );
-         HS_CALL( hs_dot(st, n2, B.X, B.Z, s->sc + SC_XZ, 1, s->red_ws) );
+         if ( tail && !want_cert )
+         {
+            HS_CALL( hs_dot_deferred(st, n2, B.Rd, B.Rd, s->sc + SC_BLK(k, 0), 0, s->red_ws, 2 * k) );
+            HS_CALL( hs_dot_deferred(st, n2, B.X, B.Z, s->sc + SC_XZ, 1, s->red_ws, 2 * k + 1) );
+         }
+         else
+         {
+            HS_CALL( hs_dot(st, n2, B.Rd, B.Rd, s->sc + SC_BLK(k, 0), 0, s->red_ws) );
+            HS_CALL( hs_dot(st, n2, B.X, B.Z, s->sc + SC_XZ, 1, s->red_ws) );
+         }
          if ( want_cert )
          {
             HS_CALL( hs_red_batch_flush() );
@@ -3478,23 +3585,22 @@
                HS_CALL( hs_trsv_sync(st, m, s->Lm, s->dinvm, 2, s->rhs2, m, SOLVE_MODE, s->trsv_ws, &s->trsv_epoch) );
          }
       }
-      if ( m == 0 || m > 64 )
-      {
-         hipLaunchKernelGGL(k_after_solve2, g1d(m1), dim3(256), 0, st, m, s->rhs2, s->u2, s->wt);
-         HS_LAUNCH_CHECK();
-      }
-      hs_red_batch_begin(st);
-      HS_CALL( hs_fill_scalar(st, s->sc + SC_S0, 0.0) );
       split_dz = predH_joined && s->comm == NULL;
       for (auto& B : s->blk)
          if ( B.Apk == NULL )
             split_dz = false;
-      if ( split_dz )
+      const bool tail = general_tail(s);
+      if ( m == 0 || m > 64 )
+         HS_CALL( hs_ipm_after_solve2(st, m, s->rhs2, s->u2, s->wt, s->u1, (split_dz && tail) ? s->cvec : NULL, s->cvec + m1, 1) );
+      hs_red_batch_begin(st);
+      HS_CALL( hs_fill_scalar(st, s->sc + SC_S0, 0.0) );
+      if ( split_dz && !tail )
       {
          HS_CALL( hs_make_ext(st, m, 1.0, 1.0, s->u2, s->cvec) );
          HS_CALL( hs_make_ext(st, m, 0.0, 1.0, s->u1, s->cvec + m1) );
          HS_LAUNCH_CHECK();
       }
+      int slot = 0;
       for (auto& B : s->blk)
       {
          const int n = B.n;
@@ -3512,9 +3618,18 @@
                return -r3;
             if ( r3 == 1 )
             {
-               HS_CALL( hs_unpack_sym(st, n, B.pk3, 0.0, NULL, B.B) );
-               HS_CALL( hs_unpack_sym(st, n, B.pk3 + B.Lp, 0.0, NULL, B.P2) );
-               HS_CALL( hs_unpack_sym(st, n, B.pk3 + 2 * B.Lp, 0.0, NULL, B.dZ) );
+               if ( tail )
+               {
+                  const double* pk[3] = {B.pk3, B.pk3 + B.Lp, B.pk3 + 2 * B.Lp};
+                  double* un[3] = {B.B, B.P2, B.dZ};
+                  HS_CALL( hs_unpack_sym3(st, n, 3, pk, un) );
+               }
+               else
+               {
+                  HS_CALL( hs_unpack_sym(st, n, B.pk3, 0.0, NULL, B.B) );
+                  HS_CALL( hs_unpack_sym(st, n, B.pk3 + B.Lp, 0.0, NULL, B.P2) );
+                  HS_CALL( hs_unpack_sym(st, n, B.pk3 + 2 * B.Lp, 0.0, NULL, B.dZ) );
+               }
                swept = true;
             }
             else
@@ -3527,7 +3642,10 @@
             HS_CALL( pass_AT(s, B, s->wt, 0.0, NULL, B.B) );
          HS_CALL( gemm(s, HS_KC, HS_MC, n, n, n, 1.0, B.X, n, B.B, n, 0.0, B.T1, n) );
          HS_CALL( gemm(s, HS_KC, HS_MC, n, n, n, 1.0, B.T1, n, B.Zinv, n, 0.0, B.W, n) );
-         HS_CALL( hs_dot(st, n2, B.B, B.W, s->sc + SC_S0, 1, s->red_ws) );
+         if ( tail )
+            HS_CALL( hs_dot_deferred(st, n2, B.B, B.W, s->sc + SC_S0, 1, s->red_ws, slot++) );
+         else
+            HS_CALL( hs_dot(st, n2, B.B, B.W, s->sc + SC_S0, 1, s->red_ws) );
       }
       if ( q > 0 )
       {
@@ -3605,14 +3723,6 @@
    int update()
    {
       phase_mark(s, PH_UPDATE);
-      for (auto& B : s->blk)
-      {
-         const long long n2 = (long long) B.n * B.n;
-         if ( B.n <= 64 )
-            continue;
-         HS_CALL( hs_copy(st, B.Xs, B.X, n2) );
-         HS_CALL( hs_copy(st, B.Zs, B.Z, n2) );
-      }
       tau0 = s->tau;
       kappa0 = s->kappa;
       applied = 0.0;
@@ -3666,23 +3776,33 @@
       for (int attempt = 0; attempt < 8; ++attempt)
       {
          HS_HIP( hipMemsetAsync(s->flags, 0, 8 * sizeof(int), st) );
-         HS_CALL( fork2(s) );
+         bool large = false, small = false;
          for (auto& B : s->blk)
-         {
-            const int n = B.n;
-            const long long n2 = (long long) n * n;
-            if ( n <= 64 )
+            (B.n > 64 ? large : small) = true;
+         if ( large && s->busy2 )
+            HS_CALL( join2(s) );
+         for (auto& B : s->blk)
+         {
+            if ( B.n <= 64 )
+               continue;
+            const hs_trial_job tj[2] = {{B.X, B.dX, B.Xs, B.Lx}, {B.Z, B.dZ, B.Zs, B.Lz}};
+            HS_CALL( hs_trial_pair(st, (long long) B.n * B.n, alpha, attempt == 0 ? 1 : 0, tj) );
+            const hs_potrf_job pj[2] = {{B.Lx, B.dinvx, s->flags + 1}, {B.Lz, B.dinvz, s->flags + 0}};
+            HS_CALL( hs_potrf_pair(st, B.n, pj) );
+         }
+         if ( small )
+         {
+            HS_CALL( fork2(s) );
+            for (auto& B : s->blk)
             {
+               const int n = B.n;
+               if ( n > 64 )
+                  continue;
                HS_CALL( hs_potrf_small_ext(st, n, B.Lx, B.dinvx, s->flags + 1, B.X, B.dX, alpha, B.Xs, B.LxInv, NULL, setf) );
                HS_CALL( hs_potrf_small_ext(st2, n, B.Lz, B.dinvz, s->flags + 0, B.Z, B.dZ, alpha, B.Zs, B.LzInv, n <= 32 ? B.Zinv : NULL, setf) );
-               continue;
             }
-            HS_CALL( hs_scale_add(st, n2, alpha, B.dX, 1.0, B.Xs, B.X) );
-            HS_CALL( factor(st, n, B.Lx, B.dinvx, B.X, 1) );
-            HS_CALL( hs_scale_add(st2, n2, alpha, B.dZ, 1.0, B.Zs, B.Z) );
-            HS_CALL( factor(st2, n, B.Lz, B.dinvz, B.Z, 0) );
-         }
-         HS_CALL( join2(s) );
+            HS_CALL( join2(s) );
+         }
          if ( K == 0 )
             break;
          if ( optimistic )
diff --git a/scip-sdp_amd/csrc/kernels.hip b/scip-sdp_amd/csrc/kernels.hip
--- a/scip-sdp_amd/csrc/kernels.hip
+++ b/scip-sdp_amd/csrc/kernels.hip
@@ -142,6 +142,50 @@
    }
 }
 
+struct unpack3_args { const double* pk[3]; double* out[3]; };
+__global__ void k_unpack_sym3(int n, unpack3_args U)
+{
+   const double* __restrict__ pk = U.pk[blockIdx.y];
+   double* __restrict__ out = U.out[blockIdx.y];
+   const long long total = (long long) n * n;
+   for (long long e = (long long) blockIdx.x * blockDim.x + threadIdx.x; e < total; e += (long long) gridDim.x * blockDim.x)
+   {
+      const int r0 = (int) (e / n), c0 = (int) (e - (long long) (e / n) * n);
+      const int r = r0 > c0 ? r0 : c0, c = r0 > c0 ? c0 : r0;
+      out[e] = pk[(long long) r * (r + 1) / 2 + c];
+   }
+}
+
+__global__ void k_unpack_dz_combine(int n, const double* __restrict__ pk, const double* __restrict__ P2, const double* __restrict__ sc, int idtau,
+   double eta, const double* __restrict__ Rd, double* __restrict__ dZ)
+{
+   const double dtau = sc[idtau];
+   const long long total = (long long) n * n;
+   for (long long e = (long long) blockIdx.x * blockDim.x + threadIdx.x; e < total; e += (long long) gridDim.x * blockDim.x)
+   {
+      const int r0 = (int) (e / n), c0 = (int) (e - (long long) (e / n) * n);
+      const int r = r0 > c0 ? r0 : c0, c = r0 > c0 ? c0 : r0;
+      const double p1 = pk[(long long) r * (r + 1) / 2 + c];
+      dZ[e] = (p1 - dtau * P2[e]) + eta * Rd[e];
+   }
+}
+
+__global__ void k_dirmat_pack(int n, double s1, const double* __restrict__ Zinv, const double* __restrict__ X,
+   const double* __restrict__ GZ, double* __restrict__ H, double* __restrict__ pk)
+{
+   const long long total = (long long) n * n;
+   for (long long i = (long long) blockIdx.x * blockDim.x + threadIdx.x; i < total; i += (long long) gridDim.x * blockDim.x)
+   {
+      const int r = (int) (i / n);
+      const int c = (int) (i - (long long) r * n);
+      const double g = 0.5 * (GZ[i] + GZ[(long long) c * n + r]);
+      const double h = s1 * Zinv[i] - X[i] - g;
+      H[i] = h;
+      if ( c <= r )
+         pk[(long long) r * (r + 1) / 2 + c] = (r == c ? 1.0 : 2.0) * h;
+   }
+}
+
 __global__ void k_zero_upper(double* A, int n)
 {
    const long long total = (long long) n * n;
@@ -297,6 +341,31 @@
    return HS_OK;
 }
 
+__global__ void k_trial_pair(long long n, double a, double b, int first, hs_trial_job J0, hs_trial_job J1)
+{
+   const hs_trial_job J = blockIdx.y ? J1 : J0;
+   const double* base = first ? J.V : J.Vs;
+   for (long long i = (long long) blockIdx.x * blockDim.x + threadIdx.x; i < n; i += (long long) gridDim.x * blockDim.x)
+   {
+      const double y = base[i];
+      double v = a * J.dV[i];
+      v += b * y;
+      if ( first )
+         J.Vs[i] = y;
+      J.V[i] = v;
+      J.L[i] = v;
+   }
+}
+
+int hs_trial_pair(hipStream_t s, long long n, double alpha, int first, const hs_trial_job* jobs)
+{
+   (void) hs_red_batch_flush();
+   if ( n <= 0 ) return HS_OK;
+   hipLaunchKernelGGL(k_trial_pair, dim3(grid_for(n, 256, 2048), 2), dim3(256), 0, s, n, alpha, 1.0, first, jobs[0], jobs[1]);
+   HS_LAUNCH_CHECK();
+   return HS_OK;
+}
+
 int hs_axpy(hipStream_t s, long long n, double a, const double* x, double* y)
 {
    (void) hs_red_batch_flush();
@@ -360,6 +429,30 @@
 {
    (void) hs_red_batch_flush();
    hipLaunchKernelGGL(k_unpack_sym, dim3(grid_for((long long) n * n, 256, 2048)), dim3(256), 0, s, n, pk, sa, add, out);
+   HS_LAUNCH_CHECK();
+   return HS_OK;
+}
+
+int hs_unpack_sym3(hipStream_t s, int n, int cnt, const double* const* pk, double* const* out)
+{
+   (void) hs_red_batch_flush();
+   if ( cnt < 1 || cnt > 3 )
+      return HS_ERR_ARG;
+   unpack3_args U = {{NULL, NULL, NULL}, {NULL, NULL, NULL}};
+   for (int k = 0; k < cnt; ++k)
+   {
+      U.pk[k] = pk[k]; U.out[k] = out[k];
+   }
+   hipLaunchKernelGGL(k_unpack_sym3, dim3(grid_for((long long) n * n, 256, 2048), cnt), dim3(256), 0, s, n, U);
+   HS_LAUNCH_CHECK();
+   return HS_OK;
+}
+
+int hs_unpack_dz_combine(hipStream_t s, int n, const double* pk, const double* P2, const double* sc, int idtau, double eta, const double* Rd,
+   double* dZ)
+{
+   (void) hs_red_batch_flush();
+   hipLaunchKernelGGL(k_unpack_dz_combine, dim3(grid_for((long long) n * n, 256, 2048)), dim3(256), 0, s, n, pk, P2, sc, idtau, eta, Rd, dZ);
    HS_LAUNCH_CHECK();
    return HS_OK;
 }
@@ -540,6 +633,14 @@
    return HS_OK;
 }
 
+int hs_dirmat_pack(hipStream_t s, int n, double s1, const double* Zinv, const double* X, const double* GZ, double* H, double* pk)
+{
+   (void) hs_red_batch_flush();
+   hipLaunchKernelGGL(k_dirmat_pack, dim3(grid_for((long long) n * n, 256, 2048)), dim3(256), 0, s, n, s1, Zinv, X, GZ, H, pk);
+   HS_LAUNCH_CHECK();
+   return HS_OK;
+}
+
 int hs_lp_dir(hipStream_t s, int q, double sigmu, double eta, const double* x, const double* z, const double* r,
    const double* elp, double* out)
 {
@@ -673,6 +774,7 @@
 #define RB_COPY1 101
 #define RB_SOLVE 102
 #define RB_FINISH 103
+#define RB_STAGE2 105
 #define RB_DIRBLK  110
 #define RB_LPDIR   111
 #define RB_VECMUL  112
@@ -801,6 +903,18 @@
       case RED_LPS0:     rb_run<RED_LPS0>(D, sh); break;
       case RB_FILL:      if ( threadIdx.x == 0 ) *(double*) D.p[3] = D.d[0]; break;
       case RB_COPY1:     if ( threadIdx.x == 0 ) *(double*) D.p[3] = *(const double*) D.p[0]; break;
+      case RB_STAGE2:
+      {
+         const double* part = (const double*) D.p[0];
+         double* out = (double*) D.p[3];
+         double v = OpSum::id();
+         for (int i = threadIdx.x; i < D.i[0]; i += 256)
+            v = OpSum::f(v, part[i]);
+         v = block_reduce_256<OpSum>(v, sh);
+         if ( threadIdx.x == 0 )
+            *out = D.accumulate ? OpSum::f(*out, v) : v;
+         break;
+      }
       case RB_DIRBLK:
          d_dir_block_small(D.i[0], D.d[0], (const double*) D.p[0], (const double*) D.p[1], (const double*) D.p[2], (const double*) D.p[3],
             D.d[1], (double*) D.p[4], rb_dyn);
@@ -1659,6 +1773,22 @@
    return reduce_launch<RED_DOT>(s, n, a, b, NULL, out, accumulate, ws);
 }
 
+int hs_dot_deferred(hipStream_t s, long long n, const double* a, const double* b, double* out, int accumulate, double* ws, int slot)
+{
+   const int g = n > 0 ? grid_for(n, 2048, 256) : 0;
+   if ( !g_rb.open || g_rb.hold > 0 || s != g_rb.s || n <= RB_MAXN || g <= 1 || g > HS_DOT_SLOT_DOUBLES || slot < 0 || slot >= HS_DOT_SLOTS )
+      return hs_dot(s, n, a, b, out, accumulate, ws);
+   double* part = ws + HS_DOT_SLOT_DOUBLES * slot;
+   hipLaunchKernelGGL((k_reduce_stage1<RED_DOT>), dim3(g), dim3(256), 0, s, n, a, b, (const double*) NULL, part, out, accumulate, 0);
+   HS_LAUNCH_CHECK();
+   if ( g_rb.args.cnt == RB_MAX )
+      HS_CALL( rb_flush() );
+   rb_desc& D = g_rb.args.d[g_rb.args.cnt++];
+   memset(&D, 0, sizeof(D));
+   D.kind = RB_STAGE2; D.accumulate = accumulate; D.i[0] = g; D.p[0] = part; D.p[3] = out;
+   return HS_OK;
+}
+
 int hs_absmax(hipStream_t s, long long n, const double* a, double* out, int accumulate, double* ws)
 {
    return reduce_launch<RED_ABSMAX>(s, n, a, NULL, NULL, out, accumulate, ws);
diff --git a/scip-sdp_amd/csrc/units.hip b/scip-sdp_amd/csrc/units.hip
--- a/scip-sdp_amd/csrc/units.hip
+++ b/scip-sdp_amd/csrc/units.hip
@@ -700,6 +700,230 @@
    return HIPSDP_OK;
 }
 
+extern "C" long long hipsdp_potrf_dinv_len(int n) { return hs_potrf_dinv_len(n); }
+extern "C" int hipsdp_potrf_pair_unit(int device, int n, int pair, double* A, double* dinv, int* fail)
+{
+   if ( n < 1 || (pair != 0 && pair != 1) || A == NULL || dinv == NULL || fail == NULL )
+      return HIPSDP_ERR_ARG;
+   HS_CALL( pick_device(device) );
+   const long long n2 = (long long) n * n;
+   const long long nd = hs_potrf_dinv_len(n);
+   DevBuf dA, dD;
+   int* dflag = NULL;
+   HS_CALL( dA.alloc(2 * n2) ); HS_CALL( dD.alloc(2 * nd) );
+   HS_HIP( hipMalloc((void**) &dflag, 2 * sizeof(int)) );
+   HS_HIP( hipMemset(dflag, 0, 2 * sizeof(int)) );
+   HS_HIP( hipMemset(dD.p, 0, (size_t) (2 * nd) * sizeof(double)) );
+   HS_CALL( dA.up(A, 2 * n2) );
+   const hs_potrf_job jobs[2] = {{dA.p, dD.p, dflag}, {dA.p + n2, dD.p + nd, dflag + 1}};
+   int rc;
+   if ( pair )
+      rc = hs_potrf_pair(0, n, jobs);
+   else
+   {
+      rc = hs_potrf(0, n, jobs[0].A, jobs[0].dinv, jobs[0].flag, NULL);
+      if ( rc == HS_OK ) rc = hs_potrf(0, n, jobs[1].A, jobs[1].dinv, jobs[1].flag, NULL);
+   }
+   if ( rc == HS_OK && hipDeviceSynchronize() != hipSuccess ) rc = HS_ERR_HIP;
+   int hflag[2] = {0, 0};
+   if ( rc == HS_OK && hipMemcpy(hflag, dflag, 2 * sizeof(int), hipMemcpyDeviceToHost) != hipSuccess ) rc = HS_ERR_HIP;
+   (void) hipFree(dflag);
+   HS_CALL( rc );
+   HS_CALL( dA.down(A, 2 * n2) ); HS_CALL( dD.down(dinv, 2 * nd) );
+   fail[0] = hflag[0]; fail[1] = hflag[1];
+   return HIPSDP_OK;
+}
+
+extern "C" int hipsdp_trial_pair_unit(int device, int n, int fused, int first, double alpha, double* io)
+{
+   if ( n < 1 || (fused != 0 && fused != 1) || (first != 0 && first != 1) || io == NULL )
+      return HIPSDP_ERR_ARG;
+   HS_CALL( pick_device(device) );
+   const long long n2 = (long long) n * n;
+   DevBuf d;
+   HS_CALL( d.alloc(8 * n2) );
+   HS_CALL( d.up(io, 8 * n2) );
+   double* X = d.p; double* Z = d.p + n2; double* dX = d.p + 2 * n2; double* dZ = d.p + 3 * n2;
+   double* Xs = d.p + 4 * n2; double* Zs = d.p + 5 * n2; double* Lx = d.p + 6 * n2; double* Lz = d.p + 7 * n2;
+   const hs_trial_job tj[2] = {{X, dX, Xs, Lx}, {Z, dZ, Zs, Lz}};
+   int rc = HS_OK;
+   if ( fused )
+      rc = hs_trial_pair(0, n2, alpha, first, tj);
+   else
+      for (int k = 0; k < 2 && rc == HS_OK; ++k)
+      {
+         if ( first ) rc = hs_copy(0, tj[k].Vs, tj[k].V, n2);
+         if ( rc == HS_OK ) rc = hs_scale_add(0, n2, alpha, tj[k].dV, 1.0, tj[k].Vs, tj[k].V);
+         if ( rc == HS_OK ) rc = hs_copy(0, tj[k].L, tj[k].V, n2);
+      }
+   if ( rc == HS_OK && hipDeviceSynchronize() != hipSuccess ) rc = HS_ERR_HIP;
+   HS_CALL( rc );
+   HS_CALL( d.down(io, 8 * n2) );
+   return HIPSDP_OK;
+}
+
+namespace {
+int nan_fill(DevBuf& d, long long n) { HS_HIP( hipMemset(d.p, 0xFF, (size_t) (n > 0 ? n : 1) * sizeof(double)) ); return HS_OK; }
+long long packed_len(int n) { const long long t = (long long) n * (n + 1) / 2; return t + (t & 1); }
+}
+
+extern "C" int hipsdp_tail_after_solve2_unit(int device, int m, int fused, const double* rhs2, const double* u1, double* u2, double* wt,
+   double* e2, double* e1)
+{
+   if ( m < 1 || (fused != 0 && fused != 1) || rhs2 == NULL || u1 == NULL || u2 == NULL || wt == NULL || e2 == NULL || e1 == NULL )
+      return HIPSDP_ERR_ARG;
+   HS_CALL( pick_device(device) );
+   DevBuf dR, dU1, dU2, dW, dE2, dE1;
+   HS_CALL( dR.alloc(2 * m) ); HS_CALL( dU1.alloc(m) ); HS_CALL( dU2.alloc(m) ); HS_CALL( dW.alloc(m + 1) ); HS_CALL( dE2.alloc(m + 1) );
+   HS_CALL( dE1.alloc(m + 1) );
+   HS_CALL( nan_fill(dU2, m) ); HS_CALL( nan_fill(dW, m + 1) ); HS_CALL( nan_fill(dE2, m + 1) ); HS_CALL( nan_fill(dE1, m + 1) );
+   HS_CALL( dR.up(rhs2, 2 * m) ); HS_CALL( dU1.up(u1, m) );
+   int rc = hs_ipm_after_solve2(0, m, dR.p, dU2.p, dW.p, dU1.p, dE2.p, dE1.p, fused);
+   if ( rc == HS_OK && hipDeviceSynchronize() != hipSuccess ) rc = HS_ERR_HIP;
+   HS_CALL( rc );
+   HS_CALL( dU2.down(u2, m) ); HS_CALL( dW.down(wt, m + 1) ); HS_CALL( dE2.down(e2, m + 1) ); HS_CALL( dE1.down(e1, m + 1) );
+   return HIPSDP_OK;
+}
+
+extern "C" int hipsdp_tail_unpack3_unit(int device, int n, int fused, const double* pk, double* out)
+{
+   if ( n < 1 || (fused != 0 && fused != 1) || pk == NULL || out == NULL )
+      return HIPSDP_ERR_ARG;
+   HS_CALL( pick_device(device) );
+   const long long n2 = (long long) n * n, Lp = packed_len(n);
+   DevBuf dP, dO;
+   HS_CALL( dP.alloc(3 * Lp) ); HS_CALL( dO.alloc(3 * n2) ); HS_CALL( nan_fill(dO, 3 * n2) );
+   HS_CALL( dP.up(pk, 3 * Lp) );
+   int rc = HS_OK;
+   if ( fused )
+   {
+      const double* p3[3] = {dP.p, dP.p + Lp, dP.p + 2 * Lp};
+      double* o3[3] = {dO.p, dO.p + n2, dO.p + 2 * n2};
+      rc = hs_unpack_sym3(0, n, 3, p3, o3);
+   }
+   else
+      for (int k = 0; k < 3 && rc == HS_OK; ++k)
+         rc = hs_unpack_sym(0, n, dP.p + k * Lp, 0.0, NULL, dO.p + k * n2);
+   if ( rc == HS_OK && hipDeviceSynchronize() != hipSuccess ) rc = HS_ERR_HIP;
+   HS_CALL( rc );
+   return dO.down(out, 3 * n2);
+}
+
+extern "C" int hipsdp_tail_dz_unit(int device, int n, int fused, const double* pk, const double* P2, const double* Rd, double dtau, double eta,
+   double* dZ)
+{
+   if ( n < 1 || (fused != 0 && fused != 1) || pk == NULL || P2 == NULL || Rd == NULL || dZ == NULL )
+      return HIPSDP_ERR_ARG;
+   HS_CALL( pick_device(device) );
+   const long long n2 = (long long) n * n, Lp = packed_len(n);
+   const int nsc = hs_ipm_sc_len(1);
+   DevBuf dP, dP2, dR, dZd, dS;
+   HS_CALL( dP.alloc(Lp) ); HS_CALL( dP2.alloc(n2) ); HS_CALL( dR.alloc(n2) ); HS_CALL( dZd.alloc(n2) ); HS_CALL( dS.alloc(nsc) );
+   HS_CALL( nan_fill(dZd, n2) );
+   std::vector<double> sc((size_t) nsc, 0.0);
+   sc[hs_ipm_sc_dtau()] = dtau;
+   HS_CALL( dS.up(sc.data(), nsc) ); HS_CALL( dP.up(pk, Lp) ); HS_CALL( dP2.up(P2, n2) ); HS_CALL( dR.up(Rd, n2) );
+   int rc;
+   if ( fused )
+      rc = hs_unpack_dz_combine(0, n, dP.p, dP2.p, dS.p, hs_ipm_sc_dtau(), eta, dR.p, dZd.p);
+   else
+   {
+      rc = hs_unpack_sym(0, n, dP.p, 0.0, NULL, dZd.p);
+      if ( rc == HS_OK ) rc = hs_ipm_dz_combine(0, n2, dZd.p, dP2.p, dS.p, eta, dR.p);
+   }
+   if ( rc == HS_OK && hipDeviceSynchronize() != hipSuccess ) rc = HS_ERR_HIP;
+   HS_CALL( rc );
+   return dZd.down(dZ, n2);
+}
+
+extern "C" int hipsdp_tail_dirmat_unit(int device, int n, int fused, double s1, const double* Zinv, const double* X, const double* GZ, double* H,
+   double* pk)
+{
+   if ( n < 1 || (fused != 0 && fused != 1) || Zinv == NULL || X == NULL || GZ == NULL || H == NULL || pk == NULL )
+      return HIPSDP_ERR_ARG;
+   HS_CALL( pick_device(device) );
+   const long long n2 = (long long) n * n, Lp = packed_len(n);
+   DevBuf dZ, dX, dG, dH, dP;
+   HS_CALL( dZ.alloc(n2) ); HS_CALL( dX.alloc(n2) ); HS_CALL( dG.alloc(n2) ); HS_CALL( dH.alloc(n2) ); HS_CALL( dP.alloc(Lp) );
+   HS_CALL( nan_fill(dH, n2) ); HS_CALL( nan_fill(dP, Lp) );
+   HS_CALL( dZ.up(Zinv, n2) ); HS_CALL( dX.up(X, n2) ); HS_CALL( dG.up(GZ, n2) );
+   int rc;
+   if ( fused )
+      rc = hs_dirmat_pack(0, n, s1, dZ.p, dX.p, dG.p, dH.p, dP.p);
+   else
+   {
+      rc = hs_dirmat(0, n, s1, dZ.p, dX.p, dG.p, dH.p);
+      if ( rc == HS_OK ) rc = hs_pack_weighted(0, n, dH.p, dP.p);
+   }
+   if ( rc == HS_OK && hipDeviceSynchronize() != hipSuccess ) rc = HS_ERR_HIP;
+   HS_CALL( rc );
+   HS_CALL( dH.down(H, n2) );
+   return dP.down(pk, Lp);
+}
+
+extern "C" int hipsdp_tail_sc_len(void) { return hs_ipm_sc_len(1); }
+extern "C" int hipsdp_tail_dir_unit(int device, int m, int n, int fused, const double* B, const double* H, const double* rhs2, const double* rp,
+   const double* b, const double* u1, const double* u2, const double* par, double* sc, double* dy, double* dyt)
+{
+   if ( m < 1 || n < 1 || (fused != 0 && fused != 1) || B == NULL || H == NULL || rhs2 == NULL || rp == NULL || b == NULL || u1 == NULL
+         || u2 == NULL || par == NULL || sc == NULL || dy == NULL || dyt == NULL )
+      return HIPSDP_ERR_ARG;
+   HS_CALL( pick_device(device) );
+   const long long n2 = (long long) n * n;
+   const int nsc = hs_ipm_sc_len(1);
+   DevBuf dB, dH, dR, dRp, db, dU1, dU2, dS, dY, dYt, dW;
+   HS_CALL( dB.alloc(n2) ); HS_CALL( dH.alloc(n2) ); HS_CALL( dR.alloc(m) ); HS_CALL( dRp.alloc(m) ); HS_CALL( db.alloc(m) );
+   HS_CALL( dU1.alloc(m) ); HS_CALL( dU2.alloc(m) ); HS_CALL( dS.alloc(nsc) ); HS_CALL( dY.alloc(m) ); HS_CALL( dYt.alloc(m + 1) );
+   HS_CALL( dW.alloc(HS_RED_WS_DOUBLES) );
+   HS_CALL( nan_fill(dY, m) ); HS_CALL( nan_fill(dYt, m + 1) ); HS_CALL( nan_fill(dW, HS_RED_WS_DOUBLES) );
+   HS_CALL( dB.up(B, n2) ); HS_CALL( dH.up(H, n2) ); HS_CALL( dR.up(rhs2, m) ); HS_CALL( dRp.up(rp, m) ); HS_CALL( db.up(b, m) );
+   HS_CALL( dU1.up(u1, m) ); HS_CALL( dU2.up(u2, m) ); HS_CALL( dS.up(sc, nsc) );
+   const double* pB = dB.p; const double* pH = dH.p;
+   const hs_dir_tail_args ta = {m, 0, 1, &n, &pB, &pH, NULL, NULL, dR.p, dRp.p, db.p, dU1.p, dU2.p, dY.p, dYt.p, dS.p, dW.p, NULL, NULL,
+      par[0], par[1], par[2], par[3], par[4], par[5]};
+   hs_red_batch_reset();
+   int rc = hs_ipm_dir_tail(0, &ta, fused, 0);
+   if ( rc == HS_OK && hipDeviceSynchronize() != hipSuccess ) rc = HS_ERR_HIP;
+   hs_red_batch_reset();
+   HS_CALL( rc );
+   HS_CALL( dS.down(sc, nsc) ); HS_CALL( dY.down(dy, m) );
+   return dYt.down(dyt, m + 1);
+}
+
+extern "C" int hipsdp_tail_dots_unit(int device, int m, int n, int fused, const double* a, const double* v, double* out)
+{
+   if ( m < 1 || n < 1 || (fused != 0 && fused != 1) || a == NULL || v == NULL || out == NULL )
+      return HIPSDP_ERR_ARG;
+   HS_CALL( pick_device(device) );
+   const long long n2 = (long long) n * n;
+   DevBuf dA, dV, dO, dW;
+   HS_CALL( dA.alloc(3 * n2) ); HS_CALL( dV.alloc(2 * m) ); HS_CALL( dO.alloc(3) ); HS_CALL( dW.alloc(HS_RED_WS_DOUBLES) );
+   HS_CALL( nan_fill(dO, 3) ); HS_CALL( nan_fill(dW, HS_RED_WS_DOUBLES) );
+   HS_CALL( dA.up(a, 3 * n2) ); HS_CALL( dV.up(v, 2 * m) );
+   const double* a0 = dA.p; const double* a1 = dA.p + n2; const double* a2 = dA.p + 2 * n2;
+   hs_red_batch_reset();
+   hs_red_batch_begin(0);
+   int rc = hs_fill_scalar(0, dO.p, 0.0);
+   if ( fused )
+   {
+      if ( rc == HS_OK ) rc = hs_dot_deferred(0, n2, a0, a1, dO.p, 1, dW.p, 0);
+      if ( rc == HS_OK ) rc = hs_dot_deferred(0, n2, a2, a2, dO.p + 1, 0, dW.p, 1);
+      if ( rc == HS_OK ) rc = hs_dot_deferred(0, n2, a0, a2, dO.p, 1, dW.p, 2);
+   }
+   else
+   {
+      if ( rc == HS_OK ) rc = hs_dot(0, n2, a0, a1, dO.p, 1, dW.p);
+      if ( rc == HS_OK ) rc = hs_dot(0, n2, a2, a2, dO.p + 1, 0, dW.p);
+      if ( rc == HS_OK ) rc = hs_dot(0, n2, a0, a2, dO.p, 1, dW.p);
+   }
+   if ( rc == HS_OK ) rc = hs_dot(0, m, dV.p, dV.p + m, dO.p + 2, 0, dW.p);
+   if ( rc == HS_OK ) rc = hs_red_batch_end();
+   if ( rc == HS_OK && hipDeviceSynchronize() != hipSuccess ) rc = HS_ERR_HIP;
+   hs_red_batch_reset();
+   HS_CALL( rc );
+   return dO.down(out, 3);
+}
+
 extern "C" int hipsdp_trtri(int device, int n, const double* A, double* Linv)
 {
    HS_CALL( pick_device(device) );
```

New measurement: 13.50, median of 6. +1.1%, better.
